# Theseus-AT/mlx-vector-db

Measured on AMD Instinct MI355X. Metric: QPS + p50 latency, cosine top-10 batch=64: 1M×768D @1 GPU; 10M×128D @8 GPU, higher is better.
Workload: dtype f32 (int8 centred corpus x int8 query integer-MFMA candidates, fp64 exact rerank); 1 GPU; c2: 1M x 768 fp32 cosine top-10, batch 64; n_rows=1000000, dim=768, global_batch=64, batch_per_gpu_equiv=64, k=10, metric=cosine, parallelism=single GPU, rows_per_gpu=1000000

## Files before the change

### mlx-vector-db_amd/csrc/vdb_api.cpp

```cpp
#include <hip/hip_runtime.h>

#include <algorithm>
#include <atomic>
#include <cmath>
#include <cstdarg>
#include <cstdio>
#include <cstring>
#include <mutex>
#include <set>
#include <unordered_map>
#include <shared_mutex>
#include <string>
#include <vector>

#include "../../include/vdb.h"
#include "vdb_compact_plan.h"
#include "vdb_subset_plan.h"
#include "vdb_range_plan.h"
#include "vdb_group_plan.h"
#include "vdb_search_plan.h"
#include "vdb_internal.h"

using namespace vdb;

namespace {

thread_local std::string g_last_error;

int set_error(int code, const char* fmt, ...) {
    char buf[1024];
    va_list ap;
    va_start(ap, fmt);
    vsnprintf(buf, sizeof(buf), fmt, ap);
    va_end(ap);
    g_last_error = buf;
    return code;
}

#define HIP_TRY(expr)                                                                                  \
    do {                                                                                               \
        hipError_t _e = (expr);                                                                        \
        if (_e != hipSuccess)                                                                          \
            return set_error(_e == hipErrorOutOfMemory ? VDB_ERR_OOM : VDB_ERR_HIP, "%s failed: %s (%s:%d)", \
                             #expr, hipGetErrorString(_e), __FILE__, __LINE__);                        \
    } while (0)

constexpr int64_t kRowAlign = ROW_ALIGN;

constexpr size_t kGatedExactBytes = 256u << 20;
constexpr int kSubsetBadWord = 12;

inline int64_t round_up(int64_t a, int64_t b) { return (a + b - 1) / b * b; }
inline int next_pow2(int v) {
    int p = 1;
    while (p < v) p <<= 1;
    return p;
}

struct Carver {
    char* base;
    size_t off = 0;
    template <typename T>
    T* take(size_t count) {
        off = (off + 255) & ~size_t(255);
        T* p = reinterpret_cast<T*>(base + off);
        off += count * sizeof(T);
        return p;
    }
};

struct Workspace {
    char* dev = nullptr;
    size_t dev_bytes = 0;
    char* exact = nullptr;
    size_t exact_cap = 0;
    int* host_flag = nullptr;
    char* host_io = nullptr;
    size_t host_io_bytes = 0;
    hipEvent_t done = nullptr;
    static constexpr int kTRing = 64;
    hipEvent_t tring[kTRing][4] = {};
    int t_head = 0, t_pending = 0;
    bool busy = false;
    bool used = false;
    hipStream_t last_st = nullptr;
    hipStream_t own = nullptr;
};

}

struct vdb_index {
    int dim = 0, metric = 0, device = 0;
    int Dp = 0, G = 0;
    int64_t count = 0;
    int64_t cap_rows = 0;
    float* X = nullptr;
    float* Xs = nullptr;
    float* Xq = nullptr;
    int8_t* Xh = nullptr;
    double* nrm64 = nullptr;
    float* inv32 = nullptr;
    float* sq32 = nullptr;
    float* rinit32 = nullptr;
    unsigned long long* d_xmax = nullptr;
    int* d_nonfinite = nullptr;
    double xmax = 0.0;
    double xres_rel = 0.0, xres_abs = 0.0;
    float* d_dir = nullptr;
    bool dir_set = false;
    double xres_dir = 0.0;
    float* d_mu = nullptr;
    float sx = 0.0f;
    int64_t dir_rows = 0;
    unsigned long long* d_i8 = nullptr;
    double i8st[6] = {0, 0, 0, 0, 0, 0};
    uint32_t* d_csum = nullptr;
    int64_t scan_checksum = 1;
    bool auto_i8 = true;
    hipStream_t stream = nullptr;
    int n_cu = 256;
    int64_t precision = VDB_PREC_AUTO;
    std::atomic<int> auto_hold{0}, auto_fails{0}, auto_ok{0};
    std::atomic<int> auto_hold8{0}, auto_fails8{0}, auto_ok8{0};
    std::atomic<bool> last_i8{false};
    std::atomic<unsigned long long> auto_seen{0};
    unsigned long long* h_totals = nullptr;
    int64_t margin = -1;
    int64_t force_exact = 0;
    int64_t n_wg_override = 0;
    int64_t timing = 0;
    int64_t pilot_tiles = -1;
    int64_t graph_fill = 0;
    int64_t scan_variant = 0;
    int64_t scan_variant_b3 = 0;
    int64_t scan_sync = 0;
    int64_t no_fallback = 0;
    int64_t pilot_rank_override = 0;
    bool no_dir_bound = false;
    int64_t finish_split = 1;
    int64_t finish_small = -1;
    int64_t scan_qlds = -1;
    int i8_refine = -1;
    int64_t device_repass = -1;
    std::atomic<int> repass_arm{0};
    int64_t i8_narrow = -1;
    std::atomic<bool> i8_wide{false};
    std::atomic<bool> auto_i8q{true};
    std::atomic<bool> i8q_off{false};
    std::atomic<bool> last_i8q{false};
    std::atomic<int> last_i8q_b{0};
    int64_t scan_q4 = -1;
    int64_t scan_wide = -1;
    int64_t remove_chunk = 0;
    int64_t update_chunk = 0;
    std::atomic<int64_t> gen{0};
    std::atomic<int64_t> n_searches{0}, n_queries{0}, n_fallback{0}, n_overflow{0}, n_incons{0}, n_repass{0}, n_q4{0};
    std::atomic<int64_t> n_wide{0};
    std::atomic<int64_t> n_xs_builds{0};
    std::atomic<int64_t> n_rows_removed{0};
    std::atomic<int64_t> n_rows_updated{0};
    std::atomic<int64_t> n_subset_searches{0}, n_subset_queries{0}, n_subset_rows{0};
    int64_t subset_wgs = 0;
    std::atomic<int64_t> n_range_searches{0}, n_range_queries{0};
    int32_t* groups = nullptr;
    uint32_t* group_valid = nullptr;
    int64_t group_n = 0, group_cap = 0;
    bool group_set = false, group_any_neg = false;
    int64_t group_valid_rows = 0;
    std::atomic<int64_t> n_group_sets{0}, n_group_searches{0}, n_group_queries{0};
    unsigned long long* d_group_fb = nullptr;
    int64_t group_fetch = 0;
    int64_t group_force_exact = 0;
    std::atomic<int64_t> n_by_prec[N_PREC] = {{0}, {0}, {0}, {0}, {0}, {0}};
    std::atomic<int64_t> scan_ns{0}, pipe_ns{0}, n_timed{0};
    unsigned long long* d_totals = nullptr;
    std::shared_mutex mu;
    std::mutex xs_mu;
    std::mutex ws_mu;
    std::vector<Workspace*> pool;
    std::unordered_map<hipStream_t, hipEvent_t> uses;
};

namespace {

std::mutex g_reg_mu;
std::set<vdb_index*> g_indices;

void free_workspace_memory(Workspace* w) {
    if (w->dev) (void)hipFree(w->dev);
    if (w->exact) (void)hipFree(w->exact);
    if (w->host_flag) (void)hipHostFree(w->host_flag);
    if (w->host_io) (void)hipHostFree(w->host_io);
    w->dev = nullptr;
    w->exact = nullptr;
    w->host_flag = nullptr;
    w->host_io = nullptr;
    w->dev_bytes = w->exact_cap = w->host_io_bytes = 0;
}

int wait_idle(vdb_index* ix);

enum XsKind { kXsNone = -1, kXsFp32 = 0, kXsSplit = 1 };
int xs_kind(int64_t precision) {
    if (precision == VDB_PREC_FP32) return kXsFp32;
    if (precision == VDB_PREC_I8 || precision == VDB_PREC_I8X3 || precision == VDB_PREC_I8Q) return kXsNone;
    return kXsSplit;
}
bool needs_i8(int64_t precision, bool auto_i8) {
    return precision == VDB_PREC_I8 || precision == VDB_PREC_I8X3 || precision == VDB_PREC_I8Q ||
           (precision == VDB_PREC_AUTO && auto_i8);
}
bool xs_eager(const vdb_index* ix) {
    const int kind = xs_kind(ix->precision);
    return kind == kXsFp32 || (kind == kXsSplit && !(ix->precision == VDB_PREC_AUTO && ix->auto_i8));
}
float* xs_ptr(const vdb_index* ix) { return __atomic_load_n(&ix->Xs, __ATOMIC_ACQUIRE); }

hipError_t build_candidate_rows(const vdb_index* ix, int64_t row0, int64_t n, hipStream_t st, bool xs = true,
                                bool xq = true) {
    const float* inv = ix->metric == VDB_METRIC_COSINE ? ix->inv32 : nullptr;
    hipError_t e = hipSuccess;
    if (xs && ix->Xs && xs_kind(ix->precision) == kXsFp32) e = launch_tile_rows(ix->X, ix->G, row0, n, ix->Xs, st);
    if (xs && ix->Xs && xs_kind(ix->precision) == kXsSplit) e = launch_split_rows(ix->X, ix->G, row0, n, inv, ix->Xs, st);
    if (e == hipSuccess && xq && needs_i8(ix->precision, ix->auto_i8)) {
        if (row0 == 0) e = hipMemsetAsync(ix->d_csum, 0, (size_t)2 * ix->Dp * sizeof(uint32_t), st);
        if (e == hipSuccess)
            e = launch_quant_rows(ix->X, inv, ix->d_mu, ix->d_dir, ix->sx, row0, n, ix->G, ix->Xq, ix->d_i8, st, ix->Xh);
        if (e == hipSuccess) e = launch_colsum8(ix->Xq, row0, n, ix->G / 4, ix->d_csum, st);
    }
    return e;
}

hipError_t read_i8_stats(vdb_index* ix, hipStream_t st) {
    unsigned long long b[6];
    hipError_t e = hipMemcpyAsync(b, ix->d_i8, sizeof(b), hipMemcpyDeviceToHost, st);
    if (e == hipSuccess) e = hipStreamSynchronize(st);
    if (e == hipSuccess) std::memcpy(ix->i8st, b, sizeof(b));
    return e;
}

hipError_t zero_now(void* p, size_t bytes, hipStream_t st) {
    hipError_t e = hipMemsetAsync(p, 0, bytes, st);
    if (e == hipSuccess) e = hipStreamSynchronize(st);
    return e;
}

bool debug_knobs_enabled() {
    const char* e = std::getenv("VDB_DEBUG_KNOBS");
    return e && std::strcmp(e, "1") == 0;
}

int ensure_capacity(vdb_index* ix, int64_t rows) {
    if (rows <= ix->cap_rows) return VDB_OK;
    if (ix->X) {
        const int wr = wait_idle(ix);
        if (wr) return wr;
    }
    int64_t cap = std::max<int64_t>(ix->cap_rows * 2, kRowAlign);
    while (cap < rows) cap *= 2;
    cap = round_up(cap, kRowAlign);
    const size_t tile_floats = (size_t)ix->G * BLOCK_FLOATS;
    const size_t x_bytes = (size_t)(cap / 32) * tile_floats * sizeof(float);
    float* X = nullptr;
    float* Xs = nullptr;
    float* Xq = nullptr;
    int8_t* Xh = nullptr;
    double* n64 = nullptr;
    float *i32 = nullptr, *s32 = nullptr, *r32 = nullptr;
    auto fail = [&](hipError_t e, const char* what) {
        (void)hipStreamSynchronize(ix->stream);
        for (void* p : {(void*)X, (void*)Xs, (void*)Xq, (void*)Xh, (void*)n64, (void*)i32, (void*)s32, (void*)r32})
            if (p) (void)hipFree(p);
        return set_error(e == hipErrorOutOfMemory ? VDB_ERR_OOM : VDB_ERR_HIP,
                         "growing the index to %lld rows: %s failed: %s", (long long)cap, what, hipGetErrorString(e));
    };
#define CAP_TRY(expr)                          \
    do {                                       \
        hipError_t _e = (expr);                \
        if (_e != hipSuccess) return fail(_e, #expr); \
    } while (0)
    CAP_TRY(hipMalloc(&X, x_bytes));
    if (ix->Xs || xs_eager(ix)) {
        CAP_TRY(hipMalloc(&Xs, x_bytes));
        CAP_TRY(hipMemsetAsync(Xs, 0, x_bytes, ix->stream));
    }
    const bool with_xq = ix->Xq || needs_i8(ix->precision, ix->auto_i8);
    if (with_xq) {
        CAP_TRY(hipMalloc(&Xq, x_bytes / 2));
        CAP_TRY(hipMemsetAsync(Xq, 0, x_bytes / 2, ix->stream));
        CAP_TRY(hipMalloc(&Xh, x_bytes / 4));
        CAP_TRY(hipMemsetAsync(Xh, 0, x_bytes / 4, ix->stream));
    }
    CAP_TRY(hipMalloc(&n64, cap * sizeof(double)));
    CAP_TRY(hipMalloc(&i32, cap * sizeof(float)));
    CAP_TRY(hipMalloc(&s32, cap * sizeof(float)));
    CAP_TRY(hipMalloc(&r32, cap * sizeof(float)));
    CAP_TRY(hipMemsetAsync(r32, 0, cap * sizeof(float), ix->stream));
    CAP_TRY(hipMemsetAsync(X, 0, x_bytes, ix->stream));
    CAP_TRY(hipMemsetAsync(n64, 0, cap * sizeof(double), ix->stream));
    CAP_TRY(hipMemsetAsync(i32, 0, cap * sizeof(float), ix->stream));
    CAP_TRY(hipMemsetAsync(s32, 0, cap * sizeof(float), ix->stream));
    if (ix->X) {
        const int64_t used_tiles = round_up(ix->count, 128) / 32;
        CAP_TRY(hipMemcpyAsync(X, ix->X, (size_t)ix->count * ix->Dp * sizeof(float), hipMemcpyDeviceToDevice,
                               ix->stream));
        if (Xs && ix->Xs)
            CAP_TRY(hipMemcpyAsync(Xs, ix->Xs, (size_t)used_tiles * tile_floats * sizeof(float),
                                   hipMemcpyDeviceToDevice, ix->stream));
        if (Xq && ix->Xq)
            CAP_TRY(hipMemcpyAsync(Xq, ix->Xq, (size_t)used_tiles * tile_floats * sizeof(float) / 2,
                                   hipMemcpyDeviceToDevice, ix->stream));
        if (Xh && ix->Xh)
            CAP_TRY(hipMemcpyAsync(Xh, ix->Xh, (size_t)ix->count * ix->Dp, hipMemcpyDeviceToDevice, ix->stream));
        CAP_TRY(hipMemcpyAsync(n64, ix->nrm64, ix->count * sizeof(double), hipMemcpyDeviceToDevice, ix->stream));
        CAP_TRY(hipMemcpyAsync(i32, ix->inv32, ix->count * sizeof(float), hipMemcpyDeviceToDevice, ix->stream));
        CAP_TRY(hipMemcpyAsync(s32, ix->sq32, ix->count * sizeof(float), hipMemcpyDeviceToDevice, ix->stream));
        CAP_TRY(hipMemcpyAsync(r32, ix->rinit32, ix->count * sizeof(float), hipMemcpyDeviceToDevice, ix->stream));
    }
    CAP_TRY(hipStreamSynchronize(ix->stream));
#undef CAP_TRY
    if (ix->X) {
        (void)hipFree(ix->X);
        if (ix->Xs) (void)hipFree(ix->Xs);
        if (ix->Xq) (void)hipFree(ix->Xq);
        if (ix->Xh) (void)hipFree(ix->Xh);
        (void)hipFree(ix->nrm64);
        (void)hipFree(ix->inv32);
        (void)hipFree(ix->sq32);
        (void)hipFree(ix->rinit32);
    }
    ix->X = X;
    ix->Xs = Xs;
    ix->Xq = Xq;
    ix->Xh = Xh;
    ix->nrm64 = n64;
    ix->inv32 = i32;
    ix->sq32 = s32;
    ix->rinit32 = r32;
    ix->cap_rows = cap;
    return VDB_OK;
}

int ensure_xq(vdb_index* ix) {
    if (ix->Xq || ix->cap_rows == 0) return VDB_OK;
    const size_t bytes = (size_t)(ix->cap_rows / 32) * ix->G * BLOCK_FLOATS * sizeof(float) / 2;
    float* Xq = nullptr;
    int8_t* Xh = nullptr;
    hipError_t e = hipMalloc(&Xq, bytes);
    if (e == hipSuccess) e = hipMalloc(&Xh, bytes / 2);
    if (e == hipSuccess) e = hipMemsetAsync(Xq, 0, bytes, ix->stream);
    if (e == hipSuccess) e = hipMemsetAsync(Xh, 0, bytes / 2, ix->stream);
    if (e == hipSuccess) e = hipStreamSynchronize(ix->stream);
    if (e != hipSuccess) {
        if (Xq) (void)hipFree(Xq);
        if (Xh) (void)hipFree(Xh);
        return set_error(e == hipErrorOutOfMemory ? VDB_ERR_OOM : VDB_ERR_HIP, "int8 copy: %s", hipGetErrorString(e));
    }
    ix->Xq = Xq;
    ix->Xh = Xh;
    return VDB_OK;
}

int ensure_xs(vdb_index* ix) {
    if (xs_ptr(ix) || ix->cap_rows == 0 || xs_kind(ix->precision) == kXsNone) return VDB_OK;
    std::lock_guard<std::mutex> lg(ix->xs_mu);
    if (ix->Xs) return VDB_OK;
    const size_t bytes = (size_t)(ix->cap_rows / 32) * ix->G * BLOCK_FLOATS * sizeof(float);
    float* Xs = nullptr;
    hipError_t e = hipMalloc(&Xs, bytes);
    if (e == hipSuccess) e = hipMemsetAsync(Xs, 0, bytes, ix->stream);
    if (e == hipSuccess && ix->count > 0) {
        const float* inv = ix->metric == VDB_METRIC_COSINE ? ix->inv32 : nullptr;
        e = xs_kind(ix->precision) == kXsFp32 ? launch_tile_rows(ix->X, ix->G, 0, ix->count, Xs, ix->stream)
                                              : launch_split_rows(ix->X, ix->G, 0, ix->count, inv, Xs, ix->stream);
    }
    if (e == hipSuccess) e = hipStreamSynchronize(ix->stream);
    if (e != hipSuccess) {
        if (Xs) (void)hipFree(Xs);
        return set_error(e == hipErrorOutOfMemory ? VDB_ERR_OOM : VDB_ERR_HIP, "split candidate copy: %s",
                         hipGetErrorString(e));
    }
    __atomic_store_n(&ix->Xs, Xs, __ATOMIC_RELEASE);
    ix->n_xs_builds++;
    return VDB_OK;
}

constexpr size_t kMaxWs = 16;

Workspace* acquire_ws(vdb_index* ix, hipStream_t st, bool own = false) {
    std::lock_guard<std::mutex> g(ix->ws_mu);
    Workspace* idle = nullptr;
    Workspace* any = nullptr;
    for (Workspace* w : ix->pool) {
        if (w->busy) continue;
        if (!w->used || (!own && w->last_st == st)) {
            w->busy = true;
            return w;
        }
        if (!idle && w->done && hipEventQuery(w->done) == hipSuccess) idle = w;
        if (!any) any = w;
    }
    Workspace* w = idle ? idle : ix->pool.size() >= kMaxWs ? any : nullptr;
    if (!w) {
        w = new Workspace();
        ix->pool.push_back(w);
    }
    w->busy = true;
    return w;
}

bool others_in_flight(vdb_index* ix, const Workspace* self) {
    std::lock_guard<std::mutex> g(ix->ws_mu);
    for (Workspace* w : ix->pool) {
        if (w == self) continue;
        if (w->busy) return true;
        if (w->used && w->done && hipEventQuery(w->done) == hipErrorNotReady) return true;
    }
    return false;
}

void release_ws(vdb_index* ix, Workspace* w, hipStream_t st) {
    if (w->done == nullptr) (void)hipEventCreateWithFlags(&w->done, hipEventDisableTiming);
    (void)hipEventRecord(w->done, st);
    w->used = true;
    w->last_st = st;
    std::lock_guard<std::mutex> g(ix->ws_mu);
    w->busy = false;
}

int note_use(vdb_index* ix, hipStream_t st) {
    std::lock_guard<std::mutex> g(ix->ws_mu);
    if (ix->uses.size() >= 64 && !ix->uses.count(st)) {
        for (auto it = ix->uses.begin(); it != ix->uses.end();) {
            if (hipEventQuery(it->second) == hipSuccess) {
                (void)hipEventDestroy(it->second);
                it = ix->uses.erase(it);
            } else {
                ++it;
            }
        }
    }
    hipEvent_t& e = ix->uses[st];
    if (!e) HIP_TRY(hipEventCreateWithFlags(&e, hipEventDisableTiming));
    HIP_TRY(hipEventRecord(e, st));
    return VDB_OK;
}

int wait_idle(vdb_index* ix) {
    std::vector<hipEvent_t> evs;
    {
        std::lock_guard<std::mutex> g(ix->ws_mu);
        for (Workspace* w : ix->pool)
            if (w->used && w->done) evs.push_back(w->done);
        for (auto& kv : ix->uses) evs.push_back(kv.second);
    }
    for (hipEvent_t e : evs) HIP_TRY(hipEventSynchronize(e));
    HIP_TRY(hipStreamSynchronize(ix->stream));
    return VDB_OK;
}

int flush_timing(vdb_index* ix, Workspace* w, int n = Workspace::kTRing) {
    while (w->t_pending > 0 && n-- > 0) {
        hipEvent_t* ev = w->tring[(w->t_head - w->t_pending + Workspace::kTRing) % Workspace::kTRing];
        HIP_TRY(hipEventSynchronize(ev[2]));
        float ms_scan = 0.f, ms_pipe = 0.f;
        HIP_TRY(hipEventElapsedTime(&ms_scan, ev[0], ev[1]));
        HIP_TRY(hipEventElapsedTime(&ms_pipe, ev[3], ev[2]));
        ix->scan_ns += (int64_t)(ms_scan * 1e6);
        ix->pipe_ns += (int64_t)(ms_pipe * 1e6);
        ix->n_timed++;
        w->t_pending--;
    }
    return VDB_OK;
}

int flush_all_timing(vdb_index* ix) {
    std::lock_guard<std::mutex> g(ix->ws_mu);
    for (Workspace* w : ix->pool)
        if (!w->busy) {
            const int rc = flush_timing(ix, w);
            if (rc) return rc;
        }
    return VDB_OK;
}

int ws_reserve(Workspace* w, size_t bytes, hipStream_t st) {
    if (w->used && w->done) HIP_TRY(hipStreamWaitEvent(st, w->done, 0));
    if (!w->host_flag) HIP_TRY(hipHostMalloc(&w->host_flag, 64 * sizeof(int), hipHostMallocDefault));
    if (bytes > w->dev_bytes) {
        if (w->dev) {
            HIP_TRY(hipStreamSynchronize(st));
            (void)hipFree(w->dev);
            w->dev = nullptr;
        }
        size_t nb = std::max(bytes, w->dev_bytes * 2);
        HIP_TRY(hipMalloc(&w->dev, nb));
        w->dev_bytes = nb;
    }
    return VDB_OK;
}

int ws_host_io(Workspace* w, size_t bytes) {
    if (bytes > w->host_io_bytes) {
        const size_t nb = std::max(bytes, w->host_io_bytes * 2);
        if (w->host_io) (void)hipHostFree(w->host_io);
        w->host_io = nullptr;
        w->host_io_bytes = 0;
        HIP_TRY(hipHostMalloc(&w->host_io, nb, hipHostMallocDefault));
        w->host_io_bytes = nb;
    }
    return VDB_OK;
}

int ws_reserve_exact(Workspace* w, size_t bytes, hipStream_t st) {
    if (bytes > w->exact_cap) {
        if (w->exact) {
            HIP_TRY(hipStreamSynchronize(st));
            (void)hipFree(w->exact);
            w->exact = nullptr;
        }
        HIP_TRY(hipMalloc(&w->exact, bytes));
        w->exact_cap = bytes;
    }
    return VDB_OK;
}

bool all_finite(const float* p, int64_t n) {
    for (int64_t i = 0; i < n; ++i)
        if (!std::isfinite(p[i])) return false;
    return true;
}

struct SearchLease {
    vdb_index* ix;
    Workspace* w = nullptr;
    hipStream_t st = nullptr;
    int rc = VDB_OK;
    SearchLease(vdb_index* ix_, int32_t mem, void* stream) : ix(ix_) {
        const bool own_stream = mem == VDB_MEM_HOST && !stream;
        st = own_stream ? nullptr : (hipStream_t)stream;
        w = acquire_ws(ix, st, own_stream);
        if (!own_stream) return;
        if (!w->own) {
            const hipError_t e = hipStreamCreateWithFlags(&w->own, hipStreamNonBlocking);
            if (e != hipSuccess) {
                {
                    std::lock_guard<std::mutex> lg(ix->ws_mu);
                    w->busy = false;
                }
                w = nullptr;
                rc = set_error(VDB_ERR_HIP, "workspace stream: %s", hipGetErrorString(e));
                return;
            }
        }
        st = w->own;
    }
    ~SearchLease() {
        if (w) release_ws(ix, w, st);
    }
    SearchLease(const SearchLease&) = delete;
    SearchLease& operator=(const SearchLease&) = delete;
};

hipError_t order_after_caller(hipStream_t st, void* caller_stream) {
    hipEvent_t ready = nullptr;
    hipError_t e = hipEventCreateWithFlags(&ready, hipEventDisableTiming);
    if (e != hipSuccess) return e;
    e = hipEventRecord(ready, (hipStream_t)caller_stream);
    if (e == hipSuccess) e = hipStreamWaitEvent(st, ready, 0);
    (void)hipEventDestroy(ready);
    return e;
}

template <typename Pack>
int stage_up(Workspace* w, int64_t in0, int64_t in_bytes, int64_t out_bytes, hipStream_t st, Pack&& pack) {
    const int rc = ws_host_io(w, (size_t)(in_bytes + out_bytes));
    if (rc) return rc;
    pack(w->host_io);
    HIP_TRY(hipMemcpyAsync(w->dev + in0, w->host_io, (size_t)in_bytes, hipMemcpyHostToDevice, st));
    return VDB_OK;
}
int stage_down(Workspace* w, int64_t in_bytes, int64_t out0, int64_t out_bytes, hipStream_t st, const char** r) {
    *r = w->host_io + in_bytes;
    HIP_TRY(hipMemcpyAsync(w->host_io + in_bytes, w->dev + out0, (size_t)out_bytes, hipMemcpyDeviceToHost, st));
    HIP_TRY(hipStreamSynchronize(st));
    return VDB_OK;
}


SearchKnobs search_knobs(const vdb_index* ix, bool i8_narrow) {
    SearchKnobs kn{};
    kn.force_exact = ix->force_exact != 0;
    kn.margin = ix->margin;
    kn.i8_narrow = i8_narrow;
    kn.scan_q4 = ix->scan_q4;
    kn.scan_wide = ix->scan_wide;
    kn.n_wg_override = ix->n_wg_override;
    kn.scan_variant = ix->scan_variant;
    kn.scan_sync = ix->scan_sync;
    kn.finish_split = ix->finish_split;
    kn.i8_refine = ix->i8_refine;
    kn.scan_checksum = ix->scan_checksum;
    kn.pilot_tiles = ix->pilot_tiles;
    kn.pilot_rank_override = ix->pilot_rank_override;
    kn.has_xh = ix->Xh != nullptr;
    kn.has_csum = ix->d_csum != nullptr;
    return kn;
}

SearchKernelFacts kernel_facts(const SearchShape& s, const SearchKnobs& kn, const SearchKP& kp) {
    SearchKernelFacts f{};
    const int Gs = search_groups(s.prec, s.G);
    if (prec_is_i8(s.prec)) {
        f.scan8wl_ok = scan8wl_ok(s.prec, s.metric, Gs, s.B);
        f.scan8w_ok = scan8w_ok(Gs, s.B);
        f.rows_per_step = scan8_rows_per_step(s.prec, s.metric);
    } else if (s.prec == PREC_BF16X3 || s.prec == PREC_BF16) {
        f.rows_per_step = scan2_rows_per_step(false);
        f.rows_per_step_q4 = scan2_rows_per_step(true);
    } else {
        f.scan_variant_ok = scan_variant_ok(s.prec, (int)kn.scan_variant, Gs);
        const int v = f.scan_variant_ok ? (int)kn.scan_variant : 0;
        f.rows_per_step = scan_rows_per_step(s.prec, v);
        f.scan_priv = scan_priv(s.prec, v, kp.KP);
    }
    return f;
}

size_t gated_exact_bytes(const vdb_index* ix, int nq, int k) {
    const ExactPlan ep = exact_plan(ix->count, ix->n_cu, nq, k, true);
    return (size_t)exact_gate_bytes(ep, nq, (int64_t)exact_scan_scratch_bytes(ep.KE, ep.n_wg_gate, ep.slots));
}

int run_exact(vdb_index* ix, Workspace* w, const float* Qd, const double* qn64, const int* qlist_dev, int nq, int k,
              const uint32_t* mask_dev, float* out_s, int64_t* out_i, double* out_k, int64_t index_offset,
              const int64_t* row_ids, hipStream_t st, const int* qcount_dev = nullptr, const int* ovf_dev = nullptr,
              int* done_dev = nullptr, unsigned long long* host_totals = nullptr) {
    const int64_t N = ix->count;
    const bool gated = qcount_dev != nullptr;
    const ExactPlan ep = exact_plan(N, ix->n_cu, nq, k, gated);
    const int KE = ep.KE, n_wg = ep.n_wg, n_lists = ep.n_wg;
    const int64_t rpw = ep.rpw;
    const ExactLayout el =
        exact_layout(ep, nq, gated && done_dev ? (int64_t)exact_scan_scratch_bytes(KE, n_wg, ep.slots) : 0);
    int rc = ws_reserve_exact(w, (size_t)el.total, st);
    if (rc) return rc;
    double* lk = reinterpret_cast<double*>(w->exact + el.lk);
    uint32_t* li = reinterpret_cast<uint32_t*>(w->exact + el.li);
    double* mk = reinterpret_cast<double*>(w->exact + el.mk);
    uint32_t* mi = reinterpret_cast<uint32_t*>(w->exact + el.mi);
    char* gscr = el.scr >= 0 ? w->exact + el.scr : nullptr;
    if (gated && done_dev) {
        const ExactTail tail{done_dev, mk, mi, k, index_offset, out_s, out_i, out_k, row_ids, host_totals};
        HIP_TRY(launch_exact_scan(ix->metric, KE, Qd, qn64, qlist_dev, nq, ix->X, ix->G, ix->dim, ix->nrm64, mask_dev,
                                  N, n_wg, rpw, lk, li, st, qcount_dev, ovf_dev, ix->d_totals, &tail, kGateSlots,
                                  gscr));
        return VDB_OK;
    }
    HIP_TRY(launch_exact_scan(ix->metric, KE, Qd, qn64, qlist_dev, nq, ix->X, ix->G, ix->dim, ix->nrm64, mask_dev, N,
                              n_wg, rpw, lk, li, st, qcount_dev, ovf_dev, gated ? ix->d_totals : nullptr));
    HIP_TRY(launch_merge_f64_u32(KE, lk, li, n_lists, KE, (int64_t)n_lists * KE, KE, nq, mk, mi, st, qcount_dev));
    HIP_TRY(launch_finalize_u32(ix->metric, mk, mi, KE, nq, qlist_dev, k, index_offset, out_s, out_i, out_k, st,
                                qcount_dev, row_ids));
    return VDB_OK;
}

}

extern "C" {

const char* vdb_last_error(void) { return g_last_error.c_str(); }

int32_t vdb_version(void) { return 2; }

int32_t vdb_device_count(int32_t* n) {
    int c = 0;
    hipError_t e = hipGetDeviceCount(&c);
    if (e != hipSuccess) c = 0;
    if (n) *n = c;
    return VDB_OK;
}

int32_t vdb_index_create(int32_t dim, int32_t metric, int32_t device, vdb_index** out) {
    if (!out) return set_error(VDB_ERR_INVALID, "out is NULL");
    *out = nullptr;
    if (dim <= 0 || dim > 65536) return set_error(VDB_ERR_INVALID, "dimension must be in [1, 65536], got %d", dim);
    if (metric != VDB_METRIC_COSINE && metric != VDB_METRIC_EUCLIDEAN)
        return set_error(VDB_ERR_UNSUPPORTED, "unsupported metric id %d (cosine=0, euclidean=1)", metric);
    int ndev = 0;
    if (hipGetDeviceCount(&ndev) != hipSuccess || ndev == 0)
        return set_error(VDB_ERR_NODEVICE, "no HIP device visible: the vdb core needs an MI355X (gfx950)");
    if (device < 0 || device >= ndev) return set_error(VDB_ERR_INVALID, "device %d out of range [0,%d)", device, ndev);
    HIP_TRY(hipSetDevice(device));
    hipDeviceProp_t prop;
    HIP_TRY(hipGetDeviceProperties(&prop, device));
    if (std::strncmp(prop.gcnArchName, "gfx950", 6) != 0)
        return set_error(VDB_ERR_NODEVICE, "device %d is %s; this build targets gfx950 only", device,
                         prop.gcnArchName);
    vdb_index* ix = new vdb_index();
    ix->dim = dim;
    ix->metric = metric;
    ix->device = device;
    ix->Dp = (int)round_up(dim, 64);
    ix->G = ix->Dp / GROUP_DIMS;
    ix->n_cu = prop.multiProcessorCount;
    if (const char* q4 = std::getenv("VDB_SCAN_Q4")) ix->scan_q4 = std::min(1, std::max(-1, std::atoi(q4)));
    if (const char* a8 = std::getenv("VDB_AUTO_I8")) ix->auto_i8 = std::atoi(a8) != 0;
    hipError_t e = hipStreamCreateWithFlags(&ix->stream, hipStreamNonBlocking);
    if (e == hipSuccess) e = hipMalloc(&ix->d_xmax, 192);
    if (e == hipSuccess) e = zero_now(ix->d_xmax, 192, ix->stream);
    if (e == hipSuccess) e = hipMalloc(&ix->d_i8, 64);
    if (e == hipSuccess) e = zero_now(ix->d_i8, 64, ix->stream);
    if (e == hipSuccess) e = hipMalloc(&ix->d_csum, (size_t)2 * ix->Dp * sizeof(uint32_t));
    if (e == hipSuccess) e = zero_now(ix->d_csum, (size_t)2 * ix->Dp * sizeof(uint32_t), ix->stream);
    if (e != hipSuccess) {
        delete ix;
        return set_error(VDB_ERR_HIP, "index setup failed: %s", hipGetErrorString(e));
    }
    ix->d_nonfinite = reinterpret_cast<int*>(reinterpret_cast<char*>(ix->d_xmax) + 32);
    {
        std::lock_guard<std::mutex> rg(g_reg_mu);
        g_indices.insert(ix);
    }
    *out = ix;
    return VDB_OK;
}

int32_t vdb_index_destroy(vdb_index* ix) {
    if (!ix) return VDB_OK;
    {
        std::lock_guard<std::mutex> rg(g_reg_mu);
        g_indices.erase(ix);
    }
    (void)hipSetDevice(ix->device);
    (void)wait_idle(ix);
    for (Workspace* w : ix->pool) {
        free_workspace_memory(w);
        if (w->done) (void)hipEventDestroy(w->done);
        if (w->own) (void)hipStreamDestroy(w->own);
        for (int r = 0; r < Workspace::kTRing; ++r)
            for (int e = 0; e < 4; ++e)
                if (w->tring[r][e]) (void)hipEventDestroy(w->tring[r][e]);
        delete w;
    }
    if (ix->X) (void)hipFree(ix->X);
    if (ix->Xs) (void)hipFree(ix->Xs);
    if (ix->Xq) (void)hipFree(ix->Xq);
    if (ix->Xh) (void)hipFree(ix->Xh);
    if (ix->nrm64) (void)hipFree(ix->nrm64);
    if (ix->inv32) (void)hipFree(ix->inv32);
    if (ix->sq32) (void)hipFree(ix->sq32);
    if (ix->rinit32) (void)hipFree(ix->rinit32);
    if (ix->d_xmax) (void)hipFree(ix->d_xmax);
    if (ix->d_dir) (void)hipFree(ix->d_dir);
    if (ix->d_mu) (void)hipFree(ix->d_mu);
    if (ix->d_i8) (void)hipFree(ix->d_i8);
    if (ix->d_csum) (void)hipFree(ix->d_csum);
    if (ix->d_totals) (void)hipFree(ix->d_totals);
    if (ix->groups) (void)hipFree(ix->groups);
    if (ix->group_valid) (void)hipFree(ix->group_valid);
    if (ix->d_group_fb) (void)hipFree(ix->d_group_fb);
    if (ix->h_totals) (void)hipHostFree(ix->h_totals);
    for (auto& kv : ix->uses) (void)hipEventDestroy(kv.second);
    if (ix->stream) (void)hipStreamDestroy(ix->stream);
    delete ix;
    return VDB_OK;
}

int32_t vdb_index_reserve(vdb_index* ix, int64_t rows) {
    if (!ix) return set_error(VDB_ERR_INVALID, "index is NULL");
    if (rows < 0) return set_error(VDB_ERR_INVALID, "rows must be >= 0");
    HIP_TRY(hipSetDevice(ix->device));
    std::unique_lock<std::shared_mutex> g(ix->mu);
    return ensure_capacity(ix, rows);
}

int32_t vdb_index_set_param(vdb_index* ix, const char* name, int64_t value) {
    if (!ix || !name) return set_error(VDB_ERR_INVALID, "NULL argument");
    std::string n(name);
    if (n == "precision") {
        if (value != VDB_PREC_FP32 && value != VDB_PREC_BF16X3 && value != VDB_PREC_BF16 && value != VDB_PREC_AUTO &&
            value != VDB_PREC_I8 && value != VDB_PREC_I8X3 && value != VDB_PREC_I8Q)
            return set_error(VDB_ERR_INVALID,
                             "precision must be %d (fp32), %d (bf16x3), %d (bf16), %d (auto), %d (i8), %d (i8x3) or "
                             "%d (i8q), got %lld",
                             VDB_PREC_FP32, VDB_PREC_BF16X3, VDB_PREC_BF16, VDB_PREC_AUTO, VDB_PREC_I8, VDB_PREC_I8X3,
                             VDB_PREC_I8Q, (long long)value);
        HIP_TRY(hipSetDevice(ix->device));
        std::unique_lock<std::shared_mutex> g(ix->mu);
        if (value == ix->precision) return VDB_OK;
        const int wr = wait_idle(ix);
        if (wr) return wr;
        const bool xs = xs_kind(value) != kXsNone && xs_kind(value) != xs_kind(ix->precision);
        const bool xq = needs_i8(value, ix->auto_i8) && !needs_i8(ix->precision, ix->auto_i8);
        if (xq) {
            const int xr = ensure_xq(ix);
            if (xr) return xr;
        }
        ix->precision = value;
        bool built = false;
        if (!ix->Xs && xs_eager(ix)) {
            const int xr = ensure_xs(ix);
            if (xr) return xr;
            built = true;
        }
        if (((xs && !built) || xq) && ix->X && ix->count > 0) {
            HIP_TRY(build_candidate_rows(ix, 0, ix->count, ix->stream, xs && !built, xq));
            HIP_TRY(read_i8_stats(ix, ix->stream));
        }
    } else if (n == "auto_i8q") {
        ix->auto_i8q = value != 0;
    } else if (n == "auto_int8") {
        HIP_TRY(hipSetDevice(ix->device));
        std::unique_lock<std::shared_mutex> g(ix->mu);
        const bool v = value != 0;
        if (v == ix->auto_i8) return VDB_OK;
        const int wr = wait_idle(ix);
        if (wr) return wr;
        const bool xq = needs_i8(ix->precision, v) && !needs_i8(ix->precision, ix->auto_i8);
        if (xq) {
            const int xr = ensure_xq(ix);
            if (xr) return xr;
        }
        ix->auto_i8 = v;
        if (!ix->Xs && xs_eager(ix)) {
            const int xr = ensure_xs(ix);
            if (xr) return xr;
        }
        if (xq && ix->X && ix->count > 0) {
            HIP_TRY(build_candidate_rows(ix, 0, ix->count, ix->stream, false, true));
            HIP_TRY(read_i8_stats(ix, ix->stream));
        }
    } else if (n == "margin") {
        ix->margin = value;
    } else if (n == "force_exact") {
        ix->force_exact = value != 0;
    } else if (n == "n_wg") {
        ix->n_wg_override = value;
    } else if (n == "scan_sync") {
        if (value < 0 || value > 2) return set_error(VDB_ERR_INVALID, "scan_sync must be 0, 1 or 2");
        ix->scan_sync = value;
    } else if (n == "scan_variant") {
        if (value < 0 || value > 2) return set_error(VDB_ERR_INVALID, "scan_variant must be 0, 1 or 2");
        ix->scan_variant = value;
    } else if (n == "scan_variant_bf16x3") {
        if (value != 0) return set_error(VDB_ERR_INVALID, "the split-bf16 pass has one variant (0)");
        ix->scan_variant_b3 = value;
    } else if (n == "graph_fill") {
        if (value < 0 || value > 1) return set_error(VDB_ERR_INVALID, "graph_fill must be 0 or 1");
        ix->graph_fill = value;
    } else if (n == "pilot_tiles") {
        if (value < -1 || value > 32768) return set_error(VDB_ERR_INVALID, "pilot_tiles must be in [-1, 32768]");
        ix->pilot_tiles = value;
    } else if (n == "timing") {
        ix->timing = value != 0;
    } else if (n == "no_fallback") {
        ix->no_fallback = value != 0;
    } else if (n == "finish_small") {
        if (value < -1 || value > 1) return set_error(VDB_ERR_INVALID, "finish_small must be -1, 0 or 1");
        ix->finish_small = value;
    } else if (n == "finish_split") {
        if (value < 1 || value > 8) return set_error(VDB_ERR_INVALID, "finish_split must be in [1, 8]");
        ix->finish_split = value;
    } else if (n == "scan_qlds") {
        if (value < -1 || value > 2) return set_error(VDB_ERR_INVALID, "scan_qlds must be -1 (auto), 0, 1 or 2");
        ix->scan_qlds = value;
    } else if (n == "scan_wide") {
        if (value < -1 || value > 1) return set_error(VDB_ERR_INVALID, "scan_wide must be -1, 0 or 1");
        ix->scan_wide = value;
    } else if (n == "scan_q4") {
        if (value < -1 || value > 1) return set_error(VDB_ERR_INVALID, "scan_q4 must be -1, 0 or 1");
        ix->scan_q4 = value;
    } else if (n == "dir_bound") {
        ix->no_dir_bound = value == 0;
    } else if (n == "i8_refine") {
        if (value < -1 || value > 1) return set_error(VDB_ERR_INVALID, "i8_refine must be -1, 0 or 1");
        ix->i8_refine = (int)value;
    } else if (n == "i8_narrow") {
        if (value < -1 || value > 0) return set_error(VDB_ERR_INVALID, "i8_narrow must be -1 or 0");
        ix->i8_narrow = value;
    } else if (n == "remove_chunk") {
        if (value < 0) return set_error(VDB_ERR_INVALID, "remove_chunk must be >= 0 (0 = sized by bytes)");
        std::unique_lock<std::shared_mutex> g(ix->mu);
        ix->remove_chunk = value;
    } else if (n == "update_chunk") {
        if (value < 0) return set_error(VDB_ERR_INVALID, "update_chunk must be >= 0 (0 = sized by bytes)");
        std::unique_lock<std::shared_mutex> g(ix->mu);
        ix->update_chunk = value;
    } else if (n == "subset_wgs") {
        if (value < 0 || value > kSubsetMaxSeg)
            return set_error(VDB_ERR_INVALID, "subset_wgs must be in [0, %d] (0 = auto)", kSubsetMaxSeg);
        std::unique_lock<std::shared_mutex> g(ix->mu);
        ix->subset_wgs = value;
    } else if (n == "group_fetch") {
        if (value < 0 || value > kGroupMaxFetch)
            return set_error(VDB_ERR_INVALID, "group_fetch must be in [0, %d] (0 = auto)", kGroupMaxFetch);
        std::unique_lock<std::shared_mutex> g(ix->mu);
        ix->group_fetch = value;
    } else if (n == "group_force_exact") {
        if (value < 0 || value > 1) return set_error(VDB_ERR_INVALID, "group_force_exact must be 0 or 1");
        std::unique_lock<std::shared_mutex> g(ix->mu);
        ix->group_force_exact = value;
    } else if (n == "device_repass") {
        if (value < -1 || value > 1) return set_error(VDB_ERR_INVALID, "device_repass must be -1, 0 or 1");
        ix->device_repass = value;
    } else if (n.rfind("debug_", 0) == 0 && !debug_knobs_enabled()) {
        return set_error(VDB_ERR_INVALID, "'%s' is a test-only knob (set VDB_DEBUG_KNOBS=1)", name);
    } else if (n == "debug_sink_row8") {
        HIP_TRY(hipSetDevice(ix->device));
        std::unique_lock<std::shared_mutex> g(ix->mu);
        if (value < 0 || value >= ix->count || !ix->Xq)
            return set_error(VDB_ERR_INVALID, "debug_sink_row8: no int8 row %lld", (long long)value);
        const int wr = wait_idle(ix);
        if (wr) return wr;
        HIP_TRY(launch_sink_row8(ix->Xq, value, ix->G / 4, ix->stream));
        HIP_TRY(hipStreamSynchronize(ix->stream));
    } else if (n == "scan_checksum") {
        if (value < 0 || value > 2) return set_error(VDB_ERR_INVALID, "scan_checksum must be 0, 1 or 2");
        ix->scan_checksum = value;
    } else if (n == "debug_stale_rinit") {
        if (value < 0) return set_error(VDB_ERR_INVALID, "debug_stale_rinit: row must be >= 0");
        HIP_TRY(hipSetDevice(ix->device));
        std::unique_lock<std::shared_mutex> g(ix->mu);
        if (value >= ix->count || !ix->rinit32) return set_error(VDB_ERR_INVALID, "debug_stale_rinit: no row %lld", (long long)value);
        const int wr = wait_idle(ix);
        if (wr) return wr;
        const float zero = 0.0f;
        HIP_TRY(hipMemcpyAsync(ix->rinit32 + value, &zero, sizeof(float), hipMemcpyHostToDevice, ix->stream));
        HIP_TRY(hipStreamSynchronize(ix->stream));
    } else if (n == "pilot_rank") {
        if (value < 0 || value > 256) return set_error(VDB_ERR_INVALID, "pilot_rank must be in [0, 256]");
        ix->pilot_rank_override = value;
    } else {
        return set_error(VDB_ERR_INVALID, "unknown parameter '%s'", name);
    }
    return VDB_OK;
}

int32_t vdb_index_get_stat(const vdb_index* cix, const char* name, int64_t* value) {
    if (!cix || !name || !value) return set_error(VDB_ERR_INVALID, "NULL argument");
    vdb_index* ix = const_cast<vdb_index*>(cix);
    std::string n(name);
    unsigned long long dt[4] = {0, 0, 0, 0};
    if ((n == "fallback_queries" || n == "overflow_queries" || n == "repass_queries") && ix->d_totals) {
        HIP_TRY(hipSetDevice(ix->device));
        const int wr = wait_idle(ix);
        if (wr) return wr;
        HIP_TRY(hipMemcpy(dt, ix->d_totals, sizeof(dt), hipMemcpyDeviceToHost));
    }
    if (n == "scan_ns" || n == "pipeline_ns" || n == "timed_searches") {
        HIP_TRY(hipSetDevice(ix->device));
        const int rc = flush_all_timing(ix);
        if (rc) return rc;
    }
    if (n == "searches") *value = ix->n_searches.load();
    else if (n == "queries") *value = ix->n_queries.load();
    else if (n == "fallback_queries") *value = ix->n_fallback.load() + (int64_t)dt[0];
    else if (n == "repass_queries") *value = ix->n_repass.load() + (int64_t)dt[3];
    else if (n == "searches_q4") *value = ix->n_q4.load();
    else if (n == "searches_wide") *value = ix->n_wide.load();
    else if (n == "auto_hold") *value = ix->auto_hold.load();
    else if (n == "auto_hold8") *value = ix->auto_hold8.load();
    else if (n == "overflow_queries") *value = ix->n_overflow.load() + (int64_t)dt[1];
    else if (n == "inconsistent_queries") *value = ix->n_incons.load();
    else if (n == "capacity") *value = ix->cap_rows;
    else if (n == "scan_ns") *value = ix->scan_ns.load();
    else if (n == "pipeline_ns") *value = ix->pipe_ns.load();
    else if (n == "timed_searches") *value = ix->n_timed.load();
    else if (n == "count") *value = ix->count;
    else if (n == "precision") *value = ix->precision;
    else if (n == "searches_fp32") *value = ix->n_by_prec[PREC_FP32].load();
    else if (n == "searches_bf16x3") *value = ix->n_by_prec[PREC_BF16X3].load();
    else if (n == "searches_bf16") *value = ix->n_by_prec[PREC_BF16].load();
    else if (n == "searches_i8") *value = ix->n_by_prec[PREC_I8].load();
    else if (n == "searches_i8x3") *value = ix->n_by_prec[PREC_I8X3].load();
    else if (n == "auto_int8") *value = ix->auto_i8 ? 1 : 0;
    else if (n == "auto_i8q") *value = ix->auto_i8q ? 1 : 0;
    else if (n == "i8q_off") *value = ix->i8q_off.load() ? 1 : 0;
    else if (n == "searches_i8q") *value = ix->n_by_prec[PREC_I8Q].load();
    else if (n == "i8_wide") *value = ix->i8_wide ? 1 : 0;
    else if (n == "device_bytes") {
        const int64_t xb = (int64_t)(ix->cap_rows / 32) * ix->G * BLOCK_FLOATS * 4;
        *value = xb + (xs_ptr(ix) ? xb : 0) + (ix->Xq ? xb / 2 : 0) + (ix->Xh ? xb / 4 : 0) + ix->cap_rows * 20;
    } else if (n == "split_copy") *value = xs_ptr(ix) ? 1 : 0;
    else if (n == "split_copy_builds") *value = ix->n_xs_builds.load();
    else if (n == "rows_removed") *value = ix->n_rows_removed.load();
    else if (n == "rows_updated") *value = ix->n_rows_updated.load();
    else if (n == "subset_searches") *value = ix->n_subset_searches.load();
    else if (n == "subset_queries") *value = ix->n_subset_queries.load();
    else if (n == "subset_rows") *value = ix->n_subset_rows.load();
    else if (n == "range_searches") *value = ix->n_range_searches.load();
    else if (n == "range_queries") *value = ix->n_range_queries.load();
    else if (n == "group_rows") *value = ix->group_set ? ix->group_n : 0;
    else if (n == "group_sets") *value = ix->n_group_sets.load();
    else if (n == "group_searches") *value = ix->n_group_searches.load();
    else if (n == "group_queries") *value = ix->n_group_queries.load();
    else if (n == "group_fallback_queries") {
        unsigned long long fb = 0;
        if (ix->d_group_fb) {
            HIP_TRY(hipSetDevice(ix->device));
            const int wr = wait_idle(ix);
            if (wr) return wr;
            HIP_TRY(hipMemcpy(&fb, ix->d_group_fb, sizeof(fb), hipMemcpyDeviceToHost));
        }
        *value = (int64_t)fb;
    }
    else if (n == "subset_bad_ids") {
        HIP_TRY(hipSetDevice(ix->device));
        const int wr = wait_idle(ix);
        if (wr) return wr;
        unsigned long long bad = 0;
        HIP_TRY(hipMemcpy(&bad, ix->d_xmax + kSubsetBadWord, sizeof(bad), hipMemcpyDeviceToHost));
        *value = (int64_t)bad;
    }
    else return set_error(VDB_ERR_INVALID, "unknown stat '%s'", name);
    return VDB_OK;
}

constexpr int64_t kDirRows = 65536;

static hipError_t setup_direction(vdb_index* ix, int64_t row0, int64_t n, hipStream_t st) {
    if (ix->dir_set) return hipSuccess;
    const float* inv = ix->metric == VDB_METRIC_COSINE ? ix->inv32 : nullptr;
    const int D = ix->dim;
    const int64_t m = std::min(n, kDirRows);
    hipError_t e = hipSuccess;
    if (!ix->d_dir) e = hipMalloc(&ix->d_dir, (size_t)ix->Dp * sizeof(float));
    if (e == hipSuccess && !ix->d_mu) e = hipMalloc(&ix->d_mu, (size_t)ix->Dp * sizeof(float));
    double* sums = nullptr;
    if (e == hipSuccess) e = hipMalloc(&sums, (size_t)D * sizeof(double));
    if (e == hipSuccess) e = hipMemsetAsync(sums, 0, (size_t)D * sizeof(double), st);
    if (e == hipSuccess) e = launch_dir_sum(ix->X, inv, row0, m, D, ix->G, sums, st);
    std::vector<double> h(D);
    if (e == hipSuccess) e = hipMemcpyAsync(h.data(), sums, (size_t)D * sizeof(double), hipMemcpyDeviceToHost, st);
    if (e == hipSuccess) e = hipStreamSynchronize(st);
    if (sums) (void)hipFree(sums);
    if (e != hipSuccess) return e;
    double nn = 0.0;
    for (double v : h) nn += v * v;
    std::vector<float> dir(ix->Dp, 0.0f), mu(ix->Dp, 0.0f);
    if (nn > 0.0 && std::isfinite(nn))
        for (int d = 0; d < D; ++d) dir[d] = (float)(h[d] / std::sqrt(nn));
    for (int d = 0; d < D; ++d) mu[d] = (float)(h[d] / (double)std::max<int64_t>(m, 1));
    e = hipMemcpyAsync(ix->d_dir, dir.data(), (size_t)ix->Dp * sizeof(float), hipMemcpyHostToDevice, st);
    if (e == hipSuccess)
        e = hipMemcpyAsync(ix->d_mu, mu.data(), (size_t)ix->Dp * sizeof(float), hipMemcpyHostToDevice, st);
    uint32_t zb = 0;
    uint32_t* dz = reinterpret_cast<uint32_t*>(ix->d_i8 + 6);
    if (e == hipSuccess) e = hipMemsetAsync(dz, 0, sizeof(uint32_t), st);
    if (e == hipSuccess) e = launch_zmax(ix->X, inv, ix->d_mu, row0, m, D, ix->G, dz, st);
    if (e == hipSuccess) e = hipMemcpyAsync(&zb, dz, sizeof(zb), hipMemcpyDeviceToHost, st);
    if (e == hipSuccess) e = hipStreamSynchronize(st);
    if (e != hipSuccess) return e;
    float zmax = 0.0f;
    std::memcpy(&zmax, &zb, sizeof(zmax));
    ix->sx = zmax > 0.0f && std::isfinite(zmax) ? 1.25f * zmax / 127.0f : 1.0f;
    ix->dir_rows = m;
    ix->dir_set = true;
    return hipSuccess;
}

static hipError_t residual_direction(vdb_index* ix, int64_t row0, int64_t n, hipStream_t st) {
    const float* inv = ix->metric == VDB_METRIC_COSINE ? ix->inv32 : nullptr;
    return launch_resid_dir(ix->X, inv, row0, n, ix->dim, ix->G, ix->d_dir, ix->d_xmax + 3, st);
}

int32_t vdb_index_add(vdb_index* ix, const float* vectors, int64_t n, int32_t mem, void* stream) {
    if (!ix) return set_error(VDB_ERR_INVALID, "index is NULL");
    if (n < 0) return set_error(VDB_ERR_INVALID, "n must be >= 0");
    if (n == 0) return VDB_OK;
    if (!vectors) return set_error(VDB_ERR_INVALID, "vectors is NULL");
    if (ix->count + n > (int64_t)0xFFFFFFFE) return set_error(VDB_ERR_INVALID, "index is limited to 2^32-2 rows");
    HIP_TRY(hipSetDevice(ix->device));
    std::unique_lock<std::shared_mutex> g(ix->mu);
    hipStream_t st = ix->stream;
    int rc = ensure_capacity(ix, ix->count + n);
    if (rc) return rc;
    if (ix->count > 0 && ix->dir_rows < kDirRows) {
        const int wr = wait_idle(ix);
        if (wr) return wr;
    }
    HIP_TRY(hipMemsetAsync(ix->d_nonfinite, 0, sizeof(int), st));
    char* bak = reinterpret_cast<char*>(ix->d_xmax);
    HIP_TRY(hipMemcpyAsync(bak + 64, ix->d_xmax, 32, hipMemcpyDeviceToDevice, st));
    HIP_TRY(hipMemcpyAsync(bak + 128, ix->d_i8, 64, hipMemcpyDeviceToDevice, st));
    if (mem == VDB_MEM_DEVICE) {
        HIP_TRY(order_after_caller(st, stream));
    }
    const int D = ix->dim;
    const int64_t chunk = std::max<int64_t>(1, (int64_t)(256ll << 20) / ((int64_t)D * 4));
    float* staging = nullptr;
    if (mem == VDB_MEM_HOST) HIP_TRY(hipMalloc(&staging, (size_t)std::min(chunk, n) * D * sizeof(float)));
    for (int64_t r = 0; r < n; r += chunk) {
        const int64_t m = std::min(chunk, n - r);
        const float* src = vectors + r * D;
        if (mem == VDB_MEM_HOST) {
            hipError_t e = hipMemcpyAsync(staging, src, (size_t)m * D * sizeof(float), hipMemcpyHostToDevice, st);
            if (e == hipSuccess)
                e = launch_pack_rows(staging, m, D, ix->G, ix->X, ix->count + r, ix->nrm64, ix->inv32, ix->sq32,
                                     ix->rinit32, ix->metric == VDB_METRIC_COSINE, ix->d_xmax, ix->d_nonfinite, st);
            if (e == hipSuccess) e = setup_direction(ix, ix->count + r, m, st);
            if (e == hipSuccess) e = build_candidate_rows(ix, ix->count + r, m, st);
            if (e == hipSuccess) e = residual_direction(ix, ix->count + r, m, st);
            if (e == hipSuccess) e = hipStreamSynchronize(st);
            if (e != hipSuccess) {
                (void)hipFree(staging);
                return set_error(VDB_ERR_HIP, "ingest failed: %s", hipGetErrorString(e));
            }
        } else {
            HIP_TRY(launch_pack_rows(src, m, D, ix->G, ix->X, ix->count + r, ix->nrm64, ix->inv32, ix->sq32,
                                     ix->rinit32, ix->metric == VDB_METRIC_COSINE, ix->d_xmax, ix->d_nonfinite, st));
            HIP_TRY(setup_direction(ix, ix->count + r, m, st));
            HIP_TRY(build_candidate_rows(ix, ix->count + r, m, st));
            HIP_TRY(residual_direction(ix, ix->count + r, m, st));
        }
    }
    if (staging) (void)hipFree(staging);
    int nonfinite = 0;
    unsigned long long xb[4] = {0, 0, 0, 0};
    HIP_TRY(hipMemcpyAsync(&nonfinite, ix->d_nonfinite, sizeof(int), hipMemcpyDeviceToHost, st));
    HIP_TRY(hipMemcpyAsync(xb, ix->d_xmax, sizeof(xb), hipMemcpyDeviceToHost, st));
    HIP_TRY(read_i8_stats(ix, st));
    if (nonfinite) {
        if (ix->count == 0) {
            ix->dir_set = false;
            ix->dir_rows = 0;
            HIP_TRY(hipMemsetAsync(ix->d_xmax, 0, 32, st));
            HIP_TRY(hipMemsetAsync(ix->d_i8, 0, 64, st));
            HIP_TRY(hipStreamSynchronize(st));
            std::memset(ix->i8st, 0, sizeof(ix->i8st));
        } else {
            HIP_TRY(hipMemcpyAsync(ix->d_xmax, bak + 64, 32, hipMemcpyDeviceToDevice, st));
            HIP_TRY(hipMemcpyAsync(ix->d_i8, bak + 128, 64, hipMemcpyDeviceToDevice, st));
            if (ix->Xq && needs_i8(ix->precision, ix->auto_i8)) {
                HIP_TRY(hipMemsetAsync(ix->d_csum, 0, (size_t)2 * ix->Dp * sizeof(uint32_t), st));
                HIP_TRY(launch_colsum8(ix->Xq, 0, ix->count, ix->G / 4, ix->d_csum, st));
            }
            HIP_TRY(read_i8_stats(ix, st));
        }
        return set_error(VDB_ERR_NONFINITE, "%d row(s) contain NaN or Inf; nothing was added", nonfinite);
    }
    if (ix->dir_rows < kDirRows && ix->count + n >= 2 * ix->dir_rows) {
        const int64_t all = ix->count + n;
        ix->dir_set = false;
        HIP_TRY(hipMemsetAsync(ix->d_xmax + 3, 0, 8, st));
        HIP_TRY(hipMemsetAsync(ix->d_i8, 0, 64, st));
        HIP_TRY(setup_direction(ix, 0, all, st));
        if (needs_i8(ix->precision, ix->auto_i8)) HIP_TRY(build_candidate_rows(ix, 0, all, st, false, true));
        HIP_TRY(residual_direction(ix, 0, all, st));
        HIP_TRY(hipMemcpyAsync(xb, ix->d_xmax, sizeof(xb), hipMemcpyDeviceToHost, st));
        HIP_TRY(read_i8_stats(ix, st));
    }
    double xm[4];
    std::memcpy(xm, xb, sizeof(xm));
    ix->xmax = xm[0];
    ix->xres_rel = xm[1];
    ix->xres_abs = xm[2];
    ix->xres_dir = xm[3];
    ix->count += n;
    ix->group_set = false;
    ix->auto_hold = 0;
    ix->auto_fails = 0;
    ix->auto_hold8 = 0;
    ix->auto_fails8 = 0;
    if (ix->h_totals) ix->auto_seen = ix->h_totals[0];
    return VDB_OK;
}

int32_t vdb_index_count(const vdb_index* ix, int64_t* n) {
    if (!ix || !n) return set_error(VDB_ERR_INVALID, "NULL argument");
    *n = ix->count;
    return VDB_OK;
}

static int32_t clear_locked(vdb_index* ix) {
    {
        const int wr = wait_idle(ix);
        if (wr) return wr;
    }
    if (ix->X) {
        HIP_TRY(hipMemsetAsync(ix->X, 0, (size_t)(ix->cap_rows / 32) * ix->G * BLOCK_FLOATS * sizeof(float),
                               ix->stream));
        HIP_TRY(hipMemsetAsync(ix->nrm64, 0, ix->cap_rows * sizeof(double), ix->stream));
        if (ix->Xs)
            HIP_TRY(hipMemsetAsync(ix->Xs, 0, (size_t)(ix->cap_rows / 32) * ix->G * BLOCK_FLOATS * sizeof(float),
                                   ix->stream));
        if (ix->Xq)
            HIP_TRY(hipMemsetAsync(ix->Xq, 0, (size_t)(ix->cap_rows / 32) * ix->G * BLOCK_FLOATS * sizeof(float) / 2,
                                   ix->stream));
    }
    HIP_TRY(hipMemsetAsync(ix->d_xmax, 0, 64, ix->stream));
    HIP_TRY(hipMemsetAsync(ix->d_i8, 0, 64, ix->stream));
    HIP_TRY(hipMemsetAsync(ix->d_csum, 0, (size_t)2 * ix->Dp * sizeof(uint32_t), ix->stream));
    HIP_TRY(hipStreamSynchronize(ix->stream));
    std::memset(ix->i8st, 0, sizeof(ix->i8st));
    ix->count = 0;
    ix->group_set = false;
    ix->auto_hold = 0;
    ix->auto_fails = 0;
    ix->auto_hold8 = 0;
    ix->auto_fails8 = 0;
    ix->xmax = 0.0;
    ix->xres_rel = ix->xres_abs = 0.0;
    ix->dir_set = false;
    ix->dir_rows = 0;
    ix->xres_dir = 0.0;
    ix->gen++;
    return VDB_OK;
}

// ... 219 lines not shown
                                            ix->d_i8, ix->Xh, st));
            UP_TRY(launch_update_colsum8(ix->Xq, d_ids, m, N, G8, +1, ix->d_csum, st));
        }
        UP_TRY(launch_update_resid_dir(ix->X, inv, d_ids, m, N, D, ix->G, ix->d_dir, ix->d_xmax + 3, st));
        if (host && r + m < n) UP_TRY(hipStreamSynchronize(st));
    }
    unsigned long long xb[4] = {0, 0, 0, 0};
    UP_TRY(hipMemcpyAsync(xb, ix->d_xmax, sizeof(xb), hipMemcpyDeviceToHost, st));
    UP_TRY(read_i8_stats(ix, st));
#undef UP_TRY
    (void)done(VDB_OK);
    double xm[4];
    std::memcpy(xm, xb, sizeof(xm));
    ix->xmax = xm[0];
    ix->xres_rel = xm[1];
    ix->xres_abs = xm[2];
    ix->xres_dir = xm[3];
    ix->gen++;
    ix->n_rows_updated += n;
    ix->auto_hold = 0;
    ix->auto_fails = 0;
    ix->auto_hold8 = 0;
    ix->auto_fails8 = 0;
    if (ix->h_totals) ix->auto_seen = ix->h_totals[0];
    return VDB_OK;
}

int32_t vdb_index_get_vectors(vdb_index* ix, int64_t start, int64_t n, float* out_host) {
    if (!ix || (!out_host && n > 0)) return set_error(VDB_ERR_INVALID, "NULL argument");
    if (start < 0 || n < 0 || start + n > ix->count)
        return set_error(VDB_ERR_INVALID, "rows [%lld, %lld) out of range [0, %lld)", (long long)start,
                         (long long)(start + n), (long long)ix->count);
    if (n == 0) return VDB_OK;
    HIP_TRY(hipSetDevice(ix->device));
    std::shared_lock<std::shared_mutex> g(ix->mu);
    const int D = ix->dim;
    const int64_t chunk = std::max<int64_t>(1, (int64_t)(256ll << 20) / ((int64_t)D * 4));
    float* tmp = nullptr;
    HIP_TRY(hipMalloc(&tmp, (size_t)std::min(chunk, n) * D * sizeof(float)));
    for (int64_t r = 0; r < n; r += chunk) {
        const int64_t m = std::min(chunk, n - r);
        hipError_t e = launch_unpack_rows(ix->X, ix->G, D, start + r, m, tmp, ix->stream);
        if (e == hipSuccess)
            e = hipMemcpyAsync(out_host + r * D, tmp, (size_t)m * D * sizeof(float), hipMemcpyDeviceToHost, ix->stream);
        if (e == hipSuccess) e = hipStreamSynchronize(ix->stream);
        if (e != hipSuccess) {
            (void)hipFree(tmp);
            return set_error(VDB_ERR_HIP, "export failed: %s", hipGetErrorString(e));
        }
    }
    (void)hipFree(tmp);
    return VDB_OK;
}

constexpr int32_t kRetryBf16x3 = 1 << 20;
constexpr int kRepassMax = 64;
constexpr int kRepassArm = 256;
constexpr int kAutoBf16MaxK = 16;

void auto_fail(vdb_index* ix) {
    const int f = std::min(8, ix->auto_fails.load() + 1);
    ix->auto_fails = f;
    ix->auto_ok = 0;
    ix->auto_hold = 16 << (f - 1);
}

bool auto_take_hold(vdb_index* ix) {
    int h = ix->auto_hold.load();
    while (h > 0)
        if (ix->auto_hold.compare_exchange_weak(h, h - 1)) return true;
    if (++ix->auto_ok >= 64) ix->auto_fails = 0;
    return false;
}

void auto_fail8(vdb_index* ix) {
    const int f = std::min(8, ix->auto_fails8.load() + 1);
    ix->auto_fails8 = f;
    ix->auto_ok8 = 0;
    ix->auto_hold8 = 16 << (f - 1);
}
bool auto_take_hold8(vdb_index* ix) {
    int h = ix->auto_hold8.load();
    while (h > 0)
        if (ix->auto_hold8.compare_exchange_weak(h, h - 1)) return true;
    if (++ix->auto_ok8 >= 64) ix->auto_fails8 = 0;
    return false;
}

static int32_t search_locked(vdb_index* ix, const float* queries, int32_t B, int32_t k, const uint32_t* row_mask,
                             int32_t mem, float* out_scores, int64_t* out_indices, double* out_keys,
                             int64_t index_offset, void* stream, const int64_t* row_ids, struct SearchOpts opt);

static int repass_flagged(vdb_index* ix, const float* Qd, const int* flag_list, int n, int k, const uint32_t* md,
                          float* out_s, int64_t* out_i, double* out_k, int64_t index_offset, const int64_t* row_ids,
                          hipStream_t st);

struct SearchOpts {
    bool force_b3 = false;
    bool repass = false;
    const int* gate = nullptr;
    bool force_i8x3 = false;
};

static int32_t search_locked(vdb_index* ix, const float* queries, int32_t B, int32_t k, const uint32_t* row_mask,
                             int32_t mem, float* out_scores, int64_t* out_indices, double* out_keys,
                             int64_t index_offset, void* stream, const int64_t* row_ids, SearchOpts opt);

static int32_t search_impl(vdb_index* ix, const float* queries, int32_t B, int32_t k, const uint32_t* row_mask,
                           int32_t mem, float* out_scores, int64_t* out_indices, double* out_keys,
                           int64_t index_offset, void* stream, const int64_t* row_ids, bool force_b3 = false) {
    if (!ix) return set_error(VDB_ERR_INVALID, "index is NULL");
    if (B <= 0) return set_error(VDB_ERR_INVALID, "n_queries must be >= 1, got %d", B);
    if (k <= 0 || k > 1024) return set_error(VDB_ERR_INVALID, "k must be in [1, 1024], got %d", k);
    if (!queries || !out_scores || !out_indices) return set_error(VDB_ERR_INVALID, "NULL query/output pointer");
    if (mem != VDB_MEM_HOST && mem != VDB_MEM_DEVICE) return set_error(VDB_ERR_INVALID, "bad mem kind %d", mem);
    if (mem == VDB_MEM_HOST && !all_finite(queries, (int64_t)B * ix->dim))
        return set_error(VDB_ERR_NONFINITE, "query contains NaN or Inf");
    HIP_TRY(hipSetDevice(ix->device));
    std::shared_lock<std::shared_mutex> g(ix->mu);
    SearchOpts opt;
    opt.force_b3 = force_b3;
    return search_locked(ix, queries, B, k, row_mask, mem, out_scores, out_indices, out_keys, index_offset, stream,
                         row_ids, opt);
}

static int repass_flagged(vdb_index* ix, const float* Qd, const int* flag_list, int n, int k, const uint32_t* md,
                          float* out_s, int64_t* out_i, double* out_k, int64_t index_offset, const int64_t* row_ids,
                          hipStream_t st) {
    const int D = ix->dim;
    const size_t qb = round_up((int64_t)n * D * 4, 256), sb = round_up((int64_t)n * k * 4, 256),
                 lb = round_up((int64_t)n * k * 8, 256);
    char* buf = nullptr;
    HIP_TRY(hipMallocAsync((void**)&buf, qb + sb + 2 * lb, st));
    float* Qs = (float*)buf;
    float* ss = (float*)(buf + qb);
    int64_t* si = (int64_t*)(buf + qb + sb);
    double* sk = (double*)(buf + qb + sb + lb);
    hipError_t e = launch_gather_rows(Qd, D, flag_list, n, Qs, st);
    int rc = e == hipSuccess ? VDB_OK : set_error(VDB_ERR_HIP, "re-pass gather: %s", hipGetErrorString(e));
    if (rc == VDB_OK) {
        SearchOpts o;
        o.force_b3 = true;
        o.repass = true;
        rc = search_locked(ix, Qs, n, k, md, VDB_MEM_DEVICE, ss, si, sk, index_offset, st, row_ids, o);
    }
    if (rc == VDB_OK) {
        e = launch_scatter_results(flag_list, n, k, ss, si, sk, out_s, out_i, out_k, st);
        if (e != hipSuccess) rc = set_error(VDB_ERR_HIP, "re-pass scatter: %s", hipGetErrorString(e));
    }
    (void)hipFreeAsync(buf, st);
    ix->n_repass += n;
    return rc;
}

static int32_t search_locked(vdb_index* ix, const float* queries, int32_t B, int32_t k, const uint32_t* row_mask,
                             int32_t mem, float* out_scores, int64_t* out_indices, double* out_keys,
                             int64_t index_offset, void* stream, const int64_t* row_ids, SearchOpts opt) {
    const int D = ix->dim;
    const int64_t N = ix->count;
    if (!opt.repass) {
        ix->n_searches++;
        ix->n_queries += B;
    }

    const bool auto_prec = ix->precision == VDB_PREC_AUTO;
    if (auto_prec && ix->h_totals && !opt.repass) {
        const unsigned long long seen = ix->h_totals[0];
        const unsigned long long prev = ix->auto_seen.exchange(seen);
        if (seen > prev) {
            if (ix->last_i8q && seen - prev > (unsigned long long)std::max(1, ix->last_i8q_b.load() / 8))
                ix->i8q_off = true;
            if (ix->last_i8) {
                auto_fail8(ix);
                ix->i8_wide = true;
            } else {
                auto_fail(ix);
            }
            ix->repass_arm = kRepassArm;
        }
    }
    const bool approx = N > 0 && !(ix->force_exact || k > kMaxApproxK);
    const bool auto_b16 = k <= kAutoBf16MaxK;
    const bool x3_i8 = auto_prec && !opt.force_b3 && !auto_b16 && ix->auto_i8;
    const bool auto_x3 = auto_prec && (opt.force_b3 || !auto_b16 || (approx && auto_take_hold(ix)));
    const bool hold8 = auto_prec && ix->auto_i8 && approx && (x3_i8 || !auto_x3) && auto_take_hold8(ix);
    const bool auto_8 = auto_prec && !auto_x3 && ix->auto_i8 && !hold8;
    const bool auto_8x3 = x3_i8 && !hold8;
    const bool auto_8q = auto_8x3 && ix->metric == 1 && k <= 100 && ix->auto_i8q && !ix->i8q_off;
    const bool force_8x3 = auto_prec && opt.force_i8x3 && ix->auto_i8 && ix->Xq;
    const int prec_req = !ix->X ? PREC_FP32
                         : force_8x3 ? PREC_I8X3
                         : ix->precision == VDB_PREC_BF16X3 ? PREC_BF16X3
                         : ix->precision == VDB_PREC_BF16 ? PREC_BF16
                         : ix->precision == VDB_PREC_I8X3 ? PREC_I8X3
                         : ix->precision == VDB_PREC_I8Q ? PREC_I8Q
                         : ix->precision == VDB_PREC_I8 ? PREC_I8
                         : auto_prec ? (auto_x3 ? (auto_8x3 ? (auto_8q ? PREC_I8Q : PREC_I8X3) : PREC_BF16X3)
                                                 : auto_8 ? PREC_I8 : PREC_BF16)
                                     : PREC_FP32;
    if (auto_prec && approx && (!auto_x3 || x3_i8)) {
        ix->last_i8 = auto_8 || auto_8x3;
        ix->last_i8q = prec_req == PREC_I8Q;
        ix->last_i8q_b = (int)B;
    }
    if (approx && !opt.gate) ix->n_by_prec[prec_req]++;
    const bool one_plane = prec_req == PREC_BF16 || prec_req == PREC_I8;

    const int prec = prec_req;
    SearchShape sh{};
    sh.B = B; sh.k = k; sh.D = D; sh.Dp = ix->Dp; sh.G = ix->G; sh.metric = ix->metric; sh.N = N; sh.n_cu = ix->n_cu;
    sh.prec = prec; sh.host = mem == VDB_MEM_HOST; sh.gated = opt.gate != nullptr; sh.repass = opt.repass;
    const SearchKnobs kn = search_knobs(ix, auto_prec && ix->i8_narrow != 0 && !ix->i8_wide);
    const SearchKP kp = search_kp(sh, kn);
    const int KP = kp.KP;
    const bool exact_all = kp.exact_all;
    if (!prec_is_i8(prec) && !exact_all && N > 0 && !xs_ptr(ix)) {
        const int xr = ensure_xs(ix);
        if (xr) return xr;
    }
    const SearchGeometry g = search_geometry(sh, kn, kp, kernel_facts(sh, kn, kp));
    const SearchPilot pilot = search_pilot(sh, kn, kp, g);
    const SearchLayout lay = search_layout(sh, g, pilot);
    const bool i8_pass = g.i8_pass, split_pass = g.split_pass, q4 = g.q4, wide_long = g.wide_long, wide8 = g.wide8;
    const bool priv = g.priv, i8_refine = g.i8_refine, chk = g.chk, chk_l = g.chk_l;
    const int Gs = g.Gs, n_seg8 = g.n_seg8, QB = g.QB, QB_pilot = g.QB_pilot, Bp = g.Bp, n_qblocks = g.n_qblocks;
    const int variant = g.variant, n_wg = g.n_wg, spw = g.spw, lockstep = g.lockstep, n_wg8 = g.n_wg8;
    const int fin_split = g.fin_split, R_rep = g.R_rep, n_pilot = pilot.n_pilot, pilot_rank = pilot.pilot_rank;
    const int64_t n_steps = g.n_steps, mask_words = g.mask_words, gl_cap = g.gl_cap;

    SearchLease lease(ix, mem, stream);
    if (lease.rc) return lease.rc;
    Workspace* const w = lease.w;
    const hipStream_t st = lease.st;
    int rc = ws_reserve(w, (size_t)lay.total, st);
    if (rc) return rc;
    char* const dev = w->dev;
    auto at = [dev](int64_t off) { return off < 0 ? nullptr : dev + off; };
    float* Qraw = (float*)at(lay.Qraw);
    uint32_t* maskd = (uint32_t*)at(lay.maskd);
    float* Qt = (float*)at(lay.Qt);
    double* qn64 = (double*)at(lay.qn64);
    double* qconst = (double*)at(lay.qconst);
    const float* q_mu = i8_pass ? ix->d_mu : nullptr;
    const float* q_dir = (prec == PREC_BF16 || i8_pass) && ix->dir_set && !ix->no_dir_bound ? ix->d_dir : nullptr;
    float* os = (float*)at(lay.os);
    int64_t* oi = (int64_t*)at(lay.oi);
    double* ok = (double*)at(lay.ok);
    int* flags = (int*)at(lay.flags);
    int* done = (int*)at(lay.done);
    uint32_t* gthr = (uint32_t*)at(lay.gthr);
    uint32_t* gslots = (uint32_t*)at(lay.gslots);
    uint32_t* pslots = gslots + (size_t)Bp * KP_MAX;
    float* gl_s = (float*)at(lay.gl_s);
    uint32_t* gl_i = (uint32_t*)at(lay.gl_i);
    uint32_t* gl_cnt = (uint32_t*)at(lay.gl_cnt);
    double* fx_ek = (double*)at(lay.fx_ek);
    uint32_t* fx_ck = (uint32_t*)at(lay.fx_ck);
    uint32_t* fx_cr = (uint32_t*)at(lay.fx_cr);
    int* fx_n = (int*)at(lay.fx_n);
    float* q8max = (float*)at(lay.q8max);
    float* q8lsl = (float*)at(lay.q8lsl);
    float* q8err = (float*)at(lay.q8err);
    float* q8scal = (float*)at(lay.q8scal);
    float* q8res = (float*)at(lay.q8res);
    float* q8err2 = (float*)at(lay.q8err2);
    uint32_t* chkp = (uint32_t*)at(lay.chkp);
    uint32_t* segc = (uint32_t*)at(lay.segc);
    uint32_t* chkr = (uint32_t*)at(lay.chkr);
    int* rs8 = (int*)at(lay.rs8);
    uint32_t* chke = (uint32_t*)at(lay.chke);
    float* rep_q = (float*)at(lay.rep_q);
    float* rep_s = (float*)at(lay.rep_s);
    int64_t* rep_i = (int64_t*)at(lay.rep_i);
    double* rep_k = (double*)at(lay.rep_k);

    const float* Qd = queries;
    const uint32_t* md = row_mask;
    float* out_s = out_scores;
    int64_t* out_i = out_indices;
    double* out_k = out_keys;
    const size_t io_q = mem == VDB_MEM_HOST ? (size_t)B * D * 4 : 0;
    const size_t io_r = (size_t)B * k * (4 + 8 + (out_keys ? 8 : 0));
    bool staged = false;
    if (mem == VDB_MEM_HOST) {
        rc = ws_host_io(w, io_q + io_r);
        if (rc) return rc;
        std::memcpy(w->host_io, queries, io_q);
        HIP_TRY(hipMemcpyAsync(Qraw, w->host_io, io_q, hipMemcpyHostToDevice, st));
        Qd = Qraw;
        if (row_mask && N > 0) {
            HIP_TRY(hipMemcpyAsync(maskd, row_mask, (size_t)mask_words * 4, hipMemcpyHostToDevice, st));
            md = maskd;
        }
        out_s = os;
        out_i = oi;
        out_k = out_keys ? ok : nullptr;
    }

    if (N == 0) {
        HIP_TRY(launch_empty_results((int64_t)B * k, out_s, out_i, out_k, st));
    } else {
        HIP_TRY(launch_prep_queries(Qd, B, Bp, D, ix->G, ix->metric, prec == PREC_FP32 ? Qt : nullptr,
                                    split_pass ? Qt : nullptr, qn64, flags, gthr, gslots, gl_cnt, done, st,
                                    i8_pass ? q8max : nullptr, q_mu, q_dir, qconst));
        if (i8_pass && !exact_all) {
            Int8Consts c8;
            c8.sx = ix->sx;
            c8.zmax_h = ix->i8st[4];
            c8.xl_max = ix->i8st[5];
            c8.rmax_half = 0.5 * ix->xmax * ix->xmax;
            HIP_TRY(launch_prep8(Qd, qn64, q8max, B, Bp, D, Gs, ix->metric, prec, c8, Qt, q8lsl, q8err, q8scal, st,
                                 q8res, q8err2));
            if (rs8) {
                if (chkr) HIP_TRY(hipMemsetAsync(chkr, 0, sizeof(uint32_t), st));
                HIP_TRY(launch_rstart8(ix->rinit32, N, q8scal, rs8, chkr, st));
            }
        }
        int n_flag = 0;
        if (!exact_all) {
            const bool timed = ix->timing != 0 && !opt.gate;
            hipEvent_t* tev = nullptr;
            if (timed) {
                if (w->t_pending == Workspace::kTRing) {
                    const int frc = flush_timing(ix, w, 1);
                    if (frc) return frc;
                }
                tev = w->tring[w->t_head];
                w->t_head = (w->t_head + 1) % Workspace::kTRing;
                w->t_pending++;
                for (int e = 0; e < 4; ++e)
                    if (!tev[e]) HIP_TRY(hipEventCreate(&tev[e]));
                HIP_TRY(hipEventRecord(tev[3], st));
            }
            const float* rowscale = ix->metric == 0 ? ix->inv32 : ix->sq32;
            const float* Xscan = i8_pass ? ix->Xq : xs_ptr(ix);
            if (n_pilot > 0) {
                if (i8_pass) {
                    HIP_TRY(launch_pilot8(prec, ix->metric, Xscan, ix->rinit32, md, Qt, q8scal, Gs, N, B,
                                          (B + QB_pilot - 1) / QB_pilot, QB_pilot, n_pilot, pslots, st,
                                          chke ? ix->d_csum : nullptr, chke, wide_long));
                    HIP_TRY(launch_pilot_bound(pslots, B, pilot_rank, gthr, st));
                } else if (split_pass) {
                    HIP_TRY(launch_pilot2(prec, ix->metric, pilot_rank, Xscan, ix->rinit32, md, Qt, Gs, N, B,
                                          (B + QB_pilot - 1) / QB_pilot, QB_pilot, n_pilot, pslots, gthr, st));
                    HIP_TRY(launch_pilot_bound(pslots, B, pilot_rank, gthr, st));
                }
                else
                    HIP_TRY(launch_pilot(prec, ix->metric, pilot_rank, Xscan, rowscale, md, Qt, Gs, N, B,
                                         n_qblocks, QB, n_pilot, pslots, gthr, st));
            }
            if (opt.gate && (q4 || !(split_pass || i8_pass)))
                return set_error(VDB_ERR_INVALID, "device re-pass: the sub-search has no gated candidate pass");
            if (timed) HIP_TRY(hipEventRecord(tev[0], st));
            if (q4) ix->n_q4++;
            if (wide8) ix->n_wide++;
            if (wide_long)
                HIP_TRY(launch_scan8wl(prec, ix->metric, Xscan, md, Qt, q8lsl, q8scal, Gs, N, B, n_seg8, gl_s, gl_i,
                                       gl_cap, segc, gthr, chkp, st));
            else if (wide8)
                HIP_TRY(launch_scan8w(prec, ix->metric, Xscan, rs8, md, Qt, q8lsl, q8scal, Gs, N, B, Bp, n_seg8, gl_s, gl_i,
                                      gl_cap, segc, gthr, chkp, Bp, chk_l ? 1 : 0, st));
            else if (i8_pass)
                HIP_TRY(launch_scan8(prec, ix->metric, KP, Xscan, (const float*)rs8, md, Qt, q8lsl, q8scal, Gs, N, B,
                                     n_qblocks, n_steps, n_wg, spw, gl_s, gl_i, gl_cnt, gl_cap, gthr, lockstep,
                                     (int)ix->scan_qlds, st, opt.gate, chkp, Bp, chk_l ? 1 : 0));
            else if (split_pass)
                HIP_TRY(launch_scan2(prec, ix->metric, KP, Xscan, ix->rinit32, md, Qt, Gs, N, B, n_qblocks, n_steps,
                                     n_wg, spw, gl_s, gl_i, gl_cnt, gl_cap, gthr, lockstep, st, q4,
                                     (int)ix->scan_qlds, opt.gate));
            else if (priv)
                HIP_TRY(launch_scan_topk_priv(prec, ix->metric, KP, Xscan, rowscale, md, Qt, Gs, N, B, n_qblocks,
                                              n_steps, n_wg, spw, gl_s, gl_i, gl_cnt, gl_cap, gthr, gslots, st));
            else
                HIP_TRY(launch_scan_topk(prec, ix->metric, KP, variant, Xscan, rowscale, md, Qt, Gs, N, B, n_qblocks,
                                         n_steps, n_wg, spw, gl_s, gl_i, gl_cnt, gl_cap, gthr, gslots, lockstep, st));
            if (timed) HIP_TRY(hipEventRecord(tev[1], st));
            FinishArgs fa;
            fa.gl_s = gl_s; fa.gl_i = gl_i; fa.gl_cnt = gl_cnt; fa.gl_cap = gl_cap;
            fa.Q = Qd; fa.qn64 = qn64; fa.X = ix->X; fa.G = ix->G; fa.D = D; fa.nrm64 = ix->nrm64; fa.k = k;
            fa.eps_rel = i8_pass ? 1.01 * 8.0 * std::ldexp(1.0, -24)
                         : prec == PREC_FP32 ? 1.01 * (double)(D + 8) * std::ldexp(1.0, -24)
                         : prec == PREC_BF16X3
                             ? 1.01 * (3.0 * D * std::ldexp(1.0, -23) + 3.1 * std::ldexp(1.0, -16) +
                                       8.0 * std::ldexp(1.0, -24))
                             : 1.01 * (2.0 * D * std::ldexp(1.0, -23) + 1.1 * std::ldexp(1.0, -16) +
                                       8.0 * std::ldexp(1.0, -24));
            fa.xmax = ix->xmax;
            fa.xres = prec != PREC_BF16 ? 0.0 : 1.01 * (ix->metric == 0 ? ix->xres_rel : ix->xres_abs);
            fa.dir = prec == PREC_BF16 && ix->dir_set && !ix->no_dir_bound ? ix->d_dir : nullptr;
            fa.dres = 1.01 * ix->xres_dir;
            if (i8_pass) {
                fa.xres = 1.01 * ix->i8st[prec == PREC_I8X3 ? 2 : 0] + 1e-300;
                fa.dir = ix->dir_set && !ix->no_dir_bound ? ix->d_dir : nullptr;
                fa.dres = 1.01 * ix->i8st[prec == PREC_I8X3 ? 3 : 1];
                fa.qerr = q8err;
                fa.mu = ix->d_mu;
                if (i8_refine) {
                    fa.xh_rm = ix->Xh;
                    fa.qres = q8res;
                    fa.qerr2 = q8err2;
                    fa.qscal = q8scal;
                    fa.sx = ix->sx;
                    fa.Dp = ix->Dp;
                }
            }
            fa.out_s = out_s; fa.out_i = out_i; fa.out_k = out_k; fa.index_offset = index_offset;
            fa.row_ids = row_ids;
            fa.flag_count = flags; fa.flag_list = flags + 1; fa.gthr = gthr; fa.overflow_count = flags + B + 1;
            fa.incons_count = flags + B + 2;
            fa.gate = opt.gate;
            if (chk) {
                fa.chkp = chkp;
                fa.chke = chke;
                fa.chkr = chkr;
                fa.chk_q = Qt;
                fa.chk_csum = ix->d_csum;
                fa.chk_g8 = Gs;
                fa.chk_nw = n_wg8;
                fa.chk_ld = Bp;
                fa.chk_l = chk_l;
            }
            fa.qconst = fa.mu == q_mu && fa.dir == q_dir ? qconst : nullptr;
            fa.seg_cnt = segc;
            fa.seg_n = n_seg8;
            fa.small = D <= 1024 && (ix->finish_small == 1 ||
                                     (ix->finish_small < 0 && B >= 32 &&
                                      ((wide_long && Gs <= 32) || (wide8 && !wide_long)) &&
                                      others_in_flight(ix, w))) ? 1 : 0;
            fa.split = fin_split; fa.sx_ek = fx_ek; fa.sx_ck = fx_ck; fa.sx_cr = fx_cr; fa.sx_n = fx_n; fa.done = done;
            HIP_TRY(launch_finish(ix->metric, KP, fa, B, st));
            if (timed) HIP_TRY(hipEventRecord(tev[2], st));
            if (ix->no_fallback && mem == VDB_MEM_DEVICE) return VDB_OK;
            if (!ix->no_fallback && mem == VDB_MEM_DEVICE && gated_exact_bytes(ix, B, k) <= kGatedExactBytes) {
                {
                    std::lock_guard<std::mutex> lg(ix->ws_mu);
                    if (!ix->d_totals) {
                        HIP_TRY(hipHostMalloc(&ix->h_totals, 2 * sizeof(unsigned long long), hipHostMallocDefault));
                        ix->h_totals[0] = ix->h_totals[1] = 0;
                        unsigned long long* d = nullptr;
                        HIP_TRY(hipMalloc(&d, 4 * sizeof(unsigned long long)));
                        HIP_TRY(zero_now(d, 4 * sizeof(unsigned long long), ix->stream));
                        ix->d_totals = d;
                    }
                }
                unsigned long long* htot =
                    auto_prec && (one_plane || prec == PREC_I8X3 || prec == PREC_I8Q) ? ix->h_totals : nullptr;
                const bool can_rep = !opt.repass && auto_prec && (one_plane || prec == PREC_I8X3 || prec == PREC_I8Q) &&
                                     xs_kind(VDB_PREC_BF16X3) == xs_kind(ix->precision) && rep_q &&
                                     k <= kMaxApproxK;
                bool rep = can_rep && ix->device_repass == 1;
                if (can_rep && ix->device_repass < 0) {
                    int a = ix->repass_arm.load();
                    while (a > 0 && !ix->repass_arm.compare_exchange_weak(a, a - 1)) {}
                    rep = a > 0;
                }
                if (rep) {
                    int* counts = flags + B + 3;
                    HIP_TRY(launch_repass_gather(Qd, D, flags, R_rep, rep_q, counts, ix->d_totals + 3, st));
                    SearchOpts o;
                    o.force_b3 = true;
                    o.force_i8x3 = true;
                    o.repass = true;
                    o.gate = counts;
                    rc = search_locked(ix, rep_q, R_rep, k, md, VDB_MEM_DEVICE, rep_s, rep_i, rep_k, index_offset, st,
                                       row_ids, o);
                    if (rc) return rc;
                    HIP_TRY(launch_scatter_results(flags + 1, R_rep, k, rep_s, rep_i, rep_k, out_s, out_i, out_k, st,
                                                   counts));
                    if (B > R_rep)
                        rc = run_exact(ix, w, Qd, qn64, flags + 1 + R_rep, B - R_rep, k, md, out_s, out_i, out_k,
                                       index_offset, row_ids, st, counts + 1, flags + B + 1, done + R_rep, htot);
                    return rc;
                }
                rc = run_exact(ix, w, Qd, qn64, flags + 1, B, k, md, out_s, out_i, out_k, index_offset, row_ids, st,
                               flags, flags + B + 1, done, htot);
                return rc;
            }
            HIP_TRY(hipMemcpyAsync(w->host_flag, flags, sizeof(int), hipMemcpyDeviceToHost, st));
            HIP_TRY(hipMemcpyAsync(w->host_flag + 1, flags + B + 1, 2 * sizeof(int), hipMemcpyDeviceToHost, st));
            if (mem == VDB_MEM_HOST) {
                char* r = w->host_io + io_q;
                HIP_TRY(hipMemcpyAsync(r, out_s, (size_t)B * k * 4, hipMemcpyDeviceToHost, st));
                HIP_TRY(hipMemcpyAsync(r + (size_t)B * k * 4, out_i, (size_t)B * k * 8, hipMemcpyDeviceToHost, st));
                if (out_keys)
                    HIP_TRY(hipMemcpyAsync(r + (size_t)B * k * 12, out_k, (size_t)B * k * 8, hipMemcpyDeviceToHost, st));
            }
            HIP_TRY(hipStreamSynchronize(st));
            n_flag = w->host_flag[0];
            staged = mem == VDB_MEM_HOST && n_flag == 0;
            if (prec == PREC_I8 && n_flag > 0) ix->i8_wide = true;
            ix->n_overflow += w->host_flag[1];
            ix->n_incons += w->host_flag[2];
            if (auto_prec && one_plane && n_flag > 0 && !ix->no_fallback) {
                if (n_flag <= std::max(1, B / 8) && n_flag <= kRepassMax) {
                    if (timed) {
                        const int frc = flush_timing(ix, w);
                        if (frc) return frc;
                    }
                    rc = repass_flagged(ix, Qd, flags + 1, n_flag, k, md, out_s, out_i, out_k, index_offset,
                                        row_ids, st);
                    if (rc) return rc;
                    n_flag = 0;
                } else {
                    if (prec == PREC_I8) auto_fail8(ix);
                    else auto_fail(ix);
                    ix->n_searches--;
                    ix->n_queries -= B;
                    return kRetryBf16x3;
                }
            }
            if (auto_prec && prec == PREC_I8X3 && n_flag > std::max(1, B / 8) && !ix->no_fallback) auto_fail8(ix);
            if (auto_prec && prec == PREC_I8Q && n_flag > std::max(1, B / 8) && !ix->no_fallback) ix->i8q_off = true;
            if (timed) {
                const int frc = flush_timing(ix, w);
                if (frc) return frc;
            }
            if (n_flag > 0 && !ix->no_fallback) {
                ix->n_fallback += n_flag;
                rc = run_exact(ix, w, Qd, qn64, flags + 1, n_flag, k, md, out_s, out_i, out_k, index_offset, row_ids,
                               st);
                if (rc) return rc;
            }
        } else {
            ix->n_fallback += B;
            rc = run_exact(ix, w, Qd, qn64, nullptr, B, k, md, out_s, out_i, out_k, index_offset, row_ids, st);
            if (rc) return rc;
        }
    }
    if (mem == VDB_MEM_HOST && staged) {
        const char* r = w->host_io + io_q;
        std::memcpy(out_scores, r, (size_t)B * k * 4);
        std::memcpy(out_indices, r + (size_t)B * k * 4, (size_t)B * k * 8);
        if (out_keys) std::memcpy(out_keys, r + (size_t)B * k * 12, (size_t)B * k * 8);
    } else if (mem == VDB_MEM_HOST) {
        HIP_TRY(hipMemcpyAsync(out_scores, out_s, (size_t)B * k * 4, hipMemcpyDeviceToHost, st));
        HIP_TRY(hipMemcpyAsync(out_indices, out_i, (size_t)B * k * 8, hipMemcpyDeviceToHost, st));
        if (out_keys) HIP_TRY(hipMemcpyAsync(out_keys, out_k, (size_t)B * k * 8, hipMemcpyDeviceToHost, st));
        HIP_TRY(hipStreamSynchronize(st));
    }
    return VDB_OK;
}

int32_t vdb_shutdown(void) {
    std::vector<vdb_index*> live;
    {
        std::lock_guard<std::mutex> rg(g_reg_mu);
        live.assign(g_indices.begin(), g_indices.end());
    }
    std::set<int> devices;
    for (vdb_index* ix : live) {
        HIP_TRY(hipSetDevice(ix->device));
        devices.insert(ix->device);
        {
            const int wr = wait_idle(ix);
            if (wr) return wr;
        }
        const int frc = flush_all_timing(ix);
        if (frc) return frc;
        std::lock_guard<std::mutex> g(ix->ws_mu);
        for (Workspace* w : ix->pool)
            if (!w->busy) free_workspace_memory(w);
    }
    for (int d : devices) {
        HIP_TRY(hipSetDevice(d));
        hipMemPool_t pool = nullptr;
        if (hipDeviceGetDefaultMemPool(&pool, d) == hipSuccess && pool) (void)hipMemPoolTrimTo(pool, 0);
    }
    return VDB_OK;
}

int32_t vdb_index_search_rows(vdb_index* ix, const float* queries, int32_t B, int32_t k, const int64_t* list_offsets,
                              int32_t n_lists, const int64_t* list_rows, int64_t n_ids, const int32_t* query_list,
                              int32_t mem, float* out_scores, int64_t* out_indices, double* out_keys,
                              int64_t index_offset, void* stream) {
    if (!ix) return set_error(VDB_ERR_INVALID, "index is NULL");
    if (B == 0) return VDB_OK;
    if (B < 0) return set_error(VDB_ERR_INVALID, "n_queries must be >= 0, got %d", B);
    if (k <= 0 || k > 1024) return set_error(VDB_ERR_INVALID, "k must be in [1, 1024], got %d", k);
    if (!queries || !out_scores || !out_indices) return set_error(VDB_ERR_INVALID, "NULL query/output pointer");
    if (mem != VDB_MEM_HOST && mem != VDB_MEM_DEVICE) return set_error(VDB_ERR_INVALID, "bad mem kind %d", mem);
    if (n_lists < 0 || n_ids < 0) return set_error(VDB_ERR_INVALID, "n_lists and n_ids must be >= 0");
    if (!list_offsets || (n_ids > 0 && !list_rows)) return set_error(VDB_ERR_INVALID, "NULL list pointer");
    if (!query_list && n_lists != B)
        return set_error(VDB_ERR_INVALID, "without a query_list n_lists (%d) must equal n_queries (%d)", n_lists, B);
    const int D = ix->dim;
    if (mem == VDB_MEM_HOST && !all_finite(queries, (int64_t)B * D))
        return set_error(VDB_ERR_NONFINITE, "query contains NaN or Inf");
    HIP_TRY(hipSetDevice(ix->device));
    std::shared_lock<std::shared_mutex> g(ix->mu);
    const int64_t N = ix->count;
    if (mem == VDB_MEM_HOST) {
        int64_t at = 0;
        switch (subset_validate(list_offsets, n_lists, list_rows, n_ids, query_list, B, N, &at)) {
            case kSubsetOk: break;
            case kSubsetBadOffsets:
                return set_error(VDB_ERR_INVALID, "list_offsets[%lld] = %lld: offsets must ascend from >= 0 to <= n_ids (%lld)",
                                 (long long)at, (long long)list_offsets[at], (long long)n_ids);
            case kSubsetBadId:
                return set_error(VDB_ERR_INVALID, "list_rows[%lld] = %lld is outside [0, %lld)", (long long)at,
                                 (long long)list_rows[at], (long long)N);
            case kSubsetUnsorted:
                return set_error(VDB_ERR_INVALID, "list_rows[%lld] = %lld: a list must be strictly ascending", (long long)at,
                                 (long long)list_rows[at]);
            case kSubsetBadQueryList:
                return set_error(VDB_ERR_INVALID, "query_list[%lld] = %d is outside [0, %d)", (long long)at,
                                 query_list[at], n_lists);
            default:
                return set_error(VDB_ERR_INVALID, "without a query_list n_lists must equal n_queries");
        }
    }
    SearchLease lease(ix, mem, stream);
    if (lease.rc) return lease.rc;
    Workspace* const w = lease.w;
    const hipStream_t st = lease.st;

    const bool host = mem == VDB_MEM_HOST;
    const int KE = subset_ke(k);
    const int n_seg = N > 0 ? subset_n_seg(ix->subset_wgs, n_ids, B, n_lists, ix->n_cu) : 1;
    const SubsetScratch sc = subset_scratch(B, D, k, n_seg, n_lists, n_ids, host, query_list != nullptr, out_keys != nullptr);
    int rc = ws_reserve(w, (size_t)sc.total, st);
    if (rc) return rc;
    char* dev = w->dev;
    SubsetArgs a{};
    a.Q = queries;
    a.offs = list_offsets;
    a.rows = list_rows;
    a.qlist = query_list;
    a.out_s = out_scores;
    a.out_i = out_indices;
    a.out_k = out_keys;
    if (host) {
        rc = stage_up(w, sc.in0, sc.in_bytes, sc.out_bytes, st, [&](char* h) {
            std::memcpy(h + (sc.q - sc.in0), queries, (size_t)B * D * 4);
            std::memcpy(h + (sc.offs - sc.in0), list_offsets, ((size_t)n_lists + 1) * 8);
            if (n_ids > 0) std::memcpy(h + (sc.rows - sc.in0), list_rows, (size_t)n_ids * 8);
            if (query_list) std::memcpy(h + (sc.qlist - sc.in0), query_list, (size_t)B * 4);
        });
        if (rc) return rc;
        a.Q = reinterpret_cast<const float*>(dev + sc.q);
        a.offs = reinterpret_cast<const int64_t*>(dev + sc.offs);
        a.rows = reinterpret_cast<const int64_t*>(dev + sc.rows);
        a.qlist = query_list ? reinterpret_cast<const int32_t*>(dev + sc.qlist) : nullptr;
        a.out_s = reinterpret_cast<float*>(dev + sc.out_s);
        a.out_i = reinterpret_cast<int64_t*>(dev + sc.out_i);
        a.out_k = out_keys ? reinterpret_cast<double*>(dev + sc.out_k) : nullptr;
    }
    if (N == 0) {
        HIP_TRY(launch_empty_results((int64_t)B * k, a.out_s, a.out_i, a.out_k, st));
    } else {
        double* qn64 = reinterpret_cast<double*>(dev + sc.qn64);
        int* done = reinterpret_cast<int*>(dev + sc.done);
        HIP_TRY(launch_prep_queries(a.Q, B, B, D, ix->G, ix->metric, nullptr, nullptr, qn64, nullptr, nullptr, nullptr,
                                    nullptr, done, st));
        a.qn64 = qn64;
        a.X = ix->X;
        a.G = ix->G;
        a.D = D;
        a.nrm64 = ix->nrm64;
        a.count = N;
        a.n_lists = n_lists;
        a.n_ids = n_ids;
        a.k = k;
// ... 844 lines not shown
```

### mlx-vector-db_amd/csrc/vdb_ingest.hip

```cpp
#include "vdb_common.h"
#include "vdb_internal.h"
#include "vdb_row_ops.h"

namespace vdb {

__global__ void __launch_bounds__(256) pack_rows_kernel(const float* __restrict__ src, int64_t n, int D, int G,
                                                        float* __restrict__ X, int64_t row0,
                                                        double* __restrict__ nrm64, float* __restrict__ inv32,
                                                        float* __restrict__ sq32, float* __restrict__ rinit32,
                                                        int normalise, unsigned long long* __restrict__ xmax_bits,
                                                        int* __restrict__ nonfinite) {
    const int lane = threadIdx.x & 63;
    const int64_t row = (int64_t)blockIdx.x * 4 + (threadIdx.x >> 6);
    if (row >= n) return;
    pack_row(src + row * (int64_t)D, (uint64_t)(row0 + row), lane, D, G, X, nrm64, inv32, sq32, rinit32, normalise,
             xmax_bits, nonfinite);
}

hipError_t launch_pack_rows(const float* src, int64_t n, int D, int G, float* X, int64_t row0, double* nrm64,
                            float* inv32, float* sq32, float* rinit32, int normalise, unsigned long long* xmax_bits,
                            int* nonfinite, hipStream_t st) {
    if (n <= 0) return hipSuccess;
    const int64_t blocks = (n + 3) / 4;
    hipLaunchKernelGGL(pack_rows_kernel, dim3((unsigned)blocks), dim3(256), 0, st, src, n, D, G, X, row0, nrm64,
                       inv32, sq32, rinit32, normalise, xmax_bits, nonfinite);
    return hipGetLastError();
}

__global__ void __launch_bounds__(256) dir_sum_kernel(const float* __restrict__ X, const float* __restrict__ inv32,
                                                      int64_t row0, int64_t n, int D, int G,
                                                      double* __restrict__ sums) {
    const int64_t r0 = (int64_t)blockIdx.x * 64;
    const int64_t r1 = r0 + 64 < n ? r0 + 64 : n;
    for (int d = threadIdx.x; d < D; d += 256) {
        double acc = 0.0;
        for (int64_t i = r0; i < r1; ++i) {
            const uint64_t r = (uint64_t)(row0 + i);
            const float x = X[row_piece_offset(r, d >> 2, G) + (d & 3)];
            acc += (double)(inv32 ? x * inv32[r] : x);
        }
        atomicAdd(sums + d, acc);
    }
}

hipError_t launch_dir_sum(const float* X, const float* inv32, int64_t row0, int64_t n, int D, int G, double* sums,
                          hipStream_t st) {
    if (n <= 0) return hipSuccess;
    hipLaunchKernelGGL(dir_sum_kernel, dim3((unsigned)((n + 63) / 64)), dim3(256), 0, st, X, inv32, row0, n, D, G,
                       sums);
    return hipGetLastError();
}

__global__ void __launch_bounds__(256) resid_dir_kernel(const float* __restrict__ X, const float* __restrict__ inv32,
                                                        int64_t row0, int64_t n, int D, int G,
                                                        const float* __restrict__ dir,
                                                        unsigned long long* __restrict__ out) {
    const int lane = threadIdx.x & 63;
    const int64_t i = (int64_t)blockIdx.x * 4 + (threadIdx.x >> 6);
    if (i >= n) return;
    resid_dir_row(X, inv32, (uint64_t)(row0 + i), lane, D, G, dir, out);
}

hipError_t launch_resid_dir(const float* X, const float* inv32, int64_t row0, int64_t n, int D, int G,
                            const float* dir, unsigned long long* out, hipStream_t st) {
    if (n <= 0) return hipSuccess;
    hipLaunchKernelGGL(resid_dir_kernel, dim3((unsigned)((n + 3) / 4)), dim3(256), 0, st, X, inv32, row0, n, D, G, dir,
                       out);
    return hipGetLastError();
}

__global__ void __launch_bounds__(256) split_rows_kernel(const float* __restrict__ X, int G, int64_t t0,
                                                         int64_t n_tiles, const float* __restrict__ inv32,
                                                         float* __restrict__ Xs) {
    const int64_t idx = (int64_t)blockIdx.x * 256 + threadIdx.x;
    if (idx >= n_tiles * G * 32) return;
    const int i = (int)(idx & 31);
    const int g8 = (int)((idx >> 5) % G);
    const uint64_t t = (uint64_t)(t0 + (idx >> 5) / G);
    split_row_piece(X, G, t * 32 + i, g8, inv32, Xs);
}

hipError_t launch_split_rows(const float* X, int G, int64_t row0, int64_t n, const float* inv32, float* Xs,
                             hipStream_t st) {
    if (n <= 0) return hipSuccess;
    const int64_t t0 = row0 >> 5, t1 = (row0 + n + 31) >> 5;
    const int64_t total = (t1 - t0) * G * 32;
    hipLaunchKernelGGL(split_rows_kernel, dim3((unsigned)((total + 255) / 256)), dim3(256), 0, st, X, G, t0, t1 - t0,
                       inv32, Xs);
    return hipGetLastError();
}

__global__ void __launch_bounds__(256) tile_rows_kernel(const float* __restrict__ X, int G, int64_t t0,
                                                        int64_t n_tiles, float* __restrict__ Xt) {
    const int64_t idx = (int64_t)blockIdx.x * 256 + threadIdx.x;
    if (idx >= n_tiles * 2 * G * 32) return;
    const int i = (int)(idx & 31);
    const int p = (int)((idx >> 5) % (2 * G));
    const uint64_t r = (uint64_t)(t0 + (idx >> 5) / (2 * G)) * 32 + i;
    tile_row_piece(X, G, r, p, Xt);
}

hipError_t launch_tile_rows(const float* X, int G, int64_t row0, int64_t n, float* Xt, hipStream_t st) {
    if (n <= 0) return hipSuccess;
    const int64_t t0 = row0 >> 5, t1 = (row0 + n + 31) >> 5;
    const int64_t total = (t1 - t0) * 2 * G * 32;
    hipLaunchKernelGGL(tile_rows_kernel, dim3((unsigned)((total + 255) / 256)), dim3(256), 0, st, X, G, t0, t1 - t0,
                       Xt);
    return hipGetLastError();
}

__global__ void __launch_bounds__(256) unpack_rows_kernel(const float* __restrict__ X, int G, int D, int64_t row0,
                                                          int64_t n, float* __restrict__ dst) {
    const int64_t row = (int64_t)blockIdx.x * 4 + (threadIdx.x >> 6);
    if (row >= n) return;
    const int lane = threadIdx.x & 63;
    for (int d = lane; d < D; d += 64) dst[row * D + d] = X[(size_t)(row0 + row) * (size_t)(8 * G) + d];
}

hipError_t launch_unpack_rows(const float* X, int G, int D, int64_t row0, int64_t n, float* dst, hipStream_t st) {
    if (n <= 0) return hipSuccess;
    hipLaunchKernelGGL(unpack_rows_kernel, dim3((unsigned)((n + 3) / 4)), dim3(256), 0, st, X, G, D, row0, n, dst);
    return hipGetLastError();
}

__global__ void __launch_bounds__(256) prep_queries_kernel(const float* __restrict__ Q, int B, int Bp, int D, int G,
                                                           int metric, float* __restrict__ Qt, float* __restrict__ Qs,
                                                           double* __restrict__ qn64, int* __restrict__ flag_count,
                                                           uint32_t* __restrict__ gthr,
                                                           uint32_t* __restrict__ gslots, uint32_t* __restrict__ gl_cnt,
                                                           int* __restrict__ done, float* __restrict__ qmax,
                                                           const float* __restrict__ mu,
                                                           const float* __restrict__ dir,
                                                           double* __restrict__ qconst) {
    const int lane = threadIdx.x & 63;
    const int b = blockIdx.x * 4 + (threadIdx.x >> 6);
    if (b == 0 && lane == 0 && flag_count) {
        flag_count[0] = 0;
        flag_count[B + 1] = 0;
        flag_count[B + 2] = 0;
    }
    if (b >= Bp) return;
    if (lane == 0 && gthr) gthr[b] = 0u;
    if (lane == 0 && gl_cnt) gl_cnt[b] = 0u;
    if (lane == 0 && done) done[b] = 0;
    if (gslots)
        for (int j = lane; j < KP_MAX + PILOT_SLOTS; j += 64)
            gslots[j < KP_MAX ? (size_t)b * KP_MAX + j : (size_t)Bp * KP_MAX + pslot_at(b, j - KP_MAX, B)] = 0u;
    const int Dp = G * GROUP_DIMS;
    const int np = (D + 255) / 256;
    const bool real = b < B;
    const float* q = Q + (int64_t)(real ? b : 0) * D;
    double acc = 0.0;
    for (int m = 0; m < np; ++m) {
#pragma unroll
        for (int j = 0; j < 4; ++j) {
            const int d = 4 * (m * 64 + lane) + j;
            const double v = (real && d < D) ? (double)q[d] : 0.0;
            acc = acc + v * v;
        }
    }
    acc = wave_sum_butterfly(acc);
    const double nq = sqrt(acc);
    if (lane == 0) qn64[b] = nq;
    const float scale = metric == 0 ? (float)(1.0 / fmax(nq, 1e-8)) : 1.0f;
    if (qconst) {
        const double qs = metric == 0 ? 1.0 / fmax(nq, 1e-8) : 1.0;
        double mq = 0.0, c = 0.0, q2 = 0.0, d2 = 0.0;
        for (int m = 0; m < np; ++m) {
            const int d0 = 4 * (m * 64 + lane);
            f32x4 qv = {0.f, 0.f, 0.f, 0.f}, mv = {0.f, 0.f, 0.f, 0.f}, dv = {0.f, 0.f, 0.f, 0.f};
            if (d0 < Dp) {
#pragma unroll
                for (int j = 0; j < 4; ++j) qv[j] = (real && d0 + j < D) ? q[d0 + j] : 0.0f;
                if (mu) mv = *(const f32x4*)(mu + d0);
                if (dir) dv = *(const f32x4*)(dir + d0);
            }
#pragma unroll
            for (int j = 0; j < 4; ++j) {
                const double x = (double)qv[j] * qs;
                mq += x * (double)mv[j];
                c += x * (double)dv[j];
                q2 += x * x;
                d2 += (double)dv[j] * (double)dv[j];
            }
        }
        mq = wave_sum_butterfly(mq);
        c = wave_sum_butterfly(c);
        q2 = wave_sum_butterfly(q2);
        d2 = wave_sum_butterfly(d2);
        if (lane == 0) {
            qconst[3 * (size_t)b] = mu ? mq : 0.0;
            qconst[3 * (size_t)b + 1] = dir ? c : 0.0;
            qconst[3 * (size_t)b + 2] = dir ? fmax(q2 - 2.0 * c * c + c * c * d2, 0.0) : 0.0;
        }
    }
    if (qmax && real) {
        float m = 0.0f;
        for (int d = lane; d < D; d += 64) m = fmaxf(m, fabsf(q[d] * scale));
#pragma unroll
        for (int off = 32; off >= 1; off >>= 1) m = fmaxf(m, __shfl_xor(m, off, 64));
        if (lane == 0) qmax[b] = m;
    }
    if (Qt) {
        const int GQ = G + QG_EXTRA;
        for (int p = lane; 4 * p < Dp + 8 * QG_EXTRA; p += 64) {
            const int ps = 4 * p < Dp ? p : p - 2 * G;
            f32x4 v;
#pragma unroll
            for (int j = 0; j < 4; ++j) {
                const int d = 4 * ps + j;
                v[j] = (real && d < D) ? q[d] * scale : 0.0f;
            }
            *(f32x4*)(Qt + tiled_piece_offset((uint64_t)b, p, GQ)) = v;
        }
    }
    if (Qs) {
        const int G16 = G >> 1, GQ16 = G16 + QG_EXTRA;
        for (int h8 = lane; h8 < 2 * GQ16; h8 += 64) {
            const int g16 = h8 >> 1, h = h8 & 1;
            const int d0 = 16 * (g16 % G16) + 8 * h;
            f32x4 a, c;
#pragma unroll
            for (int j = 0; j < 4; ++j) {
                a[j] = (real && d0 + j < D) ? q[d0 + j] * scale : 0.0f;
                c[j] = (real && d0 + 4 + j < D) ? q[d0 + 4 + j] * scale : 0.0f;
            }
            f32x4 hi, lo;
            split8(a, c, hi, lo);
            float* dst = Qs + split_block((uint64_t)(b >> 5), g16, GQ16) + (size_t)((b & 31) + 32 * h) * 4;
            *(f32x4*)dst = hi;
            *(f32x4*)(dst + 4 * BLOCK_FLOATS) = lo;
        }
    }
}

hipError_t launch_prep_queries(const float* Q, int B, int Bp, int D, int G, int metric, float* Qt, float* Qs,
                               double* qn64, int* flag_count, uint32_t* gthr, uint32_t* gslots, uint32_t* gl_cnt,
                               int* done, hipStream_t st, float* qmax, const float* mu, const float* dir,
                               double* qconst) {
    hipLaunchKernelGGL(prep_queries_kernel, dim3((Bp + 3) / 4), dim3(256), 0, st, Q, B, Bp, D, G, metric, Qt, Qs,
                       qn64, flag_count, gthr, gslots, gl_cnt, done, qmax, mu, dir, qconst);
    return hipGetLastError();
}
}
```

### mlx-vector-db_amd/csrc/vdb_internal.h

```cpp
#pragma once
#include <hip/hip_runtime.h>
#include <stdint.h>

#include "vdb_search_plan.h"

namespace vdb {

constexpr int TILE_ROWS = 32;
constexpr int GROUP_DIMS = 8;
constexpr int BLOCK_FLOATS = 256;
constexpr int ROW_ALIGN = 1024;

struct Int8Consts {
    float sx;
    double zmax_h, xl_max, rmax_half;
};
hipError_t launch_zmax(const float* X, const float* inv32, const float* mu, int64_t row0, int64_t n, int D, int G,
                       uint32_t* out, hipStream_t st);
hipError_t launch_quant_rows(const float* X, const float* inv32, const float* mu, const float* dir, float sx,
                             int64_t row0, int64_t n, int G, float* Xq, unsigned long long* stats, hipStream_t st, int8_t* xh_rm = nullptr);
hipError_t launch_prep8(const float* Q, const double* qn64, const float* qmax, int B, int Bp, int D, int G8,
                        int metric, int prec, const Int8Consts& c, float* Qq, float* lsl, float* qerr, float* qscal,
                        hipStream_t st, float* qres = nullptr, float* qerr2 = nullptr);
hipError_t launch_colsum8(const float* Xq, int64_t row0, int64_t n, int G8, uint32_t* csum, hipStream_t st);
hipError_t launch_rstart8(const float* rinit, int64_t N, const float* qscal, int* rs, uint32_t* sum, hipStream_t st);
hipError_t launch_sink_row8(float* Xq, int64_t row, int G8, hipStream_t st);
hipError_t launch_pilot8(int prec, int metric, const float* Xq, const float* rinit, const uint32_t* mask,
                         const float* Qq, const float* qscal, int G8, int64_t N, int B, int n_qblocks, int QB,
                         int n_sample, uint32_t* pslots, hipStream_t st, const uint32_t* csum = nullptr,
                         uint32_t* chke = nullptr, bool wide = false);
int scan8_rows_per_step(int prec, int metric);
bool scan8w_ok(int G8, int B);
bool scan8wl_ok(int prec, int metric, int G8, int B);
hipError_t launch_scan8wl(int prec, int metric, const float* Xq, const uint32_t* mask, const float* Qq,
                          const float* lsl, const float* qscal, int G8, int64_t N, int B, int n_seg, float* gl_s,
                          uint32_t* gl_i, int64_t gl_cap, uint32_t* seg_cnt, const uint32_t* gthr, uint32_t* chkp,
                          hipStream_t st);
hipError_t launch_scan8w(int prec, int metric, const float* Xq, const int* rs8, const uint32_t* mask, const float* Qq,
                         const float* lsl, const float* qscal, int G8, int64_t N, int B, int Bp, int n_seg,
                         float* gl_s, uint32_t* gl_i, int64_t gl_cap, uint32_t* seg_cnt, const uint32_t* gthr,
                         uint32_t* chkp, int chk_ld, int chk_l, hipStream_t st);
hipError_t launch_scan8(int prec, int metric, int KP, const float* Xq, const float* rinit, const uint32_t* mask,
                        const float* Qq, const float* lsl, const float* qscal, int G8, int64_t N, int B,
                        int n_qblocks, int64_t n_steps, int n_wg, int spw, float* gl_s, uint32_t* gl_i,
                        uint32_t* gl_cnt, int64_t gl_cap, uint32_t* gthr,
                        int lockstep, int qlds, hipStream_t st, const int* gate = nullptr,
                        uint32_t* chkp = nullptr, int chk_ld = 0, int chk_l = 0);

hipError_t launch_pack_rows(const float* src, int64_t n, int D, int G, float* X, int64_t row0,
                            double* nrm64, float* inv32, float* sq32, float* rinit32, int normalise,
                            unsigned long long* xmax_bits, int* nonfinite, hipStream_t st);

hipError_t launch_dir_sum(const float* X, const float* inv32, int64_t row0, int64_t n, int D, int G, double* sums,
                          hipStream_t st);
hipError_t launch_resid_dir(const float* X, const float* inv32, int64_t row0, int64_t n, int D, int G,
                            const float* dir, unsigned long long* out, hipStream_t st);
hipError_t launch_split_rows(const float* X, int G, int64_t row0, int64_t n, const float* inv32, float* Xs,
                             hipStream_t st);

hipError_t launch_tile_rows(const float* X, int G, int64_t row0, int64_t n, float* Xt, hipStream_t st);

size_t remove_scan_bytes(int64_t n_words);
hipError_t launch_remove_scan(const uint32_t* mask, int64_t n_words, int64_t count, uint32_t* base, uint32_t* part,
                              uint32_t* info, hipStream_t st);
struct RemoveRows {
    float* X; int Dp; double* nrm64; float* inv32; float* sq32; float* rinit32;
};
struct RemoveScratch {
    float* X; double* nrm64; float* inv32; float* sq32; float* rinit32;
};
hipError_t launch_remove_chunk(const RemoveRows& a, const uint32_t* mask, const uint32_t* base, int64_t count,
                               int64_t w0, int64_t w1, const RemoveScratch& s, hipStream_t st);
hipError_t launch_zero_rows8(float* Xq, int64_t row0, int64_t n, int G8, hipStream_t st);

hipError_t launch_update_validate(const int64_t* ids, const float* src, int64_t n, int D, int64_t count,
                                  uint32_t* bitmap, uint32_t* flags, hipStream_t st);
hipError_t launch_update_pack_rows(const float* src, const int64_t* ids, int64_t n, int64_t count, int D, int G,
                                   float* X, double* nrm64, float* inv32, float* sq32, float* rinit32, int normalise,
                                   unsigned long long* xmax_bits, int* nonfinite, hipStream_t st);
hipError_t launch_update_resid_dir(const float* X, const float* inv32, const int64_t* ids, int64_t n, int64_t count,
                                   int D, int G, const float* dir, unsigned long long* out, hipStream_t st);
hipError_t launch_update_split_rows(const float* X, int G, const int64_t* ids, int64_t n, int64_t count,
                                    const float* inv32, float* Xs, hipStream_t st);
hipError_t launch_update_tile_rows(const float* X, int G, const int64_t* ids, int64_t n, int64_t count, float* Xt,
                                   hipStream_t st);
hipError_t launch_update_quant_rows(const float* X, const float* inv32, const float* mu, const float* dir, float sx,
                                    const int64_t* ids, int64_t n, int64_t count, int G, float* Xq,
                                    unsigned long long* stats, int8_t* xh_rm, hipStream_t st);
hipError_t launch_update_colsum8(const float* Xq, const int64_t* ids, int64_t n, int64_t count, int G8, int sign,
                                 uint32_t* csum, hipStream_t st);

hipError_t launch_unpack_rows(const float* X, int G, int D, int64_t row0, int64_t n, float* dst, hipStream_t st);

__host__ __device__ inline size_t pslot_at(int q, int slot, int B) { return (size_t)slot * B + q; }
hipError_t launch_prep_queries(const float* Q, int B, int Bp, int D, int G, int metric,
                               float* Qt, float* Qs, double* qn64, int* flag_count, uint32_t* gthr,
                               uint32_t* gslots, uint32_t* gl_cnt, int* done, hipStream_t st,
                               float* qmax = nullptr, const float* mu = nullptr, const float* dir = nullptr,
                               double* qconst = nullptr);

int scan_rows_per_step(int prec, int variant);
int scan_wgs_per_cu(int prec, int variant, int KP);
bool scan_variant_ok(int prec, int variant, int G);
hipError_t launch_scan_topk(int prec, int metric, int KP, int variant, const float* X, const float* rowscale,
                            const uint32_t* mask, const float* Qt, int G, int64_t N, int B, int n_qblocks, int64_t n_steps,
                            int n_wg, int steps_per_wg, float* gl_s, uint32_t* gl_i, uint32_t* gl_cnt, int64_t gl_cap,
                            uint32_t* gthr, uint32_t* gslots, int lockstep, hipStream_t st);

bool scan_priv(int prec, int variant, int KP);
int scan_priv_capw();
hipError_t launch_scan_topk_priv(int prec, int metric, int KP, const float* X, const float* rowscale,
                                 const uint32_t* mask, const float* Qt, int G, int64_t N, int B, int n_qblocks,
                                 int64_t n_steps, int n_wg, int spw, float* gl_s, uint32_t* gl_i, uint32_t* gl_cnt,
                                 int64_t gl_cap, uint32_t* gthr, uint32_t* gslots, hipStream_t st);
hipError_t launch_select_topk(const float* gl_s, const uint32_t* gl_i, const uint32_t* gl_cnt, int64_t gl_cap, int KP,
                              int B, float* out_s, uint32_t* out_i, hipStream_t st);

hipError_t launch_pilot(int prec, int metric, int KP, const float* X, const float* rowscale, const uint32_t* mask,
                        const float* Qt, int G, int64_t N, int B, int n_qblocks, int QB, int n_sample,
                        uint32_t* pslots, uint32_t* gthr, hipStream_t st);

hipError_t launch_pilot_bound(uint32_t* pslots, int B, int KP, uint32_t* gthr, hipStream_t st);

int scan2_rows_per_step(bool q4 = false);
int scan2_qb(int KP);
hipError_t launch_scan2(int prec, int metric, int KP, const float* Xs, const float* rinit, const uint32_t* mask,
                        const float* Qs, int G, int64_t N, int B, int n_qblocks, int64_t n_steps, int n_wg, int spw,
                        float* gl_s, uint32_t* gl_i, uint32_t* gl_cnt, int64_t gl_cap, uint32_t* gthr,
                        int lockstep, hipStream_t st, bool q4 = false, int qlds = -1, const int* gate = nullptr);
hipError_t launch_pilot2(int prec, int metric, int KP, const float* Xs, const float* rinit, const uint32_t* mask,
                         const float* Qs, int G, int64_t N, int B, int n_qblocks, int QB, int n_sample,
                         uint32_t* pslots, uint32_t* gthr, hipStream_t st);

hipError_t launch_merge_f32(int KP, const float* ls, const uint32_t* li, int n_lists, int B,
                            float* out_s, uint32_t* out_i, hipStream_t st);

struct RerankArgs {
    const float* Q; const double* qn64; const float* X; int G; int D;
    const double* nrm64; const float* app_s; const uint32_t* app_i;
    int k; double eps_rel; double xmax;
    float* out_s; int64_t* out_i; double* out_k; int64_t index_offset;
    int* flag_count; int* flag_list;
    const uint32_t* gthr;
};
hipError_t launch_rerank(int metric, int KP, const RerankArgs& a, int B, hipStream_t st);

struct FinishArgs {
    int small = 0;
    const float* gl_s; const uint32_t* gl_i; const uint32_t* gl_cnt; int64_t gl_cap;
    const float* Q; const double* qn64; const float* X; int G; int D; const double* nrm64;
    int k; double eps_rel; double xmax;
    double xres;
    const float* dir = nullptr;
    double dres = 0.0;
    const float* qerr = nullptr;
    const float* mu = nullptr;
    const double* qconst = nullptr;
    float* out_s; int64_t* out_i; double* out_k; int64_t index_offset;
    int* flag_count; int* flag_list; const uint32_t* gthr;
    int* overflow_count;
    int* incons_count = nullptr;
    const int* gate = nullptr;
    const int8_t* xh_rm = nullptr;
    const float* qres = nullptr;
    const float* qerr2 = nullptr;
    const float* qscal = nullptr;
    float sx = 0.0f;
    int Dp = 0;
    const int64_t* row_ids = nullptr;
    int split = 1;
    double* sx_ek = nullptr; uint32_t* sx_ck = nullptr; uint32_t* sx_cr = nullptr; int* sx_n = nullptr;
    int* done = nullptr;
    const uint32_t* chkp = nullptr;
    const uint32_t* chke = nullptr;
    const uint32_t* chkr = nullptr;
    const float* chk_q = nullptr;
    const uint32_t* chk_csum = nullptr;
    int chk_nw = 0, chk_ld = 0, chk_g8 = 0;
    bool chk_l = false;
    const uint32_t* seg_cnt = nullptr;
    int seg_n = 0;
};
hipError_t launch_finish(int metric, int KP, const FinishArgs& a, int B, hipStream_t st);

struct ExactTail {
    int* done; double* mk; uint32_t* mi; int k; int64_t index_offset;
    float* out_s; int64_t* out_i; double* out_k; const int64_t* row_ids;
    unsigned long long* host_totals = nullptr;
};
hipError_t launch_exact_scan(int metric, int KE, const float* Q, const double* qn64, const int* qlist, int nq,
                             const float* X, int G, int D, const double* nrm64, const uint32_t* mask,
                             int64_t N, int n_wg, int64_t rows_per_wg,
                             double* lk, uint32_t* li, hipStream_t st, const int* qcount = nullptr,
                             const int* ovf = nullptr, unsigned long long* totals = nullptr,
                             const ExactTail* tail = nullptr, int gate_slots = 4, char* gscr = nullptr);
size_t exact_scan_scratch_bytes(int KE, int n_wg, int slots);

struct SubsetArgs {
    const float* Q; const double* qn64; const float* X; int G; int D; const double* nrm64; int64_t count;
    const int64_t* offs; int n_lists; const int64_t* rows; int64_t n_ids; const int32_t* qlist;
    int k; int KE;
    double* lk; uint32_t* li; double* mk; uint32_t* mi; int* done;
    unsigned long long* bad;
    float* out_s; int64_t* out_i; double* out_k; int64_t index_offset;
};
size_t subset_lds_bytes(int KE, int n_seg);
hipError_t launch_subset_search(int metric, const SubsetArgs& a, int n_queries, int n_seg, hipStream_t st);

struct RangeArgs {
    const float* Q; const double* thr; const double* qn64; const float* X; int G; int D; const double* nrm64;
    int64_t N; const uint32_t* mask;
    uint32_t* H; uint32_t* part; int64_t* cnt;
    int64_t cap; int64_t* out_c; int64_t* out_i; float* out_s; double* out_k; int64_t index_offset;
};
hipError_t launch_range_block(int metric, const RangeArgs& a, int b0, int qb, hipStream_t st);

hipError_t launch_group_valid(const int32_t* groups, int64_t n, uint32_t* bitmap, int64_t n_words,
                              unsigned long long* n_valid, hipStream_t st);
hipError_t launch_group_and(const uint32_t* a, const uint32_t* b, uint32_t* out, int64_t n_words,
                            unsigned long long* n_set, hipStream_t st);
struct GroupSelectArgs {
    const float* fs; const int64_t* fi; const double* fk; int k_fetch;
    const int32_t* groups; int64_t count; int k; int force;
    int64_t eligible; const unsigned long long* eligible_dev;
    int* need; unsigned long long* fallback_total;
    float* out_s; int64_t* out_i; int32_t* out_g; double* out_k; int64_t index_offset;
};
hipError_t launch_group_select(const GroupSelectArgs& a, int n_queries, hipStream_t st);
struct GroupExactArgs {
    const float* Q; const double* qn64; const float* X; int G; int D; const double* nrm64; int64_t N;
    const uint32_t* mask; const int32_t* groups; const int* need; int k;
    double* lk; uint32_t* lr; int32_t* lg; int* done;
    float* out_s; int64_t* out_i; int32_t* out_g; double* out_k; int64_t index_offset;
};
size_t group_exact_lds_bytes(int k);
hipError_t launch_group_exact(int metric, const GroupExactArgs& a, int n_queries, int n_seg, hipStream_t st);

hipError_t launch_merge_f64_u32(int KP, const double* lk, const uint32_t* li, int n_lists, int Lk,
                                int64_t sq, int64_t sj, int nq, double* out_k, uint32_t* out_i, hipStream_t st,
                                const int* qcount = nullptr);
hipError_t launch_merge_f64_i64(int KP, const double* lk, const int64_t* li, int n_lists, int Lk,
                                int64_t sq, int64_t sj, int nq, double* out_k, int64_t* out_i, hipStream_t st);

hipError_t launch_finalize_u32(int metric, const double* sk, const uint32_t* si, int KP, int nq, const int* qmap,
                               int k, int64_t index_offset, float* out_s, int64_t* out_i, double* out_k,
                               hipStream_t st, const int* qcount = nullptr, const int64_t* row_ids = nullptr);
hipError_t launch_finalize_i64(int metric, const double* sk, const int64_t* si, int KP, int nq, const int* qmap,
                               int k, float* out_s, int64_t* out_i, double* out_k, hipStream_t st);
hipError_t launch_gather_rows(const float* Q, int D, const int* list, int n, float* out, hipStream_t st);
hipError_t launch_repass_gather(const float* Q, int D, const int* flags, int R, float* out, int* counts,
                                unsigned long long* totals, hipStream_t st);
hipError_t launch_scatter_results(const int* list, int n, int k, const float* ss, const int64_t* si, const double* sk,
                                  float* os, int64_t* oi, double* ok, hipStream_t st, const int* n_dev = nullptr);
hipError_t launch_empty_results(int64_t n, float* out_s, int64_t* out_i, double* out_k, hipStream_t st);

struct GraphSearchArgs {
    const float* rows; int Dp; int D; const float* rowscale; int64_t n_rows;
    const int32_t* nbr; int R; const int32_t* entries; int n_entries;
    const float* Q; int k; int ef;
    int64_t* out_lab; float* out_dist; unsigned long long* stats;
    int teams = 1;
    int64_t* tmp_lab = nullptr; float* tmp_dist = nullptr;
};
hipError_t launch_graph_search(int metric, const GraphSearchArgs& a, int nq, hipStream_t st);


struct GraphPruneArgs {
    const float* X; int G; const float* rowscale;
    const int32_t* cand; int cw; int64_t n_nodes; int limit; int rw; int fill;
    int32_t* out_nbr; float* out_dist;
    const int32_t* nodes = nullptr; int sort = 0;
};
hipError_t launch_graph_scatter(int32_t* nbr, int R, const int32_t* ids, const int32_t* rows, int64_t n,
                                hipStream_t st);
hipError_t launch_graph_prune(int metric, const GraphPruneArgs& a, hipStream_t st);

hipError_t launch_similarity_matrix(const float* X, int64_t N, int D, const float* Q, int B, int metric,
                                    float* out, hipStream_t st);
hipError_t launch_normalize_rows(const float* in, int64_t n, int D, float* out, hipStream_t st);
size_t topk_workspace_bytes(int64_t n, int rows, int k);
hipError_t launch_topk_scores(const float* S, int rows, int64_t n, int k, int largest, int64_t* out_idx,
                              float* out_val, void* ws, hipStream_t st);

}
```

### mlx-vector-db_amd/csrc/vdb_scan8wl.hip

```cpp
#include "vdb_scan8_kernel.h"

namespace vdb {

template <bool NT>
__device__ __forceinline__ void w8l_glds(const void* gsrc, uint32_t lds) {
    uint32_t keep;
    if constexpr (NT)
        asm volatile("s_mov_b32 %0, m0\n\ts_mov_b32 m0, %2\n\ts_nop 0\n\tglobal_load_lds_dwordx4 %1, off nt\n\ts_mov_b32 m0, %0"
                     : "=&s"(keep) : "v"(gsrc), "s"(lds) : "memory");
    else
        asm volatile("s_mov_b32 %0, m0\n\ts_mov_b32 m0, %2\n\ts_nop 0\n\tglobal_load_lds_dwordx4 %1, off\n\ts_mov_b32 m0, %0"
                     : "=&s"(keep) : "v"(gsrc), "s"(lds) : "memory");
}

__device__ __forceinline__ void w8l_ds_read(f32x4& x, uint32_t addr) {
    asm volatile("ds_read_b128 %0, %1" : "=v"(x) : "v"(addr));
}

constexpr int W8L_NW = 8;
constexpr int W8L_QB = W8L_NW * 32;
#ifndef VDB_W8L_PD
#define VDB_W8L_PD 4
#endif
constexpr int W8L_PD = VDB_W8L_PD;
#ifndef VDB_W8L_SMAX
#define VDB_W8L_SMAX 4
#endif
constexpr int W8L_SMAX = VDB_W8L_SMAX;

template <int RL>
__host__ __device__ constexpr int w8l_cnt_bytes() { return RL > 1 ? 2 * W8L_QB * 4 : 0; }
template <int G, int RL>
__host__ __device__ constexpr int w8l_nslot() {
    return ((160 * 1024 - w8l_cnt_bytes<RL>()) / (G * 1024) < W8L_SMAX ? (160 * 1024 - w8l_cnt_bytes<RL>()) / (G * 1024)
                                                                        : W8L_SMAX) / RL * RL;
}
template <int G, int RL>
__host__ __device__ constexpr size_t w8l_lds_bytes() { return (size_t)w8l_nslot<G, RL>() * G * 1024 + w8l_cnt_bytes<RL>(); }
template <int N>
__device__ __forceinline__ void w8l_wait_bar() { asm volatile("s_waitcnt vmcnt(%0) lgkmcnt(0)\n\ts_barrier" ::"n"(N) : "memory"); }

template <int G, int RL, bool NT>
__global__ void __launch_bounds__(64 * W8L_NW, 1)
scan8wl_kernel(const float* __restrict__ Xq, const uint32_t* __restrict__ mask, const float* __restrict__ Qq,
               const float* __restrict__ lsl, const float* __restrict__ qscal, int64_t N, int B,
               float* __restrict__ gl_s, uint32_t* __restrict__ gl_i, int64_t gl_cap, uint32_t* __restrict__ seg_cnt,
               const uint32_t* __restrict__ gthr, uint32_t* __restrict__ chkp) {
    constexpr int NW = W8L_NW, NSLOT = w8l_nslot<G, RL>(), P = NSLOT / RL - 1;
    constexpr size_t TILE_B = (size_t)G * 1024;
    constexpr size_t GSTEP = 8 * BLOCK_FLOATS;
    constexpr int LPW = RL * G / NW;
    static_assert((RL * G) % NW == 0, "a round's blocks spread evenly over the waves");
    static_assert(P >= 1 && (P - 1) * LPW <= 63, "ring / vmcnt range");
    extern __shared__ __attribute__((aligned(16))) char s_dyn[];
    int* s_seg = (int*)(s_dyn + NSLOT * TILE_B);
    uint32_t* s_ck = (uint32_t*)(s_seg + W8L_QB);

    const int lane = threadIdx.x & 63;
    const int wv = __builtin_amdgcn_readfirstlane(threadIdx.x >> 6);
    const int w = blockIdx.x, n_seg = gridDim.x;
    const int qtn = (B + 31) >> 5;
    const int qtile = wv % qtn, rl = wv / qtn;
    const int q0 = qtile * 32;
    const bool active = rl < RL;
    const int64_t T = (N + 31) >> 5;
    const int my_tiles = T > w ? (int)((T - 1 - w) / n_seg + 1) : 0;
    const int n_rounds = (my_tiles + RL - 1) / RL;
    const uint32_t ring = (uint32_t)(uintptr_t)(const __attribute__((address_space(3))) char*)s_dyn;

    if constexpr (RL > 1) {
        for (int i = threadIdx.x; i < W8L_QB; i += 64 * NW) {
            s_seg[i] = 0;
            s_ck[i] = 0u;
        }
    }
    int cnt = 0;

    auto issue = [&](int R) {
        const int rs = (R % (NSLOT / RL)) * RL;
#pragma unroll
        for (int u = 0; u < LPW; ++u) {
            const int j = wv * LPW + u;
            const int i = j / G, g = j % G;
            const int m = R * RL + i;
            if (RL == 1 || m < my_tiles)
                w8l_glds<NT>(Xq + corpus_block((uint64_t)m * n_seg + w, g, 0, G) + lane * 4,
                             ring + (uint32_t)((rs + i) * TILE_B) + (uint32_t)(g * 1024));
        }
    };

    const float uH = qscal[0], invU = qscal[2];
    f32x4 qr[G];
    const int q = q0 + (lane & 31);
    const bool qok = active && q < B;
    const float thf = qok ? key_to_float(gthr[q]) : INFINITY;
    const int thc = qok ? h_floor(thf, lsl[q], invU) : INT_MAX;
    uint32_t ckh = 0u;
    if (active) {
        const float* qs = Qq + s2_blk((uint64_t)qtile, 0, G + QG_EXTRA) + lane * 4;
#pragma unroll
        for (int g = 0; g < G; ++g) qr[g] = *(const f32x4*)(qs + g * GSTEP);
    }
#pragma unroll
    for (int p = 0; p < P; ++p)
        if (p < n_rounds) issue(p);

    for (int R = 0; R < n_rounds; ++R) {
        if (P > 1 && R + P - 1 < n_rounds && (R + P) * RL <= my_tiles)
            w8l_wait_bar<(P - 1) * LPW>();
        else
            w8l_wait_bar<0>();
        if (R + P < n_rounds) issue(R + P);
        const int m = R * RL + rl;
        if (!active || m >= my_tiles) continue;
        const int64_t t = (int64_t)m * n_seg + w;
        i32x16 aH;
#pragma unroll
        for (int v = 0; v < 16; ++v) aH[v] = 0;
        constexpr int PD = W8L_PD, NB = PD + 1;
        const uint32_t sa = ring + (uint32_t)(((R % (NSLOT / RL)) * RL + rl) * TILE_B) + (uint32_t)lane * 16u;
        f32x4 xb[NB];
#pragma unroll
        for (int p = 0; p < PD; ++p) w8l_ds_read(xb[p], sa + (uint32_t)(p * 1024));
#pragma unroll
        for (int g = 0; g < G; ++g) {
            if (g < G - PD)
                asm volatile("s_waitcnt lgkmcnt(%1)" : "+v"(xb[g % NB]) : "n"(PD - 1));
            else if (g == G - PD)
                asm volatile("s_waitcnt lgkmcnt(0)" : "+v"(xb[g % NB]));
            if (g < G - PD) w8l_ds_read(xb[(g + PD) % NB], sa + (uint32_t)((g + PD) * 1024));
            aH = __builtin_amdgcn_mfma_i32_32x32x32_i8(__builtin_bit_cast(i32x4, xb[g % NB]),
                                                       __builtin_bit_cast(i32x4, qr[g]), aH, 0, 0, 0);
        }
        const bool hit = __builtin_amdgcn_ballot_w64(imax16(aH) > thc) != 0ull;
        if (chkp) {
            if ((t + 1) * 32 <= N) {
                ckh += hsum16(aH);
            } else {
#pragma unroll
                for (int v = 0; v < 16; ++v) {
                    const int64_t row = t * 32 + 8 * (v >> 2) + 4 * (lane >> 5) + (v & 3);
                    if (row < N) ckh += (uint32_t)aH[v];
                }
            }
        }
        if (hit) {
            const uint32_t cand = qok ? tile_valid16(mask, t, N, lane) : 0u;
            float sv[16];
            uint32_t pm = 0;
#pragma unroll
            for (int v = 0; v < 16; ++v) {
                sv[v] = (float)aH[v] * uH;
                pm |= (sv[v] > thf ? 1u : 0u) << v;
            }
            pm &= cand;
            int pos = 0;
            if constexpr (RL == 1) {
                const int np = __builtin_popcount(pm);
                const int np_hi = __shfl_xor(np, 32, 64);
                pos = cnt + (lane >= 32 ? np_hi : 0);
                cnt += np + np_hi;
            } else {
                if (pm != 0u) pos = atomicAdd(&s_seg[q], __builtin_popcount(pm));
            }
            const uint32_t rb = (uint32_t)(t * 32) + 4u * (uint32_t)(lane >> 5);
            float* ls = gl_s + (size_t)q * gl_cap + (size_t)w * W8_CH;
            uint32_t* li = gl_i + (size_t)q * gl_cap + (size_t)w * W8_CH;
            while (pm != 0u) {
                const int v = __builtin_ctz(pm);
                pm &= pm - 1u;
                float a_ = sv[0];
#pragma unroll
                for (int u = 1; u < 16; ++u) a_ = v == u ? sv[u] : a_;
                if (pos < W8_CH) {
                    ls[pos] = a_;
                    li[pos] = rb + (uint32_t)((v & 3) + 8 * (v >> 2));
                }
                ++pos;
            }
        }
    }
    asm volatile("s_waitcnt vmcnt(0)" ::: "memory");
    if constexpr (RL == 1) {
        if (!active) return;
        if (lane < 32 && q < B) seg_cnt[(size_t)q * n_seg + w] = (uint32_t)cnt;
        if (chkp) {
            const uint32_t hsum = ckh + (uint32_t)__shfl_xor((int)ckh, 32, 64);
            if (lane < 32 && q < B) chkp[(size_t)q * n_seg + w] = hsum;
        }
        return;
    }
    if (active && chkp) {
        const uint32_t hsum = ckh + (uint32_t)__shfl_xor((int)ckh, 32, 64);
        if (lane < 32) atomicAdd(&s_ck[q], hsum);
    }
    __syncthreads();
    for (int i = threadIdx.x; i < B; i += 64 * NW) {
        seg_cnt[(size_t)i * n_seg + w] = (uint32_t)s_seg[i];
        if (chkp) chkp[(size_t)i * n_seg + w] = s_ck[i];
    }
}

constexpr int W8L1_SMAX = 6;

template <int G>
__host__ __device__ constexpr int w8l1_nslot() {
    return (160 * 1024 - W8L_QB * 4) / (G * 1024) < W8L1_SMAX ? (160 * 1024 - W8L_QB * 4) / (G * 1024) : W8L1_SMAX;
}
template <int N>
__device__ __forceinline__ void w8l1_wait_bar() { asm volatile("s_waitcnt vmcnt(%0) lgkmcnt(0)\n\ts_barrier" ::"n"(N) : "memory"); }
template <int G>
__host__ __device__ constexpr size_t w8l1_lds_bytes() { return (size_t)w8l1_nslot<G>() * G * 1024 + (size_t)W8L_QB * 4; }

template <int G, bool NT>
__global__ void __launch_bounds__(64 * W8L_NW, 1)
scan8wl1_kernel(const float* __restrict__ Xq, const uint32_t* __restrict__ mask, const float* __restrict__ Qq,
               const float* __restrict__ lsl, const float* __restrict__ qscal, int64_t N, int B, float* __restrict__ gl_s, uint32_t* __restrict__ gl_i,
               int64_t gl_cap, uint32_t* __restrict__ seg_cnt, const uint32_t* __restrict__ gthr,
               uint32_t* __restrict__ chkp) {
    constexpr int NW = W8L_NW, NSLOT = w8l1_nslot<G>();
    constexpr size_t TILE_B = (size_t)G * 1024;
    constexpr size_t GSTEP = 8 * BLOCK_FLOATS;
    constexpr int LPW = G / NW;
    static_assert(G % NW == 0, "a tile's blocks spread evenly over the waves");
    extern __shared__ __attribute__((aligned(16))) char s_dyn[];
    int* s_seg = (int*)(s_dyn + NSLOT * TILE_B);

    const int lane = threadIdx.x & 63;
    const int wv = __builtin_amdgcn_readfirstlane(threadIdx.x >> 6);
    const int w = blockIdx.x, n_seg = gridDim.x;
    const int q0 = wv * 32;
    const bool active = q0 < B;
    const int64_t T = (N + 31) >> 5;
    const int64_t my_tiles = T > w ? (T - 1 - w) / n_seg + 1 : 0;
    const uint32_t ring = (uint32_t)(uintptr_t)(const __attribute__((address_space(3))) char*)s_dyn;

    if (lane < 32) s_seg[wv * 32 + lane] = 0;

    auto issue = [&](int64_t m) {
        const uint32_t sbase = ring + (uint32_t)((m % NSLOT) * TILE_B);
        const int64_t t = m * n_seg + w;
#pragma unroll
        for (int u = 0; u < LPW; ++u) {
            const int g = wv * LPW + u;
            w8l_glds<NT>(Xq + corpus_block((uint64_t)t, g, 0, G) + lane * 4, sbase + (uint32_t)(g * 1024));
        }
    };

    const float uH = qscal[0], invU = qscal[2];
    f32x4 qr[G];
    const int q = q0 + (lane & 31);
    const bool qok = active && q < B;
    const float thf = qok ? key_to_float(gthr[q]) : INFINITY;
    const int thc = qok ? h_floor(thf, lsl[q], invU) : INT_MAX;
    uint32_t ckh = 0u;
    if (active) {
        const float* qs = Qq + s2_blk((uint64_t)(q0 / 32), 0, G + QG_EXTRA) + lane * 4;
#pragma unroll
        for (int g = 0; g < G; ++g) qr[g] = *(const f32x4*)(qs + g * GSTEP);
    }
#pragma unroll
    for (int p = 0; p < NSLOT - 1; ++p)
        if (p < my_tiles) issue(p);

    for (int64_t m = 0; m < my_tiles; ++m) {
        static_assert(NSLOT >= 2 && NSLOT <= 6 && (NSLOT - 2) * LPW <= 63, "vmcnt range");
        switch ((int)min<int64_t>(NSLOT - 2, my_tiles - 1 - m)) {
            case 4: w8l1_wait_bar<4 * LPW>(); break;
            case 3: w8l1_wait_bar<3 * LPW>(); break;
            case 2: w8l1_wait_bar<2 * LPW>(); break;
            case 1: w8l1_wait_bar<LPW>(); break;
            default: w8l1_wait_bar<0>(); break;
        }
        if (m + NSLOT - 1 < my_tiles) issue(m + NSLOT - 1);
        if (!active) continue;
        const int64_t t = m * n_seg + w;
        i32x16 aH;
#pragma unroll
        for (int v = 0; v < 16; ++v) aH[v] = 0;
        constexpr int PD = W8L_PD, NB = PD + 1;
        const uint32_t sa = ring + (uint32_t)((m % NSLOT) * TILE_B) + (uint32_t)lane * 16u;
        f32x4 xb[NB];
#pragma unroll
        for (int p = 0; p < PD; ++p) w8l_ds_read(xb[p], sa + (uint32_t)(p * 1024));
#pragma unroll
        for (int g = 0; g < G; ++g) {
            if (g < G - PD)
                asm volatile("s_waitcnt lgkmcnt(%1)" : "+v"(xb[g % NB]) : "n"(PD - 1));
            else if (g == G - PD)
                asm volatile("s_waitcnt lgkmcnt(0)" : "+v"(xb[g % NB]));
            if (g < G - PD) w8l_ds_read(xb[(g + PD) % NB], sa + (uint32_t)((g + PD) * 1024));
            aH = __builtin_amdgcn_mfma_i32_32x32x32_i8(__builtin_bit_cast(i32x4, xb[g % NB]),
                                                       __builtin_bit_cast(i32x4, qr[g]), aH, 0, 0, 0);
        }
        const bool hit = __builtin_amdgcn_ballot_w64(imax16(aH) > thc) != 0ull;
        if (chkp) {
            if ((t + 1) * 32 <= N) {
                ckh += hsum16(aH);
            } else {
#pragma unroll
                for (int v = 0; v < 16; ++v) {
                    const int64_t row = t * 32 + 8 * (v >> 2) + 4 * (lane >> 5) + (v & 3);
                    if (row < N) ckh += (uint32_t)aH[v];
                }
            }
        }
        if (hit) {
            const int ql = lane & 31;
            const uint32_t cand = qok ? tile_valid16(mask, t, N, lane) : 0u;
            float sv[16];
            uint32_t pm = 0;
#pragma unroll
            for (int v = 0; v < 16; ++v) {
                sv[v] = (float)aH[v] * uH;
                pm |= (sv[v] > thf ? 1u : 0u) << v;
            }
            pm &= cand;
            int pos = 0;
            if (pm != 0u) pos = atomicAdd(&s_seg[wv * 32 + ql], __builtin_popcount(pm));
            const uint32_t rb = (uint32_t)(t * 32) + 4u * (uint32_t)(lane >> 5);
            float* ls = gl_s + (size_t)q * gl_cap + (size_t)w * W8_CH;
            uint32_t* li = gl_i + (size_t)q * gl_cap + (size_t)w * W8_CH;
            while (pm != 0u) {
                const int v = __builtin_ctz(pm);
                pm &= pm - 1u;
                float a_ = sv[0];
#pragma unroll
                for (int u = 1; u < 16; ++u) a_ = v == u ? sv[u] : a_;
                if (pos < W8_CH) {
                    ls[pos] = a_;
                    li[pos] = rb + (uint32_t)((v & 3) + 8 * (v >> 2));
                }
                ++pos;
            }
        }
    }
    asm volatile("s_waitcnt vmcnt(0)" ::: "memory");
    if (!active) return;
    if (lane < 32 && q < B) seg_cnt[(size_t)q * n_seg + w] = (uint32_t)s_seg[wv * 32 + lane];
    if (chkp) {
        const uint32_t hsum = ckh + (uint32_t)__shfl_xor((int)ckh, 32, 64);
        if (lane < 32 && q < B) chkp[(size_t)q * n_seg + w] = hsum;
    }
}

bool scan8wl_ok(int prec, int metric, int G8, int B) {
    return prec == PREC_I8 && metric == 0 && B >= 1 && B <= W8L_QB && (G8 == 16 || G8 == 24 || G8 == 32 || G8 == 48);
}

template <int G, int RL, bool NT>
static hipError_t scan8wl_launch(const float* Xq, const uint32_t* mask, const float* Qq, const float* lsl,
                                 const float* qscal, int64_t N, int B, int n_seg, float* gl_s, uint32_t* gl_i,
                                 int64_t gl_cap, uint32_t* seg_cnt, const uint32_t* gthr, uint32_t* chkp,
                                 hipStream_t st) {
    auto k = RL == 1 ? scan8wl1_kernel<G, NT> : scan8wl_kernel<G, RL, NT>;
    constexpr size_t lds = RL == 1 ? w8l1_lds_bytes<G>() : w8l_lds_bytes<G, RL>();
    static_assert(lds <= 160 * 1024, "LDS");
    static std::atomic<bool> lds_set{false};
    if (!lds_set.load()) {
        const hipError_t e = hipFuncSetAttribute((const void*)k, hipFuncAttributeMaxDynamicSharedMemorySize, (int)lds);
        if (e != hipSuccess) return e;
        lds_set = true;
    }
    hipLaunchKernelGGL(k, dim3((unsigned)n_seg), dim3(64 * W8L_NW), lds, st, Xq, mask, Qq, lsl, qscal, N, B, gl_s, gl_i,
                       gl_cap, seg_cnt, gthr, chkp);
    return hipGetLastError();
}

int scan8wl_rl(int G8, int B) {
#ifdef VDB_W8L_RL1
    return 1;
#else
    return (B + 31) / 32 <= W8L_NW / 2 && G8 <= 32 ? 2 : 1;
#endif
}

hipError_t launch_scan8wl(int prec, int metric, const float* Xq, const uint32_t* mask, const float* Qq,
                          const float* lsl, const float* qscal, int G8, int64_t N, int B, int n_seg, float* gl_s,
                          uint32_t* gl_i, int64_t gl_cap, uint32_t* seg_cnt, const uint32_t* gthr, uint32_t* chkp,
                          hipStream_t st) {
    if (!scan8wl_ok(prec, metric, G8, B) || n_seg <= 0 || gl_cap != (int64_t)n_seg * W8_CH) return hipErrorInvalidValue;
    const int rl = scan8wl_rl(G8, B);
#define W8L_CASE(GV, RLV)                                                                                          \
    if (G8 == GV && rl == RLV)                                                                                     \
        return scan8wl_launch<GV, RLV, true>(Xq, mask, Qq, lsl, qscal, N, B, n_seg, gl_s, gl_i, gl_cap, seg_cnt, gthr, \
                                             chkp, st);
    W8L_CASE(16, 1) W8L_CASE(24, 1) W8L_CASE(32, 1) W8L_CASE(48, 1)
    W8L_CASE(16, 2) W8L_CASE(24, 2) W8L_CASE(32, 2)
#undef W8L_CASE
    return hipErrorInvalidValue;
}

}
```

### mlx-vector-db_amd/csrc/vdb_search_plan.h

```cpp
#pragma once
#include <stdint.h>

#include <algorithm>
#include <cmath>

namespace vdb {

constexpr int PREC_FP32 = 0;
constexpr int PREC_BF16X3 = 1;
constexpr int PREC_BF16 = 2;
constexpr int PREC_I8 = 3;
constexpr int PREC_I8X3 = 4;
constexpr int PREC_I8Q = 5;
constexpr int N_PREC = 6;
inline bool prec_is_i8(int p) { return p == PREC_I8 || p == PREC_I8X3 || p == PREC_I8Q; }

constexpr int QG_EXTRA = 8;
constexpr int W8_CH = 32;
constexpr int KP_MAX = 256;
constexpr int PILOT_SLOTS = 256;
constexpr int kMaxApproxK = 200;
constexpr int kRepassDev = 16;
constexpr int64_t kI8NarrowRows = 512 * 1024;
constexpr int64_t kI8NarrowRowsShort = 4 * 1024 * 1024;
constexpr int64_t kWideMinRows = 65536;
constexpr int64_t kWideSplitMaxRows = 2500000;
constexpr int FIN_SEG_MAX = 512;
constexpr int64_t kRefineMinDp = 512;
constexpr int kGateSlots = 4;

inline int64_t plan_round_up(int64_t a, int64_t b) { return (a + b - 1) / b * b; }
inline int plan_next_pow2(int v) {
    int p = 1;
    while (p < v) p <<= 1;
    return p;
}
inline int64_t plan_align(int64_t b) { return (b + 255) / 256 * 256; }

struct SearchShape {
    int B, k;
    int D, Dp, G;
    int metric;
    int64_t N;
    int n_cu;
    int prec;
    bool host;
    bool gated;
    bool repass;
};
struct SearchKnobs {
    bool force_exact;
    int64_t margin;
    bool i8_narrow;
    int64_t scan_q4, scan_wide;
    int64_t n_wg_override;
    int64_t scan_variant;
    int64_t scan_sync;
    int64_t finish_split;
    int64_t i8_refine;
    int64_t scan_checksum;
    int64_t pilot_tiles;
    int64_t pilot_rank_override;
    bool has_xh;
    bool has_csum;
};
struct SearchKernelFacts {
    bool scan8wl_ok;
    bool scan8w_ok;
    bool scan_variant_ok;
    int rows_per_step;
    int rows_per_step_q4;
    bool scan_priv;
};

inline int search_groups(int prec, int G) { return prec == PREC_FP32 ? G : prec_is_i8(prec) ? G / 4 : G / 2; }

struct SearchKP {
    int KP;
    bool exact_all;
};
inline SearchKP search_kp(const SearchShape& s, const SearchKnobs& kn) {
    const int k = s.k, prec = s.prec;
    const bool one_plane = prec == PREC_BF16 || prec == PREC_I8;
    int margin_def = std::max(16, k / 4);
    if ((prec == PREC_BF16X3 || prec == PREC_I8X3) && s.D >= 1024) margin_def = std::max(margin_def, 48);
    if (one_plane) margin_def = std::max(16, std::min(std::max(112, k / 2), 256 - k));
    const bool i8_narrow = kn.i8_narrow && (s.N <= kI8NarrowRows || (s.Dp <= 128 && s.N <= kI8NarrowRowsShort));
    if (prec == PREC_I8) margin_def = std::max(16, (i8_narrow ? 128 : 256) - k);
    if (prec == PREC_I8Q) margin_def = std::max(16, 256 - k);
    if (s.repass) margin_def = std::max(margin_def, 128 - k);
    const int margin = kn.margin >= 0 ? (int)kn.margin : margin_def;
    SearchKP r;
    r.KP = std::max(32, plan_next_pow2(k + margin));
    r.exact_all = kn.force_exact || k > kMaxApproxK || r.KP > 256;
    if (r.KP > 256) r.KP = 256;
    return r;
}

struct SearchGeometry {
    int Gs;
    bool i8_pass, split_pass;
    bool q4;
    bool wide_long;
    bool wide8;
    int n_seg8;
    int QB, QB_pilot;
    int Bp;
    int n_qblocks;
    int variant;
    int64_t step_rows, n_steps;
    int n_wg, spw;
    int64_t mask_words;
    int lockstep;
    int n_wg8;
    int64_t gl_cap;
    bool priv;
    bool rs8_on;
    bool i8_refine;
    bool chk, chk_l;
    int fin_split;
    int R_rep;
};
inline SearchGeometry search_geometry(const SearchShape& s, const SearchKnobs& kn, const SearchKP& kp,
                                      const SearchKernelFacts& f) {
    SearchGeometry g{};
    const int B = s.B, KP = kp.KP, prec = s.prec;
    const int64_t N = s.N;
    const bool exact_all = kp.exact_all;
    g.i8_pass = prec_is_i8(prec);
    g.Gs = search_groups(prec, s.G);
    g.split_pass = prec == PREC_BF16X3 || prec == PREC_BF16;
    g.q4 = g.split_pass && !exact_all && !s.gated && KP == 128 && B >= 256 && g.Gs <= 8 &&
           (kn.scan_q4 == 1 || (kn.scan_q4 < 0));
    const int64_t n_tiles_all = plan_round_up(N, 32) / 32;
    g.wide_long = g.i8_pass && !exact_all && !s.gated && f.scan8wl_ok && N > 0 &&
                  (kn.scan_wide == 1 || (kn.scan_wide < 0 && N >= kWideMinRows && (g.Gs <= 32 || B <= 16 || B > 96)));
    g.wide8 = g.wide_long ||
              (g.i8_pass && !exact_all && !s.gated && f.scan8w_ok && N > 0 &&
               (kn.scan_wide == 1 || (kn.scan_wide < 0 && N >= kWideMinRows && (B > 256 || N <= kWideSplitMaxRows))));
    g.n_seg8 = !g.wide8 ? 0
               : kn.n_wg_override > 0
                   ? (int)std::min<int64_t>(FIN_SEG_MAX, std::min<int64_t>(kn.n_wg_override, n_tiles_all))
                   : (int)std::min<int64_t>(FIN_SEG_MAX, plan_round_up(std::min<int64_t>(s.n_cu, n_tiles_all), 8));
    g.QB = g.q4 ? 128 : g.i8_pass ? 64 : KP == 256 ? 32 : 64;
    g.QB_pilot = g.i8_pass ? 64 : KP == 256 ? 32 : 64;
    g.Bp = (int)plan_round_up(B, 128);
    g.n_qblocks = (B + g.QB - 1) / g.QB;
    g.variant = g.split_pass || g.i8_pass ? 0 : (int)kn.scan_variant;
    if (!g.split_pass && !g.i8_pass && !f.scan_variant_ok) g.variant = 0;
    g.step_rows = g.q4 ? f.rows_per_step_q4 : f.rows_per_step;
    g.n_steps = std::max<int64_t>(1, plan_round_up(N, g.step_rows) / g.step_rows);
    const int target = kn.n_wg_override > 0 ? (int)kn.n_wg_override : std::max(1, s.n_cu / g.n_qblocks);
    g.spw = (int)std::max<int64_t>(1, (g.n_steps + target - 1) / target);
    g.n_wg = (int)((g.n_steps + g.spw - 1) / g.spw);
    g.mask_words = plan_round_up(N, 32) / 32;
    g.lockstep = kn.scan_sync == 0 ? (!g.i8_pass && s.Dp > 128) : kn.scan_sync == 1;
    g.fin_split = (int)kn.finish_split;
    g.rs8_on = g.i8_pass && !exact_all && s.metric == 1;
    g.i8_refine = prec == PREC_I8 && kn.has_xh &&
                  (kn.i8_refine == 1 || (kn.i8_refine == -1 && s.Dp >= kRefineMinDp));
    g.R_rep = std::min(B, kRepassDev);
    g.chk = g.i8_pass && !exact_all && kn.scan_checksum && kn.has_csum && N > 0;
    g.chk_l = g.chk && prec == PREC_I8X3 && kn.scan_checksum == 2;
    g.n_wg8 = g.wide8 ? g.n_seg8 : (g.n_wg + 7) / 8 * 8;
    g.priv = !exact_all && !g.split_pass && !g.i8_pass && f.scan_priv;
    g.gl_cap = exact_all ? 0 : g.wide8 ? (int64_t)g.n_seg8 * W8_CH : (int64_t)((g.n_wg + 7) / 8 * 8) * 512;
    return g;
}

struct SearchPilot {
    int n_pilot;
    int pilot_rank;
};
inline SearchPilot search_pilot(const SearchShape& s, const SearchKnobs& kn, const SearchKP& kp,
                                const SearchGeometry& g) {
    const int k = s.k, KP = kp.KP;
    const int64_t N = s.N;
    const bool cheap_pilot = g.i8_pass && g.Gs == 4;
    const int64_t pilot_cap = cheap_pilot ? std::max<int64_t>(4096, std::min<int64_t>(8192, N / (32 * 40))) : 4096;
    const int64_t pilot_def = std::min<int64_t>(
        pilot_cap, std::max<int64_t>((cheap_pilot ? 1024 : 512) * std::max(1, k / 12), N / (32 * 160)));
    SearchPilot p;
    p.n_pilot = s.gated ? 0
                        : (int)std::min<int64_t>(kn.pilot_tiles >= 0 ? kn.pilot_tiles : pilot_def,
                                                 plan_round_up(N, 32) / 32);
    p.pilot_rank = KP;
    if (p.n_pilot > 0) {
        const double S = (double)std::min<int64_t>((int64_t)p.n_pilot * 32, N);
        const double x = (double)k * S / (double)N;
        double term = std::exp(-x), cdf = term;
        int r = 1;
        while (1.0 - cdf >= 1e-6 && r < KP) {
            term *= x / r;
            cdf += term;
            ++r;
        }
        const int r_min = (int)std::ceil(2.0 * KP * S / (double)N);
        p.pilot_rank = std::min(std::max(r, r_min), KP);
    }
    if (kn.pilot_rank_override > 0) p.pilot_rank = (int)std::min<int64_t>(kn.pilot_rank_override, KP);
    return p;
}

constexpr int kFlagInts = 64;
struct SearchLayout {
    int64_t Qraw, maskd;
    int64_t Qt;
    int64_t qn64, qconst;
    int64_t os, oi, ok;
    int64_t flags;
    int64_t done;
    int64_t gthr, gslots;
    int64_t gl_s, gl_i, gl_cnt;
    int64_t fx_ek, fx_ck, fx_cr, fx_n;
    int64_t q8max, q8lsl, q8err, q8scal;
    int64_t q8res, q8err2;
    int64_t chkp, segc, chkr;
    int64_t rs8;
    int64_t chke;
    int64_t rep_q, rep_s, rep_i, rep_k;
    int64_t total;
};
inline SearchLayout search_layout(const SearchShape& s, const SearchGeometry& g, const SearchPilot& p) {
    SearchLayout l;
    const int64_t B = s.B, Bp = g.Bp, k = s.k, D = s.D, Dp = s.Dp;
    int64_t o = 0;
    auto take = [&](bool on, int64_t bytes) {
        if (!on) return (int64_t)-1;
        const int64_t at = o;
        o += plan_align(bytes);
        return at;
    };
    const bool fx = g.fin_split > 1, dev = !s.host;
    l.Qraw = take(true, B * D * 4);
    l.maskd = take(true, (g.mask_words + 64) * 4);
    l.Qt = take(true, Bp * (Dp + 16 * QG_EXTRA) * 4);
    l.qn64 = take(true, Bp * 8);
    l.qconst = take(true, Bp * 3 * 8);
    l.os = take(true, B * k * 4);
    l.oi = take(true, B * k * 8);
    l.ok = take(true, B * k * 8);
    l.flags = take(true, (B + kFlagInts) * 4);
    l.done = take(true, Bp * 4);
    l.gthr = take(true, Bp * 4);
    l.gslots = take(true, Bp * (KP_MAX + PILOT_SLOTS) * 4);
    l.gl_s = take(true, B * g.gl_cap * 4);
    l.gl_i = take(true, B * g.gl_cap * 4);
    l.gl_cnt = take(true, Bp * 4);
    l.fx_ek = take(fx, B * g.fin_split * KP_MAX * 8);
    l.fx_ck = take(fx, B * g.fin_split * KP_MAX * 4);
    l.fx_cr = take(fx, B * g.fin_split * KP_MAX * 4);
    l.fx_n = take(fx, B * g.fin_split * 4);
    l.q8max = take(true, Bp * 4);
    l.q8lsl = take(true, Bp * 4);
    l.q8err = take(true, Bp * 4);
    l.q8scal = take(true, 64 * 4);
    l.q8res = take(g.i8_refine, Bp * Dp * 4);
    l.q8err2 = take(g.i8_refine, Bp * 4);
    l.chkp = take(g.chk, 2 * (int64_t)g.n_wg8 * Bp * 4);
    l.segc = take(g.wide8, Bp * g.n_seg8 * 4);
    l.chkr = take(g.chk && s.metric == 1, 64 * 4);
    l.rs8 = take(g.rs8_on, plan_round_up(s.N, std::max<int64_t>(32, g.step_rows)) * 4);
    l.chke = take(g.chk && p.n_pilot > 0, 2 * Bp * 4);
    l.rep_q = take(dev, (int64_t)g.R_rep * D * 4);
    l.rep_s = take(dev, (int64_t)g.R_rep * k * 4);
    l.rep_i = take(dev, (int64_t)g.R_rep * k * 8);
    l.rep_k = take(dev, (int64_t)g.R_rep * k * 8);
    l.total = o;
    return l;
}

struct ExactPlan {
    int KE, n_wg;
    int64_t rpw;
    int slots;
    int n_wg_gate;
};
inline ExactPlan exact_plan(int64_t N, int n_cu, int nq, int k, bool gated) {
    ExactPlan e;
    e.KE = std::max(32, plan_next_pow2(k));
    const int64_t wg_target = gated ? std::max<int64_t>(1, n_cu) : std::max<int64_t>(1, 2 * (int64_t)n_cu);
    e.n_wg_gate = (int)std::min<int64_t>(wg_target, std::max<int64_t>(1, N / 256));
    e.rpw = std::max<int64_t>(1, (N + e.n_wg_gate - 1) / e.n_wg_gate);
    e.n_wg = (int)std::max<int64_t>(1, (N + e.rpw - 1) / e.rpw);
    e.slots = std::min(nq, kGateSlots);
    return e;
}
struct ExactLayout {
    int64_t lk, li;
    int64_t mk, mi;
    int64_t scr;
    int64_t total;
};
inline int64_t exact_list_bytes(int nq, int n_wg, int KE, int64_t scratch_bytes) {
    return (int64_t)nq * n_wg * KE * 12 + (int64_t)nq * KE * 12 + 4096 + scratch_bytes;
}
inline ExactLayout exact_layout(const ExactPlan& e, int nq, int64_t scratch_bytes) {
    ExactLayout l;
    const int64_t list_elems = (int64_t)nq * e.n_wg * e.KE;
    int64_t o = 0;
    auto take = [&](int64_t bytes) {
        const int64_t at = o;
        o += plan_align(bytes);
        return at;
    };
    l.lk = take(list_elems * 8);
    l.li = take(list_elems * 4);
    l.mk = take((int64_t)nq * e.KE * 8);
    l.mi = take((int64_t)nq * e.KE * 4);
    l.scr = scratch_bytes > 0 ? take(scratch_bytes) : -1;
    l.total = exact_list_bytes(nq, e.n_wg, e.KE, scratch_bytes);
    return l;
}
inline int64_t exact_gate_bytes(const ExactPlan& e, int nq, int64_t scratch_bytes_gate) {
    return exact_list_bytes(nq, e.n_wg_gate, e.KE, scratch_bytes_gate);
}

}
```

Before: 490,800 queries/s.

## Add dynamic atomic tile dealing to the wide-long int8 scan kernel

Adds an optional work-dealing scheme to the scan8wl kernel: workgroups claim chunks of corpus tiles from a global atomic counter, which prep_queries resets, instead of a fixed strided tile assignment. A per-workgroup LDS claim queue lets claims be prefetched ahead of the load ring, and the pipeline wait logic is rewritten around claim boundaries. The aim is to balance load when workgroups finish unevenly. Auto mode leaves dealing off for both RL variants, so by default the kernel uses static claims that follow the chunked-window order, with extra bookkeeping in the loop.

```diff
diff --git a/mlx-vector-db_amd/csrc/vdb_api.cpp b/mlx-vector-db_amd/csrc/vdb_api.cpp
--- a/mlx-vector-db_amd/csrc/vdb_api.cpp
+++ b/mlx-vector-db_amd/csrc/vdb_api.cpp
@@ -151,6 +151,9 @@
     std::atomic<int> last_i8q_b{0};
     int64_t scan_q4 = -1;
     int64_t scan_wide = -1;
+    int64_t scan_deal = -1;
+    int64_t scan_deal_ch = 0;
+    int64_t debug_deal_skip = 0;
     int64_t remove_chunk = 0;
     int64_t update_chunk = 0;
     std::atomic<int64_t> gen{0};
@@ -595,6 +598,8 @@
     kn.i8_narrow = i8_narrow;
     kn.scan_q4 = ix->scan_q4;
     kn.scan_wide = ix->scan_wide;
+    kn.scan_deal = ix->scan_deal;
+    kn.scan_deal_ch = ix->scan_deal_ch;
     kn.n_wg_override = ix->n_wg_override;
     kn.scan_variant = ix->scan_variant;
     kn.scan_sync = ix->scan_sync;
@@ -613,6 +618,7 @@
     const int Gs = search_groups(s.prec, s.G);
     if (prec_is_i8(s.prec)) {
         f.scan8wl_ok = scan8wl_ok(s.prec, s.metric, Gs, s.B);
+        f.scan8wl_rl = f.scan8wl_ok ? scan8wl_rl(Gs, s.B) : 0;
         f.scan8w_ok = scan8w_ok(Gs, s.B);
         f.rows_per_step = scan8_rows_per_step(s.prec, s.metric);
     } else if (s.prec == PREC_BF16X3 || s.prec == PREC_BF16) {
@@ -868,6 +874,13 @@
     } else if (n == "scan_wide") {
         if (value < -1 || value > 1) return set_error(VDB_ERR_INVALID, "scan_wide must be -1, 0 or 1");
         ix->scan_wide = value;
+    } else if (n == "scan_deal") {
+        if (value < -1 || value > 1) return set_error(VDB_ERR_INVALID, "scan_deal must be -1, 0 or 1");
+        ix->scan_deal = value;
+    } else if (n == "scan_deal_ch") {
+        if (value != 0 && value != 4 && value != 8 && value != 16)
+            return set_error(VDB_ERR_INVALID, "scan_deal_ch must be 0 (auto), 4, 8 or 16");
+        ix->scan_deal_ch = value;
     } else if (n == "scan_q4") {
         if (value < -1 || value > 1) return set_error(VDB_ERR_INVALID, "scan_q4 must be -1, 0 or 1");
         ix->scan_q4 = value;
@@ -906,6 +919,9 @@
         ix->device_repass = value;
     } else if (n.rfind("debug_", 0) == 0 && !debug_knobs_enabled()) {
         return set_error(VDB_ERR_INVALID, "'%s' is a test-only knob (set VDB_DEBUG_KNOBS=1)", name);
+    } else if (n == "debug_deal_skip") {
+        if (value < 0) return set_error(VDB_ERR_INVALID, "debug_deal_skip must be >= 0");
+        ix->debug_deal_skip = value;
     } else if (n == "debug_sink_row8") {
         HIP_TRY(hipSetDevice(ix->device));
         std::unique_lock<std::shared_mutex> g(ix->mu);
@@ -1731,7 +1747,7 @@
     } else {
         HIP_TRY(launch_prep_queries(Qd, B, Bp, D, ix->G, ix->metric, prec == PREC_FP32 ? Qt : nullptr,
                                     split_pass ? Qt : nullptr, qn64, flags, gthr, gslots, gl_cnt, done, st,
-                                    i8_pass ? q8max : nullptr, q_mu, q_dir, qconst));
+                                    i8_pass ? q8max : nullptr, q_mu, q_dir, qconst, (uint32_t*)at(lay.tctr)));
         if (i8_pass && !exact_all) {
             Int8Consts c8;
             c8.sx = ix->sx;
@@ -1783,10 +1799,13 @@
             if (timed) HIP_TRY(hipEventRecord(tev[0], st));
             if (q4) ix->n_q4++;
             if (wide8) ix->n_wide++;
-            if (wide_long)
+            if (wide_long) {
+                const int skip = g.deal ? (int)std::min<int64_t>(ix->debug_deal_skip, n_seg8 - 1) : 0;
                 HIP_TRY(launch_scan8wl(prec, ix->metric, Xscan, md, Qt, q8lsl, q8scal, Gs, N, B, n_seg8, gl_s, gl_i,
-                                       gl_cap, segc, gthr, chkp, st));
-            else if (wide8)
+                                       gl_cap, segc, gthr, chkp, g.deal ? (uint32_t*)at(lay.tctr) : nullptr, g.deal_ch,
+                                       g.deal_win, skip ? plan_deal_cap(true, g.deal_win, n_seg8, skip) : g.deal_cap,
+                                       skip, st));
+            } else if (wide8)
                 HIP_TRY(launch_scan8w(prec, ix->metric, Xscan, rs8, md, Qt, q8lsl, q8scal, Gs, N, B, Bp, n_seg8, gl_s, gl_i,
                                       gl_cap, segc, gthr, chkp, Bp, chk_l ? 1 : 0, st));
             else if (i8_pass)
diff --git a/mlx-vector-db_amd/csrc/vdb_ingest.hip b/mlx-vector-db_amd/csrc/vdb_ingest.hip
--- a/mlx-vector-db_amd/csrc/vdb_ingest.hip
+++ b/mlx-vector-db_amd/csrc/vdb_ingest.hip
@@ -131,9 +131,10 @@
                                                            int* __restrict__ done, float* __restrict__ qmax,
                                                            const float* __restrict__ mu,
                                                            const float* __restrict__ dir,
-                                                           double* __restrict__ qconst) {
+                                                           double* __restrict__ qconst, uint32_t* __restrict__ tctr) {
     const int lane = threadIdx.x & 63;
     const int b = blockIdx.x * 4 + (threadIdx.x >> 6);
+    if (b == 0 && lane == 0 && tctr) tctr[0] = 0u;
     if (b == 0 && lane == 0 && flag_count) {
         flag_count[0] = 0;
         flag_count[B + 1] = 0;
@@ -237,9 +238,9 @@
 hipError_t launch_prep_queries(const float* Q, int B, int Bp, int D, int G, int metric, float* Qt, float* Qs,
                                double* qn64, int* flag_count, uint32_t* gthr, uint32_t* gslots, uint32_t* gl_cnt,
                                int* done, hipStream_t st, float* qmax, const float* mu, const float* dir,
-                               double* qconst) {
+                               double* qconst, uint32_t* tctr) {
     hipLaunchKernelGGL(prep_queries_kernel, dim3((Bp + 3) / 4), dim3(256), 0, st, Q, B, Bp, D, G, metric, Qt, Qs,
-                       qn64, flag_count, gthr, gslots, gl_cnt, done, qmax, mu, dir, qconst);
-    return hipGetLastError();
-}
-}
+                       qn64, flag_count, gthr, gslots, gl_cnt, done, qmax, mu, dir, qconst, tctr);
+    return hipGetLastError();
+}
+}
diff --git a/mlx-vector-db_amd/csrc/vdb_internal.h b/mlx-vector-db_amd/csrc/vdb_internal.h
--- a/mlx-vector-db_amd/csrc/vdb_internal.h
+++ b/mlx-vector-db_amd/csrc/vdb_internal.h
@@ -32,10 +32,11 @@
 int scan8_rows_per_step(int prec, int metric);
 bool scan8w_ok(int G8, int B);
 bool scan8wl_ok(int prec, int metric, int G8, int B);
+int scan8wl_rl(int G8, int B);
 hipError_t launch_scan8wl(int prec, int metric, const float* Xq, const uint32_t* mask, const float* Qq,
                           const float* lsl, const float* qscal, int G8, int64_t N, int B, int n_seg, float* gl_s,
                           uint32_t* gl_i, int64_t gl_cap, uint32_t* seg_cnt, const uint32_t* gthr, uint32_t* chkp,
-                          hipStream_t st);
+                          uint32_t* tctr, int deal_ch, int deal_win, int deal_cap, int deal_skip, hipStream_t st);
 hipError_t launch_scan8w(int prec, int metric, const float* Xq, const int* rs8, const uint32_t* mask, const float* Qq,
                          const float* lsl, const float* qscal, int G8, int64_t N, int B, int Bp, int n_seg,
                          float* gl_s, uint32_t* gl_i, int64_t gl_cap, uint32_t* seg_cnt, const uint32_t* gthr,
@@ -97,7 +98,7 @@
                                float* Qt, float* Qs, double* qn64, int* flag_count, uint32_t* gthr,
                                uint32_t* gslots, uint32_t* gl_cnt, int* done, hipStream_t st,
                                float* qmax = nullptr, const float* mu = nullptr, const float* dir = nullptr,
-                               double* qconst = nullptr);
+                               double* qconst = nullptr, uint32_t* tctr = nullptr);
 
 int scan_rows_per_step(int prec, int variant);
 int scan_wgs_per_cu(int prec, int variant, int KP);
diff --git a/mlx-vector-db_amd/csrc/vdb_scan8wl.hip b/mlx-vector-db_amd/csrc/vdb_scan8wl.hip
--- a/mlx-vector-db_amd/csrc/vdb_scan8wl.hip
+++ b/mlx-vector-db_amd/csrc/vdb_scan8wl.hip
@@ -17,6 +17,134 @@
     asm volatile("ds_read_b128 %0, %1" : "=v"(x) : "v"(addr));
 }
 
+constexpr int W8L_CQ = 8;
+constexpr uint32_t W8L_END = 0xffffffffu;
+#ifdef VDB_DEAL_STAMP
+constexpr int W8L_ST_LAUNCH = 256, W8L_ST_WG = 512;
+static __device__ unsigned long long g_deal_stamps[W8L_ST_LAUNCH][W8L_ST_WG][4];
+#endif
+
+struct W8lDeal {
+    uint32_t* ctr;
+    int ch_log2;
+    int n_win;
+    int cap;
+    int skip;
+    int stamp;
+};
+
+template <int RL, int A>
+struct w8l_dealer {
+    static_assert(RL == 1 || RL == 2, "steps per claim are a power of two");
+    static_assert(A >= 1 && A <= 5, "first claims (<= 4)");
+    uint32_t* s_q;
+    uint32_t* ctr;
+    uint32_t T, n_seg, w, n_claims;
+    int spc_log2, ch_log2, cap, n_win;
+    int s_end, s_full;
+    uint32_t ib, sb;
+    uint32_t pval;
+    int c_made;
+    bool patom, stop;
+    int n_tiles;
+
+    __device__ __forceinline__ void init(uint32_t* q, const W8lDeal& d, int64_t T_, int n_seg_, int w_) {
+        s_q = q; ctr = d.ctr; T = (uint32_t)T_; n_seg = (uint32_t)n_seg_; w = (uint32_t)w_;
+        ch_log2 = d.ch_log2; spc_log2 = d.ch_log2 - (RL - 1); n_win = d.n_win; cap = d.cap;
+        n_claims = (uint32_t)d.n_win * n_seg;
+        s_end = INT_MAX; s_full = INT_MAX; ib = sb = W8L_END; pval = W8L_END; c_made = -1; patom = false; stop = false;
+        n_tiles = 0;
+    }
+    __device__ __forceinline__ uint32_t base_of(uint32_t p) const {
+        return p >= n_claims ? W8L_END : ((p / n_seg) << ch_log2) * n_seg + p % n_seg;
+    }
+    __device__ __forceinline__ uint32_t static_claim(int c) const {
+        return c < n_win ? (uint32_t)c * n_seg + w : W8L_END;
+    }
+    __device__ __forceinline__ void publish(int c, uint32_t p, int lane) {
+        if (p >= n_claims) stop = true;
+        if (lane == 0) s_q[c & (W8L_CQ - 1)] = base_of(p);
+    }
+    __device__ __forceinline__ void first_claims(int lane) {
+        const int npre = (A + 2 * (1 << spc_log2) - 1) >> spc_log2;
+        uint32_t p[4];
+#pragma unroll
+        for (int c = 0; c < 4; ++c) {
+            p[c] = W8L_END;
+            if (c < npre && c < cap) {
+                if (ctr) {
+                    if (lane == 0) p[c] = atomicAdd(ctr, 1u);
+                } else {
+                    p[c] = static_claim(c);
+                }
+            }
+        }
+#pragma unroll
+        for (int c = 0; c < 4; ++c)
+            if (c < npre) publish(c, (uint32_t)__builtin_amdgcn_readfirstlane((int)p[c]), lane);
+    }
+    __device__ __forceinline__ void turn(int s, int wv, uint32_t& got) {
+        const int spc = 1 << spc_log2;
+        int mk = 0;
+        if (wv == 0 && ((s + A) & (spc - 1)) == 0) {
+            const int c = ((s + A) >> spc_log2) + 1;
+            c_made = c;
+            patom = false;
+            pval = W8L_END;
+            if (!stop && c < cap) {
+                if (ctr) {
+                    patom = true;
+                    mk = 1;
+                } else {
+                    pval = static_claim(c);
+                }
+            }
+        }
+        uint64_t keep;
+        const uint32_t zero = 0u, one = 1u;
+        asm volatile("s_cmp_lg_u32 %5, 0\n\ts_cbranch_scc0 .Lw8l_nomake_%=\n\t"
+                     "s_mov_b64 %1, exec\n\ts_mov_b64 exec, 1\n\tglobal_atomic_add %0, %2, %3, %4 sc0\n\ts_mov_b64 exec, %1\n"
+                     ".Lw8l_nomake_%=:"
+                     : "+v"(got), "=&s"(keep) : "v"(zero), "v"(one), "s"(ctr), "s"(__builtin_amdgcn_readfirstlane(mk))
+                     : "memory", "scc");
+    }
+    __device__ __forceinline__ void turn_end(int wv, int lane, uint32_t& got) {
+        const int rd = wv == 0 && c_made >= 0 && patom ? 1 : 0;
+        uint32_t p = W8L_END;
+        asm volatile("s_cmp_eq_u32 %2, 0\n\ts_cbranch_scc1 .Lw8l_noread_%=\n\t"
+                     "s_waitcnt vmcnt(0)\n\tv_readfirstlane_b32 %1, %0\n"
+                     ".Lw8l_noread_%=:"
+                     : "+v"(got), "+s"(p) : "s"(__builtin_amdgcn_readfirstlane(rd)) : "memory", "scc");
+        if (wv != 0 || c_made < 0) return;
+        publish(c_made, patom ? p : pval, lane);
+        c_made = -1;
+    }
+    __device__ __forceinline__ void issue_claim(int si) {
+        if (si >= s_end || (si & ((1 << spc_log2) - 1)) != 0) return;
+        ib = (uint32_t)__builtin_amdgcn_readfirstlane((int)s_q[(si >> spc_log2) & (W8L_CQ - 1)]);
+        if (ib == W8L_END)
+            s_end = si;
+        else if (ib + (uint32_t)((1 << ch_log2) - 1) * n_seg >= T)
+            s_full = min(s_full, si);
+    }
+    __device__ __forceinline__ void score_claim(int s) {
+        if ((s & ((1 << spc_log2) - 1)) == 0)
+            sb = (uint32_t)__builtin_amdgcn_readfirstlane((int)s_q[(s >> spc_log2) & (W8L_CQ - 1)]);
+    }
+    __device__ __forceinline__ uint32_t tile(uint32_t b, int s, int i) const {
+        return b + (uint32_t)((s & ((1 << spc_log2) - 1)) * RL + i) * n_seg;
+    }
+};
+template <int N>
+__device__ __forceinline__ void w8l_wait_bar() { asm volatile("s_waitcnt vmcnt(%0) lgkmcnt(0)\n\ts_barrier" ::"n"(N) : "memory"); }
+
+__device__ __forceinline__ void w8l_skip_out(int B, int n_seg, int w, uint32_t* seg_cnt, uint32_t* chkp) {
+    for (int i = threadIdx.x; i < B; i += blockDim.x) {
+        seg_cnt[(size_t)i * n_seg + w] = 0u;
+        if (chkp) chkp[(size_t)i * n_seg + w] = 0u;
+    }
+}
+
 constexpr int W8L_NW = 8;
 constexpr int W8L_QB = W8L_NW * 32;
 #ifndef VDB_W8L_PD
@@ -29,7 +157,7 @@
 constexpr int W8L_SMAX = VDB_W8L_SMAX;
 
 template <int RL>
-__host__ __device__ constexpr int w8l_cnt_bytes() { return RL > 1 ? 2 * W8L_QB * 4 : 0; }
+__host__ __device__ constexpr int w8l_cnt_bytes() { return (RL > 1 ? 2 * W8L_QB * 4 : 0) + W8L_CQ * 4; }
 template <int G, int RL>
 __host__ __device__ constexpr int w8l_nslot() {
     return ((160 * 1024 - w8l_cnt_bytes<RL>()) / (G * 1024) < W8L_SMAX ? (160 * 1024 - w8l_cnt_bytes<RL>()) / (G * 1024)
@@ -37,24 +165,23 @@
 }
 template <int G, int RL>
 __host__ __device__ constexpr size_t w8l_lds_bytes() { return (size_t)w8l_nslot<G, RL>() * G * 1024 + w8l_cnt_bytes<RL>(); }
-template <int N>
-__device__ __forceinline__ void w8l_wait_bar() { asm volatile("s_waitcnt vmcnt(%0) lgkmcnt(0)\n\ts_barrier" ::"n"(N) : "memory"); }
 
 template <int G, int RL, bool NT>
 __global__ void __launch_bounds__(64 * W8L_NW, 1)
 scan8wl_kernel(const float* __restrict__ Xq, const uint32_t* __restrict__ mask, const float* __restrict__ Qq,
                const float* __restrict__ lsl, const float* __restrict__ qscal, int64_t N, int B,
                float* __restrict__ gl_s, uint32_t* __restrict__ gl_i, int64_t gl_cap, uint32_t* __restrict__ seg_cnt,
-               const uint32_t* __restrict__ gthr, uint32_t* __restrict__ chkp) {
+               const uint32_t* __restrict__ gthr, uint32_t* __restrict__ chkp, W8lDeal dl) {
     constexpr int NW = W8L_NW, NSLOT = w8l_nslot<G, RL>(), P = NSLOT / RL - 1;
     constexpr size_t TILE_B = (size_t)G * 1024;
     constexpr size_t GSTEP = 8 * BLOCK_FLOATS;
     constexpr int LPW = RL * G / NW;
     static_assert((RL * G) % NW == 0, "a round's blocks spread evenly over the waves");
-    static_assert(P >= 1 && (P - 1) * LPW <= 63, "ring / vmcnt range");
+    static_assert(P >= 1 && P <= 3 && (P - 1) * LPW <= 63, "ring / vmcnt range; first claims (w8l_dealer: A <= 5)");
     extern __shared__ __attribute__((aligned(16))) char s_dyn[];
     int* s_seg = (int*)(s_dyn + NSLOT * TILE_B);
     uint32_t* s_ck = (uint32_t*)(s_seg + W8L_QB);
+    uint32_t* s_q = s_ck + W8L_QB;
 
     const int lane = threadIdx.x & 63;
     const int wv = __builtin_amdgcn_readfirstlane(threadIdx.x >> 6);
@@ -64,9 +191,14 @@
     const int q0 = qtile * 32;
     const bool active = rl < RL;
     const int64_t T = (N + 31) >> 5;
-    const int my_tiles = T > w ? (int)((T - 1 - w) / n_seg + 1) : 0;
-    const int n_rounds = (my_tiles + RL - 1) / RL;
     const uint32_t ring = (uint32_t)(uintptr_t)(const __attribute__((address_space(3))) char*)s_dyn;
+    if (w < dl.skip) return w8l_skip_out(B, n_seg, w, seg_cnt, chkp);
+#ifdef VDB_DEAL_STAMP
+    const unsigned long long st_t0 = wall_clock64();
+#endif
+    w8l_dealer<RL, P> deal;
+    deal.init(s_q, dl, T, n_seg, w);
+    if (wv == 0) deal.first_claims(lane);
 
     if constexpr (RL > 1) {
         for (int i = threadIdx.x; i < W8L_QB; i += 64 * NW) {
@@ -77,16 +209,22 @@
     int cnt = 0;
 
     auto issue = [&](int R) {
+        deal.issue_claim(R);
+        if (R >= deal.s_end) return;
         const int rs = (R % (NSLOT / RL)) * RL;
 #pragma unroll
         for (int u = 0; u < LPW; ++u) {
             const int j = wv * LPW + u;
             const int i = j / G, g = j % G;
-            const int m = R * RL + i;
-            if (RL == 1 || m < my_tiles)
-                w8l_glds<NT>(Xq + corpus_block((uint64_t)m * n_seg + w, g, 0, G) + lane * 4,
+            const uint32_t t = deal.tile(deal.ib, R, i);
+            if (t < (uint32_t)T)
+                w8l_glds<NT>(Xq + corpus_block((uint64_t)t, g, 0, G) + lane * 4,
                              ring + (uint32_t)((rs + i) * TILE_B) + (uint32_t)(g * 1024));
         }
+#ifdef VDB_DEAL_STAMP
+#pragma unroll
+        for (int i = 0; i < RL; ++i) deal.n_tiles += deal.tile(deal.ib, R, i) < (uint32_t)T ? 1 : 0;
+#endif
     };
 
     const float uH = qscal[0], invU = qscal[2];
@@ -101,19 +239,23 @@
 #pragma unroll
         for (int g = 0; g < G; ++g) qr[g] = *(const f32x4*)(qs + g * GSTEP);
     }
-#pragma unroll
-    for (int p = 0; p < P; ++p)
-        if (p < n_rounds) issue(p);
-
-    for (int R = 0; R < n_rounds; ++R) {
-        if (P > 1 && R + P - 1 < n_rounds && (R + P) * RL <= my_tiles)
+    __syncthreads();
+    uint32_t got;
+    asm volatile("v_mov_b32 %0, 0" : "=v"(got));
+#pragma unroll
+    for (int p = 0; p < P; ++p) issue(p);
+
+    for (int R = 0; R < deal.s_end; ++R) {
+        if (P > 1 && R + P - 1 < deal.s_full)
             w8l_wait_bar<(P - 1) * LPW>();
         else
             w8l_wait_bar<0>();
-        if (R + P < n_rounds) issue(R + P);
-        const int m = R * RL + rl;
-        if (!active || m >= my_tiles) continue;
-        const int64_t t = (int64_t)m * n_seg + w;
+        deal.turn(R, wv, got);
+        issue(R + P);
+        do {
+        deal.score_claim(R);
+        const int64_t t = deal.tile(deal.sb, R, rl < RL ? rl : 0);
+        if (!active || t >= T) continue;
         i32x16 aH;
 #pragma unroll
         for (int v = 0; v < 16; ++v) aH[v] = 0;
@@ -179,6 +321,8 @@
                 ++pos;
             }
         }
+        } while (0);
+        deal.turn_end(wv, lane, got);
     }
     asm volatile("s_waitcnt vmcnt(0)" ::: "memory");
     if constexpr (RL == 1) {
@@ -199,25 +343,33 @@
         seg_cnt[(size_t)i * n_seg + w] = (uint32_t)s_seg[i];
         if (chkp) chkp[(size_t)i * n_seg + w] = s_ck[i];
     }
+#ifdef VDB_DEAL_STAMP
+    if (threadIdx.x == 0 && w < W8L_ST_WG) {
+        unsigned long long* o = g_deal_stamps[dl.stamp % W8L_ST_LAUNCH][w];
+        o[0] = st_t0;
+        o[1] = wall_clock64();
+        o[2] = (unsigned long long)deal.n_tiles;
+        o[3] = 1ull;
+    }
+#endif
 }
 
 constexpr int W8L1_SMAX = 6;
 
+constexpr int W8L1_CNT_B = W8L_QB * 4 + W8L_CQ * 4;
 template <int G>
 __host__ __device__ constexpr int w8l1_nslot() {
-    return (160 * 1024 - W8L_QB * 4) / (G * 1024) < W8L1_SMAX ? (160 * 1024 - W8L_QB * 4) / (G * 1024) : W8L1_SMAX;
-}
-template <int N>
-__device__ __forceinline__ void w8l1_wait_bar() { asm volatile("s_waitcnt vmcnt(%0) lgkmcnt(0)\n\ts_barrier" ::"n"(N) : "memory"); }
+    return (160 * 1024 - W8L1_CNT_B) / (G * 1024) < W8L1_SMAX ? (160 * 1024 - W8L1_CNT_B) / (G * 1024) : W8L1_SMAX;
+}
 template <int G>
-__host__ __device__ constexpr size_t w8l1_lds_bytes() { return (size_t)w8l1_nslot<G>() * G * 1024 + (size_t)W8L_QB * 4; }
+__host__ __device__ constexpr size_t w8l1_lds_bytes() { return (size_t)w8l1_nslot<G>() * G * 1024 + (size_t)W8L1_CNT_B; }
 
 template <int G, bool NT>
 __global__ void __launch_bounds__(64 * W8L_NW, 1)
 scan8wl1_kernel(const float* __restrict__ Xq, const uint32_t* __restrict__ mask, const float* __restrict__ Qq,
                const float* __restrict__ lsl, const float* __restrict__ qscal, int64_t N, int B, float* __restrict__ gl_s, uint32_t* __restrict__ gl_i,
                int64_t gl_cap, uint32_t* __restrict__ seg_cnt, const uint32_t* __restrict__ gthr,
-               uint32_t* __restrict__ chkp) {
+               uint32_t* __restrict__ chkp, W8lDeal dl) {
     constexpr int NW = W8L_NW, NSLOT = w8l1_nslot<G>();
     constexpr size_t TILE_B = (size_t)G * 1024;
     constexpr size_t GSTEP = 8 * BLOCK_FLOATS;
@@ -225,6 +377,7 @@
     static_assert(G % NW == 0, "a tile's blocks spread evenly over the waves");
     extern __shared__ __attribute__((aligned(16))) char s_dyn[];
     int* s_seg = (int*)(s_dyn + NSLOT * TILE_B);
+    uint32_t* s_q = (uint32_t*)(s_seg + W8L_QB);
 
     const int lane = threadIdx.x & 63;
     const int wv = __builtin_amdgcn_readfirstlane(threadIdx.x >> 6);
@@ -232,14 +385,26 @@
     const int q0 = wv * 32;
     const bool active = q0 < B;
     const int64_t T = (N + 31) >> 5;
-    const int64_t my_tiles = T > w ? (T - 1 - w) / n_seg + 1 : 0;
     const uint32_t ring = (uint32_t)(uintptr_t)(const __attribute__((address_space(3))) char*)s_dyn;
+    if (w < dl.skip) return w8l_skip_out(B, n_seg, w, seg_cnt, chkp);
+#ifdef VDB_DEAL_STAMP
+    const unsigned long long st_t0 = wall_clock64();
+#endif
+    w8l_dealer<1, NSLOT - 1> deal;
+    deal.init(s_q, dl, T, n_seg, w);
+    if (wv == 0) deal.first_claims(lane);
 
     if (lane < 32) s_seg[wv * 32 + lane] = 0;
 
-    auto issue = [&](int64_t m) {
+    auto issue = [&](int m) {
+        deal.issue_claim(m);
+        if (m >= deal.s_end) return;
         const uint32_t sbase = ring + (uint32_t)((m % NSLOT) * TILE_B);
-        const int64_t t = m * n_seg + w;
+        const uint32_t t = deal.tile(deal.ib, m, 0);
+        if (t >= (uint32_t)T) return;
+#ifdef VDB_DEAL_STAMP
+        ++deal.n_tiles;
+#endif
 #pragma unroll
         for (int u = 0; u < LPW; ++u) {
             const int g = wv * LPW + u;
@@ -259,22 +424,28 @@
 #pragma unroll
         for (int g = 0; g < G; ++g) qr[g] = *(const f32x4*)(qs + g * GSTEP);
     }
-#pragma unroll
-    for (int p = 0; p < NSLOT - 1; ++p)
-        if (p < my_tiles) issue(p);
-
-    for (int64_t m = 0; m < my_tiles; ++m) {
-        static_assert(NSLOT >= 2 && NSLOT <= 6 && (NSLOT - 2) * LPW <= 63, "vmcnt range");
-        switch ((int)min<int64_t>(NSLOT - 2, my_tiles - 1 - m)) {
-            case 4: w8l1_wait_bar<4 * LPW>(); break;
-            case 3: w8l1_wait_bar<3 * LPW>(); break;
-            case 2: w8l1_wait_bar<2 * LPW>(); break;
-            case 1: w8l1_wait_bar<LPW>(); break;
-            default: w8l1_wait_bar<0>(); break;
-        }
-        if (m + NSLOT - 1 < my_tiles) issue(m + NSLOT - 1);
+    __syncthreads();
+    uint32_t got;
+    asm volatile("v_mov_b32 %0, 0" : "=v"(got));
+#pragma unroll
+    for (int p = 0; p < NSLOT - 1; ++p) issue(p);
+
+    for (int m = 0; m < deal.s_end; ++m) {
+        static_assert(NSLOT >= 3 && NSLOT <= 6 && (NSLOT - 2) * LPW < 63, "vmcnt range; first claims (w8l_dealer: A <= 5)");
+        switch (min(NSLOT - 2, deal.s_full - 1 - m)) {
+            case 4: w8l_wait_bar<4 * LPW>(); break;
+            case 3: w8l_wait_bar<3 * LPW>(); break;
+            case 2: w8l_wait_bar<2 * LPW>(); break;
+            case 1: w8l_wait_bar<LPW>(); break;
+            default: w8l_wait_bar<0>(); break;
+        }
+        deal.turn(m, wv, got);
+        issue(m + NSLOT - 1);
+        do {
         if (!active) continue;
-        const int64_t t = m * n_seg + w;
+        deal.score_claim(m);
+        const int64_t t = deal.tile(deal.sb, m, 0);
+        if (t >= T) continue;
         i32x16 aH;
 #pragma unroll
         for (int v = 0; v < 16; ++v) aH[v] = 0;
@@ -334,6 +505,8 @@
                 ++pos;
             }
         }
+        } while (0);
+        deal.turn_end(wv, lane, got);
     }
     asm volatile("s_waitcnt vmcnt(0)" ::: "memory");
     if (!active) return;
@@ -342,6 +515,15 @@
         const uint32_t hsum = ckh + (uint32_t)__shfl_xor((int)ckh, 32, 64);
         if (lane < 32 && q < B) chkp[(size_t)q * n_seg + w] = hsum;
     }
+#ifdef VDB_DEAL_STAMP
+    if (threadIdx.x == 0 && w < W8L_ST_WG) {
+        unsigned long long* o = g_deal_stamps[dl.stamp % W8L_ST_LAUNCH][w];
+        o[0] = st_t0;
+        o[1] = wall_clock64();
+        o[2] = (unsigned long long)deal.n_tiles;
+        o[3] = 1ull;
+    }
+#endif
 }
 
 bool scan8wl_ok(int prec, int metric, int G8, int B) {
@@ -352,8 +534,13 @@
 static hipError_t scan8wl_launch(const float* Xq, const uint32_t* mask, const float* Qq, const float* lsl,
                                  const float* qscal, int64_t N, int B, int n_seg, float* gl_s, uint32_t* gl_i,
                                  int64_t gl_cap, uint32_t* seg_cnt, const uint32_t* gthr, uint32_t* chkp,
-                                 hipStream_t st) {
-    auto k = RL == 1 ? scan8wl1_kernel<G, NT> : scan8wl_kernel<G, RL, NT>;
+                                 const W8lDeal& dl, hipStream_t st) {
+    const auto k = [] {
+        if constexpr (RL == 1)
+            return scan8wl1_kernel<G, NT>;
+        else
+            return scan8wl_kernel<G, RL, NT>;
+    }();
     constexpr size_t lds = RL == 1 ? w8l1_lds_bytes<G>() : w8l_lds_bytes<G, RL>();
     static_assert(lds <= 160 * 1024, "LDS");
     static std::atomic<bool> lds_set{false};
@@ -363,7 +550,7 @@
         lds_set = true;
     }
     hipLaunchKernelGGL(k, dim3((unsigned)n_seg), dim3(64 * W8L_NW), lds, st, Xq, mask, Qq, lsl, qscal, N, B, gl_s, gl_i,
-                       gl_cap, seg_cnt, gthr, chkp);
+                       gl_cap, seg_cnt, gthr, chkp, dl);
     return hipGetLastError();
 }
 
@@ -378,13 +565,28 @@
 hipError_t launch_scan8wl(int prec, int metric, const float* Xq, const uint32_t* mask, const float* Qq,
                           const float* lsl, const float* qscal, int G8, int64_t N, int B, int n_seg, float* gl_s,
                           uint32_t* gl_i, int64_t gl_cap, uint32_t* seg_cnt, const uint32_t* gthr, uint32_t* chkp,
-                          hipStream_t st) {
+                          uint32_t* tctr, int deal_ch, int deal_win, int deal_cap, int deal_skip, hipStream_t st) {
     if (!scan8wl_ok(prec, metric, G8, B) || n_seg <= 0 || gl_cap != (int64_t)n_seg * W8_CH) return hipErrorInvalidValue;
+    const int64_t T = (N + 31) / 32;
+    if ((deal_ch != 4 && deal_ch != 8 && deal_ch != 16) || deal_win < 1 ||
+        (int64_t)deal_win * n_seg * deal_ch < T || (int64_t)deal_win * n_seg >= (int64_t)1 << 31 || deal_cap < 1 ||
+        deal_skip < 0 || deal_skip >= n_seg || (deal_skip > 0 && !tctr))
+        return hipErrorInvalidValue;
+    W8lDeal dl{};
+    dl.ctr = tctr;
+    dl.ch_log2 = deal_ch == 4 ? 2 : deal_ch == 8 ? 3 : 4;
+    dl.n_win = deal_win;
+    dl.cap = deal_cap;
+    dl.skip = deal_skip;
+#ifdef VDB_DEAL_STAMP
+    static std::atomic<int> n_launch{0};
+    dl.stamp = n_launch.fetch_add(1) % W8L_ST_LAUNCH;
+#endif
     const int rl = scan8wl_rl(G8, B);
 #define W8L_CASE(GV, RLV)                                                                                          \
     if (G8 == GV && rl == RLV)                                                                                     \
         return scan8wl_launch<GV, RLV, true>(Xq, mask, Qq, lsl, qscal, N, B, n_seg, gl_s, gl_i, gl_cap, seg_cnt, gthr, \
-                                             chkp, st);
+                                             chkp, dl, st);
     W8L_CASE(16, 1) W8L_CASE(24, 1) W8L_CASE(32, 1) W8L_CASE(48, 1)
     W8L_CASE(16, 2) W8L_CASE(24, 2) W8L_CASE(32, 2)
 #undef W8L_CASE
@@ -392,3 +594,16 @@
 }
 
 }
+
+#ifdef VDB_DEAL_STAMP
+extern "C" int vdb_debug_deal_stamps(unsigned long long* out, int n_launches) {
+    return (int)hipMemcpyFromSymbol(out, HIP_SYMBOL(vdb::g_deal_stamps),
+                                    sizeof(unsigned long long) * 4 * vdb::W8L_ST_WG * (size_t)n_launches);
+}
+extern "C" int vdb_debug_deal_stamps_clear() {
+    void* p = nullptr;
+    hipError_t e = hipGetSymbolAddress(&p, HIP_SYMBOL(vdb::g_deal_stamps));
+    if (e != hipSuccess) return (int)e;
+    return (int)hipMemset(p, 0, sizeof(vdb::g_deal_stamps));
+}
+#endif
diff --git a/mlx-vector-db_amd/csrc/vdb_search_plan.h b/mlx-vector-db_amd/csrc/vdb_search_plan.h
--- a/mlx-vector-db_amd/csrc/vdb_search_plan.h
+++ b/mlx-vector-db_amd/csrc/vdb_search_plan.h
@@ -28,6 +28,7 @@
 constexpr int FIN_SEG_MAX = 512;
 constexpr int64_t kRefineMinDp = 512;
 constexpr int kGateSlots = 4;
+constexpr bool kDealAutoRl[2] = {false, false};
 
 inline int64_t plan_round_up(int64_t a, int64_t b) { return (a + b - 1) / b * b; }
 inline int plan_next_pow2(int v) {
@@ -36,6 +37,11 @@
     return p;
 }
 inline int64_t plan_align(int64_t b) { return (b + 255) / 256 * 256; }
+inline int plan_deal_cap(bool deal, int n_win, int n_seg, int skip) {
+    if (!deal) return n_win;
+    const int64_t rest = std::max(1, n_seg - skip);
+    return (int)std::max<int64_t>(2 * (int64_t)n_win, ((int64_t)n_win * n_seg + rest - 1) / rest);
+}
 
 struct SearchShape {
     int B, k;
@@ -53,6 +59,8 @@
     int64_t margin;
     bool i8_narrow;
     int64_t scan_q4, scan_wide;
+    int64_t scan_deal;
+    int64_t scan_deal_ch;
     int64_t n_wg_override;
     int64_t scan_variant;
     int64_t scan_sync;
@@ -66,6 +74,7 @@
 };
 struct SearchKernelFacts {
     bool scan8wl_ok;
+    int scan8wl_rl;
     bool scan8w_ok;
     bool scan_variant_ok;
     int rows_per_step;
@@ -104,6 +113,10 @@
     bool wide_long;
     bool wide8;
     int n_seg8;
+    bool deal;
+    int deal_ch;
+    int deal_win;
+    int deal_cap;
     int QB, QB_pilot;
     int Bp;
     int n_qblocks;
@@ -142,6 +155,12 @@
                : kn.n_wg_override > 0
                    ? (int)std::min<int64_t>(FIN_SEG_MAX, std::min<int64_t>(kn.n_wg_override, n_tiles_all))
                    : (int)std::min<int64_t>(FIN_SEG_MAX, plan_round_up(std::min<int64_t>(s.n_cu, n_tiles_all), 8));
+    if (g.wide_long) {
+        g.deal = kn.scan_deal == 1 || (kn.scan_deal < 0 && kDealAutoRl[f.scan8wl_rl == 2 ? 1 : 0]);
+        g.deal_ch = kn.scan_deal_ch > 0 ? (int)kn.scan_deal_ch : f.scan8wl_rl == 2 ? 8 : 16;
+        g.deal_win = (int)((n_tiles_all + (int64_t)g.n_seg8 * g.deal_ch - 1) / ((int64_t)g.n_seg8 * g.deal_ch));
+        g.deal_cap = plan_deal_cap(g.deal, g.deal_win, g.n_seg8, 0);
+    }
     g.QB = g.q4 ? 128 : g.i8_pass ? 64 : KP == 256 ? 32 : 64;
     g.QB_pilot = g.i8_pass ? 64 : KP == 256 ? 32 : 64;
     g.Bp = (int)plan_round_up(B, 128);
@@ -216,6 +235,7 @@
     int64_t q8max, q8lsl, q8err, q8scal;
     int64_t q8res, q8err2;
     int64_t chkp, segc, chkr;
+    int64_t tctr;
     int64_t rs8;
     int64_t chke;
     int64_t rep_q, rep_s, rep_i, rep_k;
@@ -260,6 +280,7 @@
     l.chkp = take(g.chk, 2 * (int64_t)g.n_wg8 * Bp * 4);
     l.segc = take(g.wide8, Bp * g.n_seg8 * 4);
     l.chkr = take(g.chk && s.metric == 1, 64 * 4);
+    l.tctr = take(g.wide_long, 256);
     l.rs8 = take(g.rs8_on, plan_round_up(s.N, std::max<int64_t>(32, g.step_rows)) * 4);
     l.chke = take(g.chk && p.n_pilot > 0, 2 * Bp * 4);
     l.rep_q = take(dev, (int64_t)g.R_rep * D * 4);
```

After: 489,900 queries/s. No clear change (-0.2%).
